# maxgillett/tinysplat

Measured on AMD Instinct MI355X. Metric: Gaussians*pixels/s fwd+bwd, higher is better.
Workload: dtype f32; 1 GPU; 1000000 random Gaussians, SH degree 3, 1920x1080, fwd+bwd (RGB), BASELINE configs[2]; max_per_tile=614, parallelism=single GPU, tile_lists=16x16 (gsplat's) (auto), gaussian_order=as generated (i.i.d.)

## Files before the change

### include/tinysplat_hip.h

```cpp
#ifndef TINYSPLAT_HIP_H
#define TINYSPLAT_HIP_H

#include <stdint.h>

#ifdef __cplusplus
extern "C" {
#endif

#define TS_ABI_VERSION 8

#define TS_E_BADARG (-1)
#define TS_E_DEGREE (-2)

#define TS_TILE 16
#define TS_SPLAT_RECORD_FLOATS 12
#define TS_PARTIAL_ROW_FLOATS 12

int ts_abi_version(void);

typedef struct ts_camera {
    float fx, fy, cx, cy;
    int32_t img_width, img_height;
    int32_t tile_bounds_x, tile_bounds_y;
    int32_t tile_row0, tile_rows;
    float glob_scale;
    float clip_thresh;
    int32_t wide_tiles;
    int32_t hints;
} ts_camera;
#define TS_HINT_BALANCED_WALK 1
#define TS_HINT_COOP_SPLIT (1 << 20)
#define TS_CAM_LIST_SEGMENTS(s) (((s) & 15) << 8)
#define TS_CAM_WHOLE_TILES(w16) (((w16) & 15) << 12)
#define TS_CAM_COOP_TILES(c16) (((c16) & 15) << 16)
int64_t ts_final_floats(const ts_camera* cam_host, int32_t channels);
int32_t ts_cut_tiles(const ts_camera* cam_host, int32_t* band, int32_t* whole);
int32_t ts_num_tiles(const ts_camera* cam_host);


#define TS_PROJECT_LOG_SCALES 1
#define TS_PROJECT_RAW_QUATS 2

int ts_project_fwd(int32_t n, const float* means3d, const float* scales, const float* quats,
                   const float* viewmat, const float* projmat, const ts_camera* cam_host,
                   int32_t flags, float* xys, float* depths, int32_t* radii, float* conics,
                   int32_t* num_tiles_hit, float* cov3d, void* stream);

int ts_project_bwd(int32_t n, const float* means3d, const float* scales, const float* quats,
                   const float* viewmat, const float* projmat, const ts_camera* cam_host,
                   int32_t flags, const int32_t* radii, const float* v_xy, const float* v_depth,
                   const float* v_conic, const float* v_cov3d,
                   float* v_means3d, float* v_scales, float* v_quats, void* stream);


int ts_sh_fwd(int32_t n, int32_t degrees_to_use, int32_t num_bases, const float* viewdirs,
              const float* coeffs, float* colors, void* stream);

int ts_sh_bwd(int32_t n, int32_t degrees_to_use, int32_t num_bases, const float* viewdirs,
              const float* v_colors, float* v_coeffs, void* stream);

int ts_sh_colors_fwd(int32_t n, int32_t degrees_to_use, int32_t num_bases, const float* means3d,
                     const float* origin, const float* colors_dc, const float* colors_rest,
                     float* colors, uint8_t* clamp_mask, const int32_t* live, void* stream);
int ts_sh_colors_bwd(int32_t n, int32_t degrees_to_use, int32_t num_bases, const float* means3d,
                     const float* origin, const uint8_t* clamp_mask, const float* v_colors,
                     float* v_colors_dc, float* v_colors_rest, void* stream);
int ts_colors_pack_fwd(int32_t n, int32_t degrees_to_use, int32_t num_bases, const float* means3d,
                       const float* origin, const float* colors_dc, const float* colors_rest,
                       uint8_t* clamp_mask, const int32_t* live, int32_t channels, int32_t flags,
                       const float* xys, const int32_t* radii, const float* conics, const float* opacity,
                       const int32_t* cum_tiles_hit, const ts_camera* cam_host, const float* depths,
                       float* splats, void* stream);


int64_t ts_scan_ws_ints(int32_t n);
int ts_scan_tiles(int32_t n, const int32_t* num_tiles_hit, int32_t* cum_tiles_hit,
                  int32_t* scan_ws, int32_t* total_out, void* stream);

int64_t ts_bin_ws_ints(int32_t n, int32_t num_tiles);

int ts_bin_count(int32_t n, const float* xys, const int32_t* radii, const float* splats,
                 const ts_camera* cam_host, int32_t* bin_ws, void* stream);

int ts_tile_offsets(int32_t n, int32_t num_tiles, int32_t* bin_ws, int32_t* tile_bins,
                    const int32_t* cum_tiles_hit, int64_t capacity, void* stream);
int ts_tile_offsets_stats(int32_t n, int32_t num_tiles, int32_t* bin_ws, int32_t* tile_bins,
                          const int32_t* cum_tiles_hit, int64_t capacity, int32_t* longest_list, void* stream);

int ts_bin_scatter(int32_t n, const float* xys, const int32_t* radii, const float* splats,
                   const ts_camera* cam_host, const int32_t* bin_ws, int32_t* bucket_ids, int32_t* scratch,
                   void* stream);

int ts_sort_tiles(int32_t num_tiles, const int32_t* tile_bins, const float* depths,
                  const int32_t* bucket_ids, int32_t* gaussian_ids_sorted, int32_t* sort_ws,
                  int32_t* zeroed_counter, void* stream);
int ts_sort_tiles_above(int32_t num_tiles, const int32_t* tile_bins, const float* depths,
                        const int32_t* bucket_ids, int32_t* gaussian_ids_sorted, int32_t* sort_ws,
                        int32_t* zeroed_counter, void* stream);

int32_t ts_bin_group_form(int32_t n);
int ts_bin_count_groups(int32_t n, const float* xys, const int32_t* radii, const float* splats,
                        const ts_camera* cam_host, int32_t* bin_ws, void* stream);
int ts_group_offsets(int32_t n, int32_t num_tiles, int32_t* bin_ws, int32_t* tile_bins,
                     const int32_t* cum_tiles_hit, int64_t capacity, int32_t* longest_list, void* stream);
int ts_bin_scatter_groups(int32_t n, const float* xys, const int32_t* radii, const float* splats,
                          const ts_camera* cam_host, int32_t* bin_ws, int32_t* tile_bins, int32_t* bucket_ids,
                          int32_t* scratch, void* stream);
int32_t ts_bin_one_walk_form(int32_t n, int32_t num_tiles);
int32_t ts_bin_stage_capacity(void);
int ts_bin_emit_groups(int32_t n, const float* xys, const int32_t* radii, const float* splats,
                       const ts_camera* cam_host, const int32_t* cum_tiles_hit, int64_t capacity, int32_t* bin_ws,
                       int32_t* scratch, void* stream);
int ts_emit_offsets(int32_t n, int32_t num_tiles, int32_t* bin_ws, int32_t* tile_bins,
                    const int32_t* cum_tiles_hit, int64_t capacity, int32_t* longest_list, void* stream);
int ts_bin_gather_groups(int32_t n, int32_t num_tiles, int32_t* bin_ws, int32_t* tile_bins, int32_t* bucket_ids,
                         const int32_t* scratch, void* stream);
int ts_sort_tiles_stats(int32_t num_tiles, const int32_t* tile_bins, const float* depths,
                        const int32_t* bucket_ids, int32_t* gaussian_ids_sorted, int32_t* sort_ws,
                        int32_t* zeroed_counter, int32_t n, const int32_t* bin_ws, int32_t* longest_list,
                        void* stream);
int ts_sort_tiles_above_stats(int32_t num_tiles, const int32_t* tile_bins, const float* depths,
                              const int32_t* bucket_ids, int32_t* gaussian_ids_sorted, int32_t n,
                              const int32_t* bin_ws, int32_t* longest_list, void* stream);

#define TS_RASTER_LOGIT_OPACITY 1

int ts_pack_splats(int32_t n, int32_t channels, int32_t flags, const float* xys, const int32_t* radii,
                   const float* conics, const float* colors, const float* opacity,
                   const int32_t* cum_tiles_hit, const ts_camera* cam_host, const float* depths,
                   float* splats, void* stream);

#define TS_RASTER_CLAMP_RGB 2
#define TS_RASTER_SPLIT_BLOCKS 4
#define TS_RASTER_NARROW_WAVES 8
#define TS_RASTER_FLAG_GEN(g) (((g) & 0xff) << 8)
int ts_raster_fwd(int32_t channels, int32_t flags, const ts_camera* cam_host, const int32_t* tile_bins,
                  const int32_t* gaussian_ids_sorted, const float* splats, const float* background,
                  float* out_img, float* final_Ts, int32_t* final_index, uint8_t* clamp_mask,
                  void* stream);
int ts_raster_fwd_planes(int32_t channels, int32_t flags, const ts_camera* cam_host, const int32_t* tile_bins,
                         const int32_t* gaussian_ids_sorted, const float* splats, const float* background,
                         float* out_img, float* out_depth, float* final_Ts, int32_t* final_index,
                         uint8_t* clamp_mask, void* stream);

int ts_raster_fwd_sort(int32_t channels, int32_t flags, const ts_camera* cam_host, const int32_t* tile_bins,
                       const int32_t* bucket_ids, const float* depths, int32_t* gaussian_ids_sorted,
                       const float* splats, const float* background, float* out_img, float* out_depth,
                       float* final_Ts, int32_t* final_index, uint8_t* clamp_mask, void* stream);

int ts_raster_bwd(int32_t channels, int32_t flags, int64_t num_intersects, const ts_camera* cam_host,
                  const int32_t* tile_bins, const int32_t* gaussian_ids_sorted, const float* splats,
                  const float* background, const float* final_Ts, const int32_t* final_index,
                  const float* v_out_img, const float* v_out_alpha, const uint8_t* clamp_mask,
                  float* partials, uint8_t* row_flags, void* stream);
int ts_raster_bwd_planes(int32_t channels, int32_t flags, int64_t num_intersects, const ts_camera* cam_host,
                         const int32_t* tile_bins, const int32_t* gaussian_ids_sorted, const float* splats,
                         const float* background, const float* final_Ts, const int32_t* final_index,
                         const float* v_out_img, const float* v_out_depth, int32_t planes,
                         const float* v_out_alpha, const uint8_t* clamp_mask,
                         float* partials, uint8_t* row_flags, void* stream);

int ts_reduce_partials(int32_t n, int32_t channels, int32_t flags, const int32_t* num_tiles_hit,
                       const int32_t* cum_tiles_hit, const float* partials,
                       const uint8_t* row_flags, const float* splats, float* v_xy, float* v_conic,
                       float* v_colors, float* v_opacity, float* v_depth, const uint8_t* color_mask,
                       void* stream);

#define TS_FRAME_TIGHT 1
#define TS_FRAME_SPLIT 2
#define TS_FRAME_NARROW_WAVES 8
#define TS_FRAME_DIRECT_SCATTER 32
#define TS_FRAME_PLANES 64
#define TS_FRAME_LIST_STATS 256
#define TS_FRAME_SEPARATE_SORT 128
#define TS_FRAME_STRIPE 16
#define TS_FRAME_GROUP_COUNTS 1024
#define TS_FRAME_ONE_WALK 2048
#define TS_FRAME_SURVIVORS 512
typedef struct ts_frame {
    int32_t n, num_bases, sh_degree, channels, flags;
    int32_t flag_gen;
    ts_camera cam;
    const float *means, *scales, *quats, *opacities, *colors_dc, *colors_rest;
    const float *view34, *projview, *origin, *background;
    float *xys, *depths, *conics, *colors, *splats;
    int32_t *radii, *num_tiles_hit, *cum_tiles_hit;
    uint8_t* sh_mask;
    int32_t *scan_ws, *bin_ws, *tile_bins;
    int32_t* total_host;
    int64_t num_intersects;
    int64_t capacity;
    int32_t *bucket_ids, *gaussian_ids_sorted;
    float *out_img, *final_Ts;
    int32_t* final_index;
    uint8_t* clamp_mask;
    const float* v_out_img;
    float* partials;
    uint8_t* row_flags;
    float *v_xy, *v_conic, *v_colors, *v_depth, *v_opacity;
    float *v_means, *v_scales, *v_quats, *v_colors_dc, *v_colors_rest;
    float* out_depth;
    const float* v_out_depth;
    int32_t* survivors;
} ts_frame;
int32_t ts_frame_struct_bytes(void);
int ts_frame_fwd_project(const ts_frame* f, void* stream);
int ts_frame_fwd_prepare(const ts_frame* f, void* stream);
int ts_frame_fwd_composite(const ts_frame* f, void* stream);
int ts_frame_bwd_composite(const ts_frame* f, void* stream);
int ts_frame_bwd_params(const ts_frame* f, void* stream);

typedef void (*ts_entry_probe)(const char* entry, int32_t end, void* user);
int ts_set_entry_probe(ts_entry_probe fn, void* user);

#define TS_MAX_RANKS 16
#define TS_EXPORT_RECORD_FLOATS 16
typedef struct ts_stripes {
    int32_t num;
    int32_t row[TS_MAX_RANKS + 1];
} ts_stripes;
int64_t ts_route_ws_ints(int32_t n, int32_t num_ranks);
int ts_route_count(int32_t n, const float* xys, const int32_t* radii, const ts_camera* cam_host,
                   const ts_stripes* stripes_host, int32_t* route_ws, int32_t* counts, void* stream);
int ts_route_count_padded(int32_t n, const float* xys, const int32_t* radii, const ts_camera* cam_host,
                          const ts_stripes* stripes_host, const int32_t* group_base_host, int32_t* route_ws,
                          int32_t* counts, void* stream);
int ts_route_pack(int32_t n, int32_t gid_base, const float* xys, const int32_t* radii, const float* depths,
                  const float* splats, const ts_camera* cam_host, const ts_stripes* stripes_host,
                  const int32_t* route_ws, float* records, void* stream);
int ts_import_records(int32_t m, const float* records, const ts_camera* cam_host, float* xys, float* depths,
                      int32_t* radii, int32_t* num_tiles_hit, void* stream);
int ts_import_pack(int32_t m, const float* records, const int32_t* cum_tiles_hit, const ts_camera* cam_host,
                   float* splats, void* stream);
int ts_reduce_partials_rows(int32_t n, int32_t channels, int32_t flags, const int32_t* num_tiles_hit,
                            const int32_t* cum_tiles_hit, const float* partials, const uint8_t* row_flags,
                            const float* splats, float* grad_rows, void* stream);
int ts_route_accumulate(int32_t n, int32_t channels, const float* xys, const int32_t* radii, const float* splats,
                        const uint8_t* color_mask, const ts_camera* cam_host, const ts_stripes* stripes_host,
                        const int32_t* route_ws, const float* grad_rows, float* v_xy, float* v_conic,
                        float* v_colors, float* v_depth, float* v_opacity, void* stream);

int ts_shard_owner_fwd(const ts_frame* fo, const ts_stripes* stripes_host, int32_t* route_ws, int32_t* counts,
                       void* stream);
int ts_shard_owner_fwd_padded(const ts_frame* fo, const ts_stripes* stripes_host, const int32_t* group_base_host,
                              int32_t* route_ws, int32_t* counts, void* stream);
int ts_shard_owner_fwd_fused(int32_t n, int32_t degrees_to_use, int32_t num_bases, const float* means3d,
                             const float* scales, const float* quats, const float* view34, const float* projview,
                             const ts_camera* cam_host, int32_t project_flags, const float* origin,
                             const float* colors_dc, const float* colors_rest, const float* opacity, int32_t channels,
                             int32_t raster_flags, float* xys, float* depths, int32_t* radii, float* conics,
                             int32_t* num_tiles_hit, uint8_t* clamp_mask, float* splats, const ts_stripes* stripes_host,
                             const int32_t* group_base_host, int32_t* route_ws, int32_t* counts, void* stream);
int ts_shard_owner_bwd_fused(int32_t n, int32_t channels, int32_t degrees_to_use, int32_t num_bases, const float* means3d,
                             const float* scales, const float* quats, const float* view34, const float* projview,
                             const float* origin, const float* xys, const int32_t* radii, const float* splats,
                             const uint8_t* color_mask, const ts_camera* cam_host, const ts_stripes* stripes_host,
                             const int32_t* route_ws, const float* grad_rows, float* v_xy, float* v_conic,
                             float* v_colors, float* v_depth, float* v_opacity, float* v_colors_dc, float* v_colors_rest,
                             float* v_means3d, float* v_scales, float* v_quats, void* stream);
int ts_shard_stripe_fwd_import(const ts_frame* fs, const float* records, void* stream);
int ts_shard_stripe_bwd(const ts_frame* fs, float* grad_rows, void* stream);
int ts_shard_owner_bwd(const ts_frame* fo, const ts_stripes* stripes_host, const int32_t* route_ws,
                       const float* grad_rows, void* stream);

typedef struct ts_rank_step {
    ts_stripes stripes;
    int32_t group_base[TS_MAX_RANKS + 1];
    int32_t gid_base;
    int32_t send_rows, recv_rows;
    int32_t* route_ws;
    int32_t* counts;
    float *send, *recv;
    float *grad_rows, *back;
} ts_rank_step;
int32_t ts_rank_step_struct_bytes(void);
int ts_shard_rank_fwd_a(const ts_frame* fo, const ts_rank_step* r, void* stream);
int ts_shard_rank_fwd_b(const ts_frame* fs, const ts_rank_step* r, void* stream);
int ts_shard_rank_bwd_a(const ts_frame* fs, const ts_rank_step* r, void* stream);
int ts_shard_rank_bwd_b(const ts_frame* fo, const ts_rank_step* r, void* stream);


int64_t ts_photometric_ws_floats(int32_t height, int32_t width);
int ts_photometric_loss_rgbd(int32_t height, int32_t width, int32_t pixel_floats, const float* image,
                             const float* target, const float* depth_target, float w_l1,
                             float w_ssim, float w_depth, float* ws, float* v_image, void* stream);
int ts_photometric_loss(int32_t height, int32_t width, const float* image, const float* target,
                        float w_l1, float w_ssim, float* ws, float* v_image, void* stream);
int ts_photometric_loss_planes(int32_t height, int32_t width, const float* image, const float* depth,
                               const float* target, const float* depth_target, float w_l1, float w_ssim,
                               float w_depth, float* ws, float* v_image, float* v_depth, void* stream);
int ts_photometric_loss_reduce(int32_t height, int32_t width, float w_l1, float w_ssim, float w_depth,
                               const float* ws, float* out4, void* stream);

#define TS_ADAM_MAX_TENSORS 8
int ts_adam_step(int32_t num_tensors, float* const* params_host, const float* const* grads_host,
                 float* const* exp_avg_host, float* const* exp_avg_sq_host, const int64_t* numel_host,
                 const float* lr_host, const int32_t* steps_host, float beta1, float beta2, float eps,
                 void* stream);

#define TS_ADAM_MEANS 0
#define TS_ADAM_COLORS_DC 1
#define TS_ADAM_COLORS_REST 2
#define TS_ADAM_SCALES 3
#define TS_ADAM_QUATS 4
#define TS_ADAM_OPACITIES 5
typedef struct ts_adam {
    float* exp_avg[6];
    float* exp_avg_sq[6];
    float lr[6];
    int32_t step[6];
    float beta1, beta2, eps;
} ts_adam;
int ts_sh_colors_bwd_adam(int32_t n, int32_t degrees_to_use, int32_t num_bases, const float* means3d,
                          const float* origin, const uint8_t* clamp_mask, const float* v_colors,
                          float* colors_dc, float* colors_rest, const ts_adam* adam_host, void* stream);
int ts_project_bwd_adam(int32_t n, float* means3d, float* scales, float* quats, const float* viewmat,
                        const float* projmat, const ts_camera* cam_host, int32_t flags, const int32_t* radii,
                        const float* v_xy, const float* v_depth, const float* v_conic, float* opacities,
                        const float* v_opacity, const ts_adam* adam_host, void* stream);
int ts_frame_bwd_params_adam(const ts_frame* f, const ts_adam* adam_host, void* stream);

#define TS_DENSIFY_CLONE 1
#define TS_DENSIFY_SPLIT 2
#define TS_DENSIFY_PRUNE 4

typedef struct ts_densify_policy {
    float interval_densify;
    float max_dim;
    float tau_means;
    float scale_thresh;
} ts_densify_policy;
// ... 161 lines not shown
```

### tinysplat_amd/_lib.py

```python
from __future__ import annotations

import ctypes
import os
from ctypes import POINTER, c_double, c_float, c_int32, c_int64, c_void_p
from pathlib import Path

LIB_PATH = Path(os.environ["TS_LIB_PATH"]) if os.environ.get("TS_LIB_PATH") else \
    Path(__file__).resolve().parent / "csrc" / "libtinysplat_hip.so"
ABI_VERSION = 8
HINT_BALANCED_WALK = 1
HINT_COOP_SPLIT = 1 << 20
PARTIAL_ROW_FLOATS = 12


class TsCamera(ctypes.Structure):
    _fields_ = [
        ("fx", c_float), ("fy", c_float), ("cx", c_float), ("cy", c_float),
        ("img_width", c_int32), ("img_height", c_int32),
        ("tile_bounds_x", c_int32), ("tile_bounds_y", c_int32),
        ("tile_row0", c_int32), ("tile_rows", c_int32),
        ("glob_scale", c_float), ("clip_thresh", c_float),
        ("wide_tiles", c_int32), ("hints", c_int32),
    ]


_P = c_void_p
_CAM = POINTER(TsCamera)


class TsDensifyPolicy(ctypes.Structure):
    _fields_ = [("interval_densify", c_float), ("max_dim", c_float), ("tau_means", c_float),
                ("scale_thresh", c_float)]


class TsFrame(ctypes.Structure):
    _fields_ = ([("n", c_int32), ("num_bases", c_int32), ("sh_degree", c_int32), ("channels", c_int32),
                 ("flags", c_int32), ("flag_gen", c_int32), ("cam", TsCamera)]
                + [(name, c_void_p) for name in (
                    "means", "scales", "quats", "opacities", "colors_dc", "colors_rest",
                    "view34", "projview", "origin", "background",
                    "xys", "depths", "conics", "colors", "splats",
                    "radii", "num_tiles_hit", "cum_tiles_hit", "sh_mask",
                    "scan_ws", "bin_ws", "tile_bins", "total_host")]
                + [("num_intersects", c_int64), ("capacity", c_int64)]
                + [(name, c_void_p) for name in (
                    "bucket_ids", "gaussian_ids_sorted", "out_img", "final_Ts", "final_index", "clamp_mask",
                    "v_out_img", "partials", "row_flags",
                    "v_xy", "v_conic", "v_colors", "v_depth", "v_opacity",
                    "v_means", "v_scales", "v_quats", "v_colors_dc", "v_colors_rest",
                    "out_depth", "v_out_depth", "survivors")])


_FRAME = POINTER(TsFrame)


class TsAdam(ctypes.Structure):
    _fields_ = [("exp_avg", c_void_p * 6), ("exp_avg_sq", c_void_p * 6), ("lr", c_float * 6), ("step", c_int32 * 6),
                ("beta1", c_float), ("beta2", c_float), ("eps", c_float)]


_ADAM = POINTER(TsAdam)

MAX_RANKS = 16


class TsStripes(ctypes.Structure):
    _fields_ = [("num", c_int32), ("row", c_int32 * (MAX_RANKS + 1))]


_STRIPES = POINTER(TsStripes)


class TsRankStep(ctypes.Structure):
    _fields_ = [("stripes", TsStripes), ("group_base", c_int32 * (MAX_RANKS + 1)), ("gid_base", c_int32),
                ("send_rows", c_int32), ("recv_rows", c_int32), ("route_ws", c_void_p), ("counts", c_void_p),
                ("send", c_void_p), ("recv", c_void_p), ("grad_rows", c_void_p), ("back", c_void_p)]


_RANK = POINTER(TsRankStep)

ENTRY_PROBE = ctypes.CFUNCTYPE(None, ctypes.c_char_p, c_int32, c_void_p)

SIGNATURES = {
    "ts_abi_version": (c_int32, []),
    "ts_project_fwd": (c_int32, [c_int32, _P, _P, _P, _P, _P, _CAM, c_int32, _P, _P, _P, _P, _P, _P, _P]),
    "ts_project_bwd": (c_int32, [c_int32, _P, _P, _P, _P, _P, _CAM, c_int32, _P, _P, _P, _P, _P, _P, _P, _P, _P]),
    "ts_sh_fwd": (c_int32, [c_int32, c_int32, c_int32, _P, _P, _P, _P]),
    "ts_sh_bwd": (c_int32, [c_int32, c_int32, c_int32, _P, _P, _P, _P]),
    "ts_sh_colors_fwd": (c_int32, [c_int32, c_int32, c_int32, _P, _P, _P, _P, _P, _P, _P, _P]),
    "ts_sh_colors_bwd": (c_int32, [c_int32, c_int32, c_int32, _P, _P, _P, _P, _P, _P, _P]),
    "ts_scan_ws_ints": (c_int64, [c_int32]),
    "ts_scan_tiles": (c_int32, [c_int32, _P, _P, _P, _P, _P]),
    "ts_bin_ws_ints": (c_int64, [c_int32, c_int32]),
    "ts_bin_count": (c_int32, [c_int32, _P, _P, _P, _CAM, _P, _P]),
    "ts_tile_offsets": (c_int32, [c_int32, c_int32, _P, _P, _P, c_int64, _P]),
    "ts_tile_offsets_stats": (c_int32, [c_int32, c_int32, _P, _P, _P, c_int64, _P, _P]),
    "ts_bin_scatter": (c_int32, [c_int32, _P, _P, _P, _CAM, _P, _P, _P, _P]),
    "ts_sort_tiles": (c_int32, [c_int32, _P, _P, _P, _P, _P, _P, _P]),
    "ts_sort_tiles_above": (c_int32, [c_int32, _P, _P, _P, _P, _P, _P, _P]),
    "ts_bin_group_form": (c_int32, [c_int32]),
    "ts_bin_count_groups": (c_int32, [c_int32, _P, _P, _P, _CAM, _P, _P]),
    "ts_group_offsets": (c_int32, [c_int32, c_int32, _P, _P, _P, c_int64, _P, _P]),
    "ts_bin_scatter_groups": (c_int32, [c_int32, _P, _P, _P, _CAM, _P, _P, _P, _P, _P]),
    "ts_bin_one_walk_form": (c_int32, [c_int32, c_int32]),
    "ts_bin_stage_capacity": (c_int32, []),
    "ts_bin_emit_groups": (c_int32, [c_int32, _P, _P, _P, _CAM, _P, c_int64, _P, _P, _P]),
    "ts_emit_offsets": (c_int32, [c_int32, c_int32, _P, _P, _P, c_int64, _P, _P]),
    "ts_bin_gather_groups": (c_int32, [c_int32, c_int32, _P, _P, _P, _P, _P]),
    "ts_sort_tiles_stats": (c_int32, [c_int32, _P, _P, _P, _P, _P, _P, c_int32, _P, _P, _P]),
    "ts_sort_tiles_above_stats": (c_int32, [c_int32, _P, _P, _P, _P, c_int32, _P, _P, _P]),
    "ts_num_tiles": (c_int32, [_CAM]),
    "ts_final_floats": (c_int64, [_CAM, c_int32]),
    "ts_cut_tiles": (c_int32, [_CAM, _P, _P]),
    "ts_colors_pack_fwd": (c_int32, [c_int32, c_int32, c_int32, _P, _P, _P, _P, _P, _P, c_int32, c_int32,
                                     _P, _P, _P, _P, _P, _CAM, _P, _P, _P]),
    "ts_pack_splats": (c_int32, [c_int32, c_int32, c_int32, _P, _P, _P, _P, _P, _P, _CAM, _P, _P, _P]),
    "ts_raster_fwd": (c_int32, [c_int32, c_int32, _CAM, _P, _P, _P, _P, _P, _P, _P, _P, _P]),
    "ts_raster_bwd": (c_int32, [c_int32, c_int32, c_int64, _CAM, _P, _P, _P, _P, _P, _P, _P, _P, _P, _P, _P, _P]),
    "ts_raster_fwd_planes": (c_int32, [c_int32, c_int32, _CAM, _P, _P, _P, _P, _P, _P, _P, _P, _P, _P]),
    "ts_raster_fwd_sort": (c_int32, [c_int32, c_int32, _CAM, _P, _P, _P, _P, _P, _P, _P, _P, _P, _P, _P, _P]),
    "ts_raster_bwd_planes": (c_int32, [c_int32, c_int32, c_int64, _CAM, _P, _P, _P, _P, _P, _P, _P, _P, c_int32,
                                       _P, _P, _P, _P, _P]),
    "ts_bench_stream_read": (c_int32, [_P, c_int64, _P, _P]),
    "ts_bench_gather48": (c_int32, [_P, _P, c_int64, _P, _P]),
    "ts_photometric_ws_floats": (c_int64, [c_int32, c_int32]),
    "ts_photometric_loss": (c_int32, [c_int32, c_int32, _P, _P, c_float, c_float, _P, _P, _P]),
    "ts_photometric_loss_rgbd": (c_int32, [c_int32, c_int32, c_int32, _P, _P, _P, c_float, c_float, c_float, _P, _P, _P]),
    "ts_photometric_loss_planes": (c_int32, [c_int32, c_int32, _P, _P, _P, _P, c_float, c_float, c_float, _P, _P, _P,
                                             _P]),
    "ts_photometric_loss_reduce": (c_int32, [c_int32, c_int32, c_float, c_float, c_float, _P, _P, _P]),
    "ts_adam_step": (c_int32, [c_int32, _P, _P, _P, _P, _P, _P, _P, c_float, c_float, c_float, _P]),
    "ts_sh_colors_bwd_adam": (c_int32, [c_int32, c_int32, c_int32, _P, _P, _P, _P, _P, _P, _ADAM, _P]),
    "ts_project_bwd_adam": (c_int32, [c_int32, _P, _P, _P, _P, _P, _CAM, c_int32, _P, _P, _P, _P, _P, _P, _ADAM, _P]),
    "ts_frame_bwd_params_adam": (c_int32, [_FRAME, _ADAM, _P]),
    "ts_grad_accum": (c_int32, [c_int32, _P, _P, _P]),
    "ts_densify_classify": (c_int32, [c_int32, _P, _P, _P, POINTER(TsDensifyPolicy), _P, _P]),
    "ts_densify_ws_ints": (c_int64, [c_int32]),
    "ts_densify_plan": (c_int32, [c_int32, _P, _P, _P, _P, _P]),
    "ts_gather_rows": (c_int32, [c_int32, _P, _P, _P, c_int32, c_int32, _P, _P]),
    "ts_split_fixup": (c_int32, [c_int32, _P, _P, _P, _P, _P, _P, _P, _P]),
    "ts_ply_row_floats": (c_int32, [c_int32]),
    "ts_ply_pack_rows": (c_int32, [c_int32, c_int32, _P, _P, _P, _P, _P, _P, _P, _P]),
    "ts_ply_unpack_rows": (c_int32, [c_int32, c_int32, _P, _P, _P, _P, _P, _P, _P, _P]),
    "ts_reduce_partials": (c_int32, [c_int32, c_int32, c_int32, _P, _P, _P, _P, _P, _P, _P, _P, _P, _P, _P, _P]),
    "ts_route_ws_ints": (c_int64, [c_int32, c_int32]),
    "ts_route_count": (c_int32, [c_int32, _P, _P, _CAM, _STRIPES, _P, _P, _P]),
    "ts_route_count_padded": (c_int32, [c_int32, _P, _P, _CAM, _STRIPES, _P, _P, _P, _P]),
    "ts_route_pack": (c_int32, [c_int32, c_int32, _P, _P, _P, _P, _CAM, _STRIPES, _P, _P, _P]),
    "ts_import_records": (c_int32, [c_int32, _P, _CAM, _P, _P, _P, _P, _P]),
    "ts_import_pack": (c_int32, [c_int32, _P, _P, _CAM, _P, _P]),
    "ts_reduce_partials_rows": (c_int32, [c_int32, c_int32, c_int32, _P, _P, _P, _P, _P, _P, _P]),
    "ts_route_accumulate": (c_int32, [c_int32, c_int32, _P, _P, _P, _P, _CAM, _STRIPES, _P, _P, _P, _P, _P, _P, _P, _P]),
    "ts_shard_owner_fwd": (c_int32, [_FRAME, _STRIPES, _P, _P, _P]),
    "ts_shard_owner_fwd_padded": (c_int32, [_FRAME, _STRIPES, _P, _P, _P, _P]),
    "ts_shard_owner_fwd_fused": (c_int32, [c_int32, c_int32, c_int32, _P, _P, _P, _P, _P, _CAM, c_int32, _P, _P, _P, _P,
                                           c_int32, c_int32, _P, _P, _P, _P, _P, _P, _P, _STRIPES, _P, _P, _P, _P]),
    "ts_shard_owner_bwd_fused": (c_int32, [c_int32, c_int32, c_int32, c_int32, _P, _P, _P, _P, _P, _P, _P, _P, _P, _P,
                                           _CAM, _STRIPES, _P, _P, _P, _P, _P, _P, _P, _P, _P, _P, _P, _P, _P]),
    "ts_shard_stripe_fwd_import": (c_int32, [_FRAME, _P, _P]),
    "ts_shard_stripe_bwd": (c_int32, [_FRAME, _P, _P]),
    "ts_shard_owner_bwd": (c_int32, [_FRAME, _STRIPES, _P, _P, _P]),
    "ts_rank_step_struct_bytes": (c_int32, []),
    "ts_shard_rank_fwd_a": (c_int32, [_FRAME, _RANK, _P]),
    "ts_shard_rank_fwd_b": (c_int32, [_FRAME, _RANK, _P]),
    "ts_shard_rank_bwd_a": (c_int32, [_FRAME, _RANK, _P]),
    "ts_shard_rank_bwd_b": (c_int32, [_FRAME, _RANK, _P]),
    "ts_frame_struct_bytes": (c_int32, []),
    "ts_frame_fwd_project": (c_int32, [_FRAME, _P]),
    "ts_frame_fwd_prepare": (c_int32, [_FRAME, _P]),
    "ts_frame_fwd_composite": (c_int32, [_FRAME, _P]),
    "ts_frame_bwd_composite": (c_int32, [_FRAME, _P]),
    "ts_frame_bwd_params": (c_int32, [_FRAME, _P]),
    "ts_set_entry_probe": (c_int32, [_P, _P]),
    "ts_knn_ws_bytes": (c_int64, [c_int32, c_int32, c_int32]),
    "ts_knn": (c_int32, [c_int32, _P, c_int32, _P, c_int32, _P, _P, _P, _P, _P]),
    "ts_init_from_points": (c_int32, [c_int32, c_int32, _P, _P, _P, _P, _P, _P, _P, _P, _P, _P, _P, _P, _P, _P]),
    "ts_opacity_entropy_ws_bytes": (c_int64, [c_int32]),
    "ts_opacity_entropy": (c_int32, [c_int32, _P, _P, _P, _P, _P]),
    "ts_density_sample_ws_bytes": (c_int64, [c_int32]),
    "ts_density_sample": (c_int32, [c_int32, c_int32, c_int32, _P, _P, _P, _P, _P, _P, _P, _P, _P, _P, _P]),
    "ts_density_loss_ws_bytes": (c_int64, [c_int32]),
    "ts_density_loss": (c_int32, [c_int32, c_int32, _P, _P, _P, _P, _P, _P, _P, _P, c_int32, c_int32, _P, _P, c_int32,
                                  c_float, _P, _P, _P, _P, _P, _P, _P, _P, _P, _P]),
    "ts_segment_sum_ws_bytes": (c_int64, [c_int64, c_int32]),
    "ts_segment_sum": (c_int32, [c_int64, c_int32, c_int32, _P, _P, _P, _P, _P, _P, _P]),
    "ts_extract_pack": (c_int32, [c_int32, _P, _P, _P, _P, _P, _P, _P]),
    "ts_extract_rays": (c_int32, [c_int32, _P, c_int32, c_int32, _P, c_int32, _P, _P, _P, _P, _P, _P]),
    "ts_extract_samples": (c_int32, [c_int32, c_int32, c_int32, c_float, _P, _P, _P, _P, _P, _P, _P]),
    "ts_extract_march": (c_int32, [c_int32, c_int32, c_int32, c_float, c_float, _P, _P, _P, _P, _P, _P, _P, _P, _P, _P,
                                   _P, _P, _P]),
    "ts_extract_normals": (c_int32, [c_int32, c_int32, _P, _P, _P, _P, _P]),
    "ts_extract_chunk_bytes": (c_int64, [c_int32, c_int32, c_int32]),
    "ts_mesh_boxes": (c_int32, [c_int32, _P, _P, _P, c_float, _P, _P]),
    "ts_mesh_mark": (c_int32, [c_int32, _P, _P, _P, _P, _P]),
    "ts_mesh_chunk_bytes": (c_int64, [c_int32, c_int32]),
    "ts_mesh_corners": (c_int32, [c_int32, _P, _P, _P, _P, _P]),
    "ts_mesh_density": (c_int32, [c_int32, c_int32, _P, _P, _P, _P, _P, _P, _P, _P]),
    "ts_mesh_count": (c_int32, [c_int32, _P, _P, _P, c_float, _P, _P, _P]),
    "ts_mesh_emit": (c_int32, [c_int32, _P, _P, _P, c_float, _P, _P, _P, _P, _P, _P]),
    "ts_field_colors": (c_int32, [c_int32, c_int32, _P, _P, _P, _P, _P, _P, c_int32, c_int32, _P, _P]),
    "ts_simplify_count": (c_int32, [c_int32, c_int32, _P, _P, _P, _P, _P, _P]),
    "ts_simplify_keys": (c_int32, [c_int32, _P, _P, _P, _P, _P]),
    "ts_simplify_ws_bytes": (c_int64, [c_int64]),
    "ts_simplify_accumulate": (c_int32, [c_int32, c_int32, c_int32, _P, _P, _P, _P, c_int32, c_int64, _P, _P, c_int64,
                                         c_int64, _P, _P, _P]),
    "ts_simplify_solve": (c_int32, [c_int32, _P, _P, _P, _P, _P, c_double, _P, _P]),
    "ts_simplify_faces": (c_int32, [c_int32, c_int32, _P, _P, _P, _P, _P]),
    "ts_clean_degenerate": (c_int32, [c_int32, _P, _P, _P]),
    "ts_clean_edge_keys": (c_int32, [c_int32, c_int32, _P, _P, _P]),
    "ts_clean_face_weights": (c_int32, [c_int32, c_int32, _P, _P, _P, _P]),
    "ts_clean_mark": (c_int32, [c_int32, c_int64, _P, _P, _P, _P]),
    "ts_clean_components": (c_int32, [c_int32, c_int32, _P, _P, _P, _P]),
    "ts_splat_keys": (c_int32, [c_int32, _P, _P, _P, _P]),
    "ts_splat_pack": (c_int32, [c_int32, c_int32, _P, _P, _P, _P, _P, _P, _P, _P]),
    "ts_splat_unpack": (c_int32, [c_int32, _P, _P, _P, _P, _P, _P, _P]),
    "ts_undistort_image": (c_int32, [_P, c_int32, c_int32, POINTER(c_float), POINTER(c_float), POINTER(c_float),
                                     c_int32, c_int32, c_int32, _P, _P]),
    "ts_jpeg_ws_bytes": (c_int64, [c_int32, c_int32, c_int32, c_int32]),
    "ts_jpeg_max_bytes": (c_int64, [c_int32, c_int32, c_int32, c_int32]),
    "ts_jpeg_header": (c_int64, [c_int32, c_int32, c_int32, c_int32, c_int32, _P, c_int64]),
    "ts_jpeg_encode": (c_int32, [_P, c_int32, c_int32, c_int32, c_int32, c_int32, c_int32, c_int32, _P, _P, c_int64, _P,
                                 _P, _P]),
    "ts_image_metrics_ws_bytes": (c_int64, [c_int32, c_int32]),
    "ts_image_metrics": (c_int32, [c_int32, c_int32, c_int32, _P, _P, c_int32, _P, _P, _P]),
}

_lib = None


class HipLibraryError(RuntimeError):
    pass


def load() -> ctypes.CDLL:
    global _lib
    if _lib is not None:
        return _lib
    if not LIB_PATH.exists():
        raise HipLibraryError(
            f"{LIB_PATH} is missing: tinysplat_amd has no CPU or PyTorch fallback. "
            "Build it with `python -m tinysplat_amd._build` (needs hipcc, targets gfx950).")
    stamp = LIB_PATH.with_suffix(LIB_PATH.suffix + ".flags")
    if stamp.exists() and "-DTS_" in stamp.read_text() and os.environ.get("TS_ALLOW_VARIANT_LIB") != "1":
        raise HipLibraryError(
            f"{LIB_PATH} was built with developer -DTS_* overrides (ablation variant; its results may be "
            "wrong). Rebuild with `python -m tinysplat_amd._build`, or set TS_ALLOW_VARIANT_LIB=1.")
    lib = ctypes.CDLL(str(LIB_PATH))
    for name, (res, args) in SIGNATURES.items():
        try:
            fn = getattr(lib, name)
        except AttributeError as e:
            raise HipLibraryError(f"{LIB_PATH} does not export {name}") from e
        fn.restype = res
        fn.argtypes = args
    v = lib.ts_abi_version()
    if v != ABI_VERSION:
        raise HipLibraryError(f"ABI version mismatch: library {v}, binding {ABI_VERSION}")
    if lib.ts_frame_struct_bytes() != ctypes.sizeof(TsFrame):
        raise HipLibraryError("struct ts_frame: the ctypes mirror does not match the library's layout")
    if lib.ts_rank_step_struct_bytes() != ctypes.sizeof(TsRankStep):
        raise HipLibraryError("struct ts_rank_step: the ctypes mirror does not match the library's layout")
    _lib = lib
    return lib


def check(code: int, what: str) -> None:
    if code == 0:
        return
# ... 6 lines not shown
```

### tinysplat_amd/csrc/binning.hip

```cpp
#include <hip/hip_runtime.h>

#include "../../include/tinysplat_hip.h"
#include "host_util.h"
#include "pack.h"
#include "splat_math.h"

namespace {

constexpr int kThreads = 256;
constexpr int kScanItems = 4;
constexpr int kScanBlock = kThreads * kScanItems;

__device__ __forceinline__ int wave_inclusive_scan(int v) {
    const int lane = threadIdx.x & 63;
#pragma unroll
    for (int d = 1; d < 64; d <<= 1) {
        const int u = __shfl_up(v, d, 64);
        if (lane >= d) v += u;
    }
    return v;
}

template <int WAVES = 4>
__device__ __forceinline__ int block_inclusive_scan(int v, int* total) {
    __shared__ int wave_sums[WAVES];
    const int lane = threadIdx.x & 63, wave = threadIdx.x >> 6;
    int inc = wave_inclusive_scan(v);
    if (lane == 63) wave_sums[wave] = inc;
    __syncthreads();
    int add = 0, tot = 0;
#pragma unroll
    for (int w = 0; w < WAVES; ++w) {
        const int s = wave_sums[w];
        if (w < wave) add += s;
        tot += s;
    }
    *total = tot;
    __syncthreads();
    return inc + add;
}

__global__ __launch_bounds__(kThreads) void scan_local_kernel(int n, const int* __restrict__ in,
                                                              int* __restrict__ out,
                                                              int* __restrict__ block_sums,
                                                              int* __restrict__ total_out) {
    const int base = blockIdx.x * kScanBlock + threadIdx.x * kScanItems;
    int v[kScanItems];
    int sum = 0;
#pragma unroll
    for (int k = 0; k < kScanItems; ++k) {
        v[k] = (base + k < n) ? in[base + k] : 0;
        sum += v[k];
        v[k] = sum;
    }
    int total;
    const int inc = block_inclusive_scan(sum, &total);
    const int excl = inc - sum;
#pragma unroll
    for (int k = 0; k < kScanItems; ++k)
        if (base + k < n) {
            out[base + k] = v[k] + excl;
            if (total_out && gridDim.x == 1 && base + k == n - 1)
                __hip_atomic_store(total_out, v[k] + excl, __ATOMIC_RELEASE, __HIP_MEMORY_SCOPE_SYSTEM);
        }
    if (threadIdx.x == 0) block_sums[blockIdx.x] = total;
}

__global__ __launch_bounds__(kThreads) void scan_add_kernel(int n, int* __restrict__ out,
                                                            const int* __restrict__ block_sums,
                                                            int* __restrict__ total_out) {
    __shared__ int red[kThreads / 64];
    int part = 0;
    for (int j = threadIdx.x; j < (int)blockIdx.x; j += kThreads) part += block_sums[j];
#pragma unroll
    for (int d = 32; d >= 1; d >>= 1) part += __shfl_xor(part, d, 64);
    if ((threadIdx.x & 63) == 0) red[threadIdx.x >> 6] = part;
    __syncthreads();
    int add = 0;
#pragma unroll
    for (int w = 0; w < kThreads / 64; ++w) add += red[w];
    const int base = blockIdx.x * kScanBlock + threadIdx.x * kScanItems;
#pragma unroll
    for (int k = 0; k < kScanItems; ++k)
        if (base + k < n) {
            const int v = out[base + k] + add;
            if (blockIdx.x != 0) out[base + k] = v;
            if (total_out && base + k == n - 1)
                __hip_atomic_store(total_out, v, __ATOMIC_RELEASE, __HIP_MEMORY_SCOPE_SYSTEM);
        }
}

#ifndef TS_BIN_THREADS
#define TS_BIN_THREADS 1024
#endif
constexpr int kBinThreads = TS_BIN_THREADS;
#ifndef TS_BIN_CHUNK
#define TS_BIN_CHUNK 4096
#endif
constexpr int kBinChunkMin = TS_BIN_CHUNK;
constexpr int kBinMaxChunks = 512;
constexpr int kBinWindowMax = 36864;
constexpr int kBinTargetBlocks = 1;

__host__ __device__ inline int bin_num_chunks(int n) {
    int per = n / 192;
    per = per < 1024 ? 1024 : (per > kBinChunkMin ? kBinChunkMin : per);
    int b = (n + per - 1) / per;
    if (b < 1) b = 1;
    if (b > kBinMaxChunks) b = kBinMaxChunks;
    return b;
}

inline int bin_window_tiles(int n, int num_tiles) {
    const int chunks = bin_num_chunks(n);
    int nwin = (kBinTargetBlocks + chunks - 1) / chunks;
    const int max_win = (num_tiles + 255) / 256;
    if (nwin > max_win) nwin = max_win;
    if (nwin < 1) nwin = 1;
    int window = (num_tiles + nwin - 1) / nwin;
    window = (window + 63) & ~63;
    if (window > kBinWindowMax) window = kBinWindowMax;
    return window;
}

using ts::TightTest;

#ifndef TS_BIN_PRE
#define TS_BIN_PRE 2
#endif
constexpr int kBinPre = TS_BIN_PRE;
template <typename Emit>
__device__ __forceinline__ void walk_chunk(int g0, int g1, const float* __restrict__ xys,
                                           const int* __restrict__ radii,
                                           const float4* __restrict__ splats, const ts_camera& cam,
                                           Emit emit) {
    const int ws = cam.wide_tiles ? 1 : 0;
    const int tbx = (cam.tile_bounds_x + ws) >> ws;
    const bool tight_lists = splats != nullptr;
    for (int base = g0 + threadIdx.x; base < g1; base += kBinPre * kBinThreads) {
        int r[kBinPre];
        float2 xy[kBinPre];
        float4 q0[kBinPre], q1[kBinPre];
#pragma unroll
        for (int u = 0; u < kBinPre; ++u) {
            const int i = base + u * kBinThreads;
            r[u] = i < g1 ? radii[i] : 0;
        }
#pragma unroll
        for (int u = 0; u < kBinPre; ++u) {
            const int i = base + u * kBinThreads;
            xy[u] = make_float2(0.f, 0.f);
            q0[u] = q1[u] = make_float4(0.f, 0.f, 0.f, 0.f);
            if (r[u] > 0) {
                xy[u] = reinterpret_cast<const float2*>(xys)[i];
                if (tight_lists) { q0[u] = splats[3 * (size_t)i]; q1[u] = splats[3 * (size_t)i + 1]; }
            }
        }
#pragma unroll
        for (int u = 0; u < kBinPre; ++u) {
            if (r[u] <= 0) continue;
            const ts::TileBox b = ts::tile_bbox(xy[u].x, xy[u].y, (float)r[u], cam.tile_bounds_x,
                                                cam.tile_bounds_y, cam.tile_row0, cam.tile_rows);
            if (b.maxy <= b.miny || b.maxx <= b.minx) continue;
            const TightTest tight(tight_lists, q0[u].x, q0[u].y, q0[u].z, q0[u].w, q1[u].x, q1[u].y, (float)r[u]);
            if (tight.cull_all) continue;
            const int i = base + u * kBinThreads;
            for (int ty = b.miny; ty < b.maxy; ++ty) {
                int lo, hi;
                tight.row_range(ty, b.minx, b.maxx, lo, hi);
                if (hi <= lo) continue;
                for (int tx = lo >> ws; tx <= (hi - 1) >> ws; ++tx) emit((ty - cam.tile_row0) * tbx + tx, i);
            }
        }
    }
}

constexpr int kItemCap = 4096;
constexpr int kStashWords = 11;
constexpr size_t kBalancedLds = (size_t)(kStashWords * kBinThreads + kItemCap + 32) * 4;
template <typename Emit>
__device__ __forceinline__ void walk_chunk_balanced(int g0, int g1, const float* __restrict__ xys,
                                                    const int* __restrict__ radii,
                                                    const float4* __restrict__ splats, const ts_camera& cam,
                                                    Emit emit) {
    static_assert(kBinThreads == 1024, "one Gaussian per thread and batch, items packed as lt | row << 10");
    __shared__ float stash[kStashWords][kBinThreads];
    __shared__ int items[kItemCap];
    __shared__ int wave_sum[kBinThreads / 64 + 1];
    const int ws = cam.wide_tiles ? 1 : 0;
    const int tbx = (cam.tile_bounds_x + ws) >> ws;
    const bool tight_lists = splats != nullptr;
    const int tid = threadIdx.x, lane = tid & 63, wave = tid >> 6;
    for (int base = g0; base < g1; base += kBinThreads) {
// ... 841 lines not shown

constexpr int kMaxSub = 512;
constexpr int kSubTarget = 96;
constexpr int kLargeLdsU64 = kSortCap + 2048;

__device__ __forceinline__ void sort_tile_sample(const int* __restrict__ g,
                                                 const float* __restrict__ depths,
                                                 int* __restrict__ out, int n,
                                                 unsigned long long* lds) {
    unsigned long long* scratch = lds;
    unsigned long long* smp = lds + kSortCap;
    int* start = reinterpret_cast<int*>(lds + kSortCap + 1024);
    int* cursor = start + (kMaxSub + 1);
    int* big = cursor + kMaxSub;
    __shared__ int nbig;
    const int t = threadIdx.x, lane = t & 63, wave = t >> 6;
    const int ns = n > 8192 ? 1024 : 256;
    int nb = n / kSubTarget;
    nb = nb < 2 ? 2 : (nb > kMaxSub ? kMaxSub : nb);

    if (ns == 1024) {
        unsigned long long k[4];
#pragma unroll
        for (int e = 0; e < 4; ++e)
            k[e] = make_key(depths, g[(int)(((long long)(t * 4 + e) * n) >> 10)]);
        bitonic_regs<4, kThreads>(k, t, 1024, scratch);
#pragma unroll
        for (int e = 0; e < 4; ++e) smp[t * 4 + e] = k[e];
    } else {
        unsigned long long k[1];
        k[0] = make_key(depths, g[(int)(((long long)t * n) >> 8)]);
        bitonic_regs<1, kThreads>(k, t, 256, scratch);
        smp[t] = k[0];
    }
    for (int b = t; b < nb; b += kThreads) cursor[b] = 0;
    if (t == 0) nbig = 0;
    __syncthreads();

    auto sub_of = [&](unsigned long long key) {
        int lo = 0, hi = nb - 1;
        while (lo < hi) {
            const int mid = (lo + hi) >> 1;
            if (smp[((mid + 1) * ns) / nb] <= key) lo = mid + 1; else hi = mid;
        }
        return lo;
    };
    for (int i = t; i < n; i += kThreads) atomicAdd(&cursor[sub_of(make_key(depths, g[i]))], 1);
    __syncthreads();
    {
        const int c0 = (2 * t < nb) ? cursor[2 * t] : 0, c1 = (2 * t + 1 < nb) ? cursor[2 * t + 1] : 0;
        int total;
        const int inc = block_inclusive_scan(c0 + c1, &total);
        const int ex = inc - (c0 + c1);
        if (2 * t < nb) start[2 * t] = ex;
        if (2 * t + 1 < nb) start[2 * t + 1] = ex + c0;
        if (t == 0) start[nb] = n;
    }
    __syncthreads();
    for (int b = t; b < nb; b += kThreads) cursor[b] = start[b];
    __syncthreads();
    for (int i = t; i < n; i += kThreads) {
        const int id = g[i];
        out[atomicAdd(&cursor[sub_of(make_key(depths, id))], 1)] = id;
    }
    __threadfence_block();
    __syncthreads();
    for (int b = wave; b < nb; b += kThreads / 64) {
        const int s0 = start[b], m = start[b + 1] - s0;
        if (m <= 1) continue;
        if (m <= 256) {
            unsigned long long k[4];
#pragma unroll
            for (int e = 0; e < 4; ++e) {
                const int i = lane * 4 + e;
                k[e] = i < m ? make_key(depths, out[s0 + i]) : ~0ull;
            }
            bitonic_regs<4, 64>(k, lane, min(pow2_at_least(m), 256), nullptr);
#pragma unroll
            for (int e = 0; e < 4; ++e) {
                const int i = lane * 4 + e;
                if (i < m) out[s0 + i] = (int)(unsigned int)k[e];
            }
        } else if (lane == 0) {
            big[atomicAdd(&nbig, 1)] = b;
        }
    }
    __syncthreads();
    const int nbg = nbig;
    for (int q = 0; q < nbg; ++q) {
        const int b = big[q];
        const int s0 = start[b], m = start[b + 1] - s0;
        __syncthreads();
        if (m <= kSortCap) {
            sort_bucket_block(out + s0, depths, out + s0, m, scratch);
        } else {
            IdKeyArray a{out + s0, depths};
            bitonic_network(a, m);
        }
        __syncthreads();
    }
}

__global__ __launch_bounds__(kThreads) void sort_tiles_small_kernel(
    int num_tiles, const int* __restrict__ tile_bins, const float* __restrict__ depths,
    const int* __restrict__ bucket_ids, int* __restrict__ ids_sorted, int* __restrict__ large_count,
    int* __restrict__ large_list, const ListStats stats) {
    if (stats.group_max && blockIdx.x == 0) store_longest(stats);
    const int lane = threadIdx.x & 63;
    const int tile = blockIdx.x * (kThreads / 64) + (threadIdx.x >> 6);
    if (tile >= num_tiles) return;
    const int2 range = reinterpret_cast<const int2*>(tile_bins)[tile];
    const int n = range.y - range.x;
    if (n <= 0) return;
    if (n > kWaveSortMax) {
        if (n > kSortCap && lane == 0) large_list[atomicAdd(large_count, 1)] = tile;
        return;
    }
    const int* g = bucket_ids + range.x;
    int* out = ids_sorted + range.x;
    if (n <= 64) sort_tile_wave<1>(g, depths, out, n, lane);
    else if (n <= 128) sort_tile_wave<2>(g, depths, out, n, lane);
    else if (n <= 256) sort_tile_wave<4>(g, depths, out, n, lane);
    else if (n <= 512) sort_tile_wave<8>(g, depths, out, n, lane);
    else sort_tile_wave<16>(g, depths, out, n, lane);
}

__global__ __launch_bounds__(kThreads) void sort_tiles_mid_kernel(
    const int* __restrict__ tile_bins, const float* __restrict__ depths,
    const int* __restrict__ bucket_ids, int* __restrict__ ids_sorted, int* __restrict__ large_count,
    int* __restrict__ large_list) {
    __shared__ unsigned long long lk[kSortCap / 2];
    const int2 range = reinterpret_cast<const int2*>(tile_bins)[blockIdx.x];
    const int n = range.y - range.x;
    if (n > kSortCap && large_count && threadIdx.x == 0) large_list[atomicAdd(large_count, 1)] = blockIdx.x;
    if (n <= kWaveSortMax || n > kSortCap) return;
    sort_bucket_block(bucket_ids + range.x, depths, ids_sorted + range.x, n, lk);
}

__global__ __launch_bounds__(kThreads) void sort_tiles_large_kernel(
    const int* __restrict__ tile_bins, const float* __restrict__ depths,
    const int* __restrict__ bucket_ids, int* __restrict__ ids_sorted,
    const int* __restrict__ large_count, const int* __restrict__ large_list) {
    __shared__ unsigned long long lds_large[kLargeLdsU64];
    const int count = *large_count;
    for (int q = blockIdx.x; q < count; q += gridDim.x) {
        const int2 range = reinterpret_cast<const int2*>(tile_bins)[large_list[q]];
        const int n = range.y - range.x;
        if (n <= kSortCap) continue;
        __syncthreads();
        sort_tile_sample(bucket_ids + range.x, depths, ids_sorted + range.x, n, lds_large);
    }
}

__global__ __launch_bounds__(kThreads) void sort_tiles_above_kernel(
    const int* __restrict__ tile_bins, const float* __restrict__ depths,
    const int* __restrict__ bucket_ids, int* __restrict__ ids_sorted, const ListStats stats) {
    __shared__ unsigned long long lds_u64[kLargeLdsU64 > kSortCap / 2 ? kLargeLdsU64 : kSortCap / 2];
    if (stats.group_max && blockIdx.x == 0) store_longest(stats);
    const int2 range = reinterpret_cast<const int2*>(tile_bins)[blockIdx.x];
    const int n = range.y - range.x;
    if (n <= kWaveSortMax) return;
    if (n <= kSortCap) sort_bucket_block(bucket_ids + range.x, depths, ids_sorted + range.x, n, lds_u64);
    else sort_tile_sample(bucket_ids + range.x, depths, ids_sorted + range.x, n, lds_u64);
}

__global__ __launch_bounds__(kThreads) void pack_splats_kernel(int n, const ts::PackArgs a,
                                                              const float* __restrict__ colors) {
    const int i = blockIdx.x * kThreads + threadIdx.x;
    if (i >= n) return;
    if (a.radii[i] <= 0) return;
    float c0, c1, c2, c3 = 0.0f;
    if (a.channels == 4 && a.depths == nullptr) {
        const float4 c = reinterpret_cast<const float4*>(colors)[i];
        c0 = c.x; c1 = c.y; c2 = c.z; c3 = c.w;
    } else {
        c0 = colors[3 * i]; c1 = colors[3 * i + 1]; c2 = colors[3 * i + 2];
        if (a.channels == 4) c3 = a.depths[i];
    }
    ts::pack_one(a, i, c0, c1, c2, c3);
}

}

extern "C" {

int32_t ts_num_tiles(const ts_camera* cam) {
    if (!cam) return 0;
    const int tbx = cam->wide_tiles ? (cam->tile_bounds_x + 1) / 2 : cam->tile_bounds_x;
    return cam->tile_rows * tbx;
}

int64_t ts_scan_ws_ints(int32_t n) {
    return n <= 0 ? 1 : (int64_t)((n + kScanBlock - 1) / kScanBlock);
}

int ts_scan_tiles(int32_t n, const int32_t* num_tiles_hit, int32_t* cum_tiles_hit,
                  int32_t* scan_ws, int32_t* total_out, void* stream) {
    if (n < 0) return TS_E_BADARG;
    if (n == 0) return 0;
    if (!num_tiles_hit || !cum_tiles_hit || !scan_ws) return TS_E_BADARG;
    hipStream_t s = (hipStream_t)stream;
    const int nb = (n + kScanBlock - 1) / kScanBlock;
    hipLaunchKernelGGL(scan_local_kernel, dim3(nb), dim3(kThreads), 0, s, n, num_tiles_hit,
                       cum_tiles_hit, scan_ws, total_out);
    if (nb > 1)
        hipLaunchKernelGGL(scan_add_kernel, dim3(nb), dim3(kThreads), 0, s, n, cum_tiles_hit, scan_ws,
                           total_out);
    return launch_status();
}

int64_t ts_bin_ws_ints(int32_t n, int32_t num_tiles) { return bin_geometry(n, num_tiles).spare + 1; }

int ts_bin_count(int32_t n, const float* xys, const int32_t* radii, const float* splats,
                 const ts_camera* cam, int32_t* bin_ws, void* stream) {
    if (n < 0 || !cam || !bin_ws) return TS_E_BADARG;
    const int nt = ts_num_tiles(cam);
    if (nt <= 0) return 0;
    if (n > 0 && (!xys || !radii)) return TS_E_BADARG;
    const BinGeometry g = bin_geometry(n, nt);
    const int window = bin_window_tiles(n, nt);
    const int windows = (nt + window - 1) / window;
    const size_t lds = (size_t)window * sizeof(int);
    if (lds > 64 * 1024)
        (void)hipFuncSetAttribute(reinterpret_cast<const void*>(&bin_count_kernel),
                                  hipFuncAttributeMaxDynamicSharedMemorySize, (int)lds);
    hipLaunchKernelGGL(bin_count_kernel, dim3(g.chunks, windows), dim3(kBinThreads), lds,
                       (hipStream_t)stream, n, g.chunk, xys, radii,
                       reinterpret_cast<const float4*>(splats), *cam, nt, window, bin_ws);
    return launch_status();
}

int ts_tile_offsets(int32_t n, int32_t num_tiles, int32_t* bin_ws, int32_t* tile_bins,
                    const int32_t* cum_tiles_hit, int64_t capacity, void* stream) {
    return ts_tile_offsets_stats(n, num_tiles, bin_ws, tile_bins, cum_tiles_hit, capacity, nullptr, stream);
}

int ts_tile_offsets_stats(int32_t n, int32_t num_tiles, int32_t* bin_ws, int32_t* tile_bins,
                          const int32_t* cum_tiles_hit, int64_t capacity, int32_t* longest_list, void* stream) {
    if (n < 0 || num_tiles < 0) return TS_E_BADARG;
    if (num_tiles == 0) return 0;
    if (!bin_ws || !tile_bins) return TS_E_BADARG;
    const BinGeometry g = bin_geometry(n, num_tiles);
    int* tile_total = bin_ws + g.tile_start;
    const int per_group = (g.chunks + kScanGroups - 1) / kScanGroups;
    hipStream_t s = (hipStream_t)stream;
    hipLaunchKernelGGL(column_scan_kernel, dim3((num_tiles + kColTiles - 1) / kColTiles),
                       dim3(kColTiles * kScanGroups), 0, s, num_tiles, g.chunks, per_group, bin_ws, tile_total, true);
    hipLaunchKernelGGL(tile_offsets_kernel, dim3(1), dim3(kOffsetsThreads), 0, s, num_tiles, tile_total,
                       tile_bins, bin_ws + g.spare,
                       (cum_tiles_hit && n > 0) ? cum_tiles_hit + (n - 1) : nullptr, (long long)capacity, longest_list);
    return launch_status();
}

int32_t ts_bin_group_form(int32_t n) { return two_hop(n) ? 1 : 0; }

int ts_bin_count_groups(int32_t n, const float* xys, const int32_t* radii, const float* splats,
                        const ts_camera* cam, int32_t* bin_ws, void* stream) {
    if (!cam || !bin_ws || !xys || !radii || !two_hop(n)) return TS_E_BADARG;
    const int nt = ts_num_tiles(cam);
    if (nt <= 0) return 0;
    const BinGeometry g = bin_geometry(n, nt);
    hipLaunchKernelGGL(group_bin_count_kernel, dim3(g.chunks), dim3(kBinThreads), (size_t)g.groups * sizeof(int),
                       (hipStream_t)stream, n, g.chunk, xys, radii, reinterpret_cast<const float4*>(splats), *cam,
                       g.groups, bin_ws);
    return launch_status();
}

}

namespace {
template <bool BASES>
int group_offsets(const BinGeometry& g, int num_tiles, int* bin_ws, int* tile_bins, const int* total_ptr,
                  long long capacity, int* longest_list, hipStream_t s) {
    int* counts = bin_ws + (BASES ? 0 : g.counts);
    int* col_total = nullptr;
    if ((long long)g.chunks * g.groups > kGoSingleMax || g.groups > kGoLdsGroups) {
        col_total = bin_ws + (BASES ? g.group_totals : g.col_total);
        const int per_group = (g.chunks + kScanGroups - 1) / kScanGroups;
        hipLaunchKernelGGL(column_scan_kernel, dim3((g.groups + kColTiles - 1) / kColTiles),
                           dim3(kColTiles * kScanGroups), 0, s, g.groups, g.chunks, per_group, counts, col_total, BASES);
        counts = nullptr;
    }
    hipLaunchKernelGGL(group_tile_offsets_kernel<BASES>, dim3(1), dim3(kGoThreads), 0, s, num_tiles, g.groups, g.chunks,
                       counts, (const int*)col_total, bin_ws + g.tile_start, tile_bins, bin_ws + g.spare, total_ptr,
                       capacity, longest_list);
    return launch_status();
}
}

extern "C" {

int ts_group_offsets(int32_t n, int32_t num_tiles, int32_t* bin_ws, int32_t* tile_bins,
                     const int32_t* cum_tiles_hit, int64_t capacity, int32_t* longest_list, void* stream) {
    if (num_tiles < 0 || !two_hop(n)) return TS_E_BADARG;
    if (num_tiles == 0) return 0;
    if (!bin_ws || !tile_bins) return TS_E_BADARG;
    return group_offsets<true>(bin_geometry(n, num_tiles), num_tiles, bin_ws, tile_bins,
                               cum_tiles_hit ? cum_tiles_hit + (n - 1) : nullptr, (long long)capacity, longest_list,
                               (hipStream_t)stream);
}

int ts_bin_scatter_groups(int32_t n, const float* xys, const int32_t* radii, const float* splats,
                          const ts_camera* cam, int32_t* bin_ws, int32_t* tile_bins, int32_t* bucket_ids,
                          int32_t* scratch, void* stream) {
    if (!cam || !xys || !radii || !bin_ws || !tile_bins || !bucket_ids || !scratch || !two_hop(n))
        return TS_E_BADARG;
    const int nt = ts_num_tiles(cam);
    if (nt <= 0) return 0;
    const BinGeometry g = bin_geometry(n, nt);
    int* tile_start = bin_ws + g.tile_start;
    hipStream_t s = (hipStream_t)stream;
    const auto coarse = (cam->hints & TS_HINT_BALANCED_WALK) ? bin_scatter_coarse_kernel<true, true>
                                                             : bin_scatter_coarse_kernel<false, true>;
    hipLaunchKernelGGL(coarse, dim3(g.chunks), dim3(kBinThreads), (size_t)g.groups * sizeof(int), s, n, g.chunk, xys,
                       radii, reinterpret_cast<const float4*>(splats), *cam, nt, (const int*)bin_ws,
                       (const int*)tile_start, scratch);
    hipLaunchKernelGGL(bin_scatter_fine_groups_kernel, dim3(g.groups), dim3(kFineThreads), 0, s, nt, tile_start,
                       tile_bins, bin_ws + g.group_max, (const int*)scratch, bucket_ids);
    return launch_status();
}

int32_t ts_bin_one_walk_form(int32_t n, int32_t num_tiles) { return one_walk_form(n, num_tiles) ? 1 : 0; }

int32_t ts_bin_stage_capacity(void) { return kStageCap; }

int ts_bin_emit_groups(int32_t n, const float* xys, const int32_t* radii, const float* splats,
                       const ts_camera* cam, const int32_t* cum_tiles_hit, int64_t capacity, int32_t* bin_ws,
                       int32_t* scratch, void* stream) {
    if (!cam || !xys || !radii || !cum_tiles_hit || !bin_ws || !scratch) return TS_E_BADARG;
    const int nt = ts_num_tiles(cam);
    if (!one_walk_form(n, nt) || (cam->hints & TS_HINT_BALANCED_WALK)) return TS_E_BADARG;
    const BinGeometry g = bin_geometry(n, nt);
    const size_t lds = (size_t)g.groups * 8 + (size_t)kStageCap * 6;
    (void)hipFuncSetAttribute(reinterpret_cast<const void*>(&bin_scatter_emit_kernel),
                              hipFuncAttributeMaxDynamicSharedMemorySize, (int)lds);
    hipLaunchKernelGGL(bin_scatter_emit_kernel, dim3(g.chunks), dim3(kBinThreads), lds, (hipStream_t)stream, n, g.chunk,
                       xys, radii, reinterpret_cast<const float4*>(splats), *cam, g.groups, cum_tiles_hit,
                       (long long)capacity, bin_ws + g.counts, bin_ws + g.starts, scratch);
    return launch_status();
}

int ts_emit_offsets(int32_t n, int32_t num_tiles, int32_t* bin_ws, int32_t* tile_bins,
                    const int32_t* cum_tiles_hit, int64_t capacity, int32_t* longest_list, void* stream) {
    if (!one_walk_form(n, num_tiles) || !bin_ws || !tile_bins || !cum_tiles_hit) return TS_E_BADARG;
    return group_offsets<false>(bin_geometry(n, num_tiles), num_tiles, bin_ws, tile_bins, cum_tiles_hit + (n - 1),
                                (long long)capacity, longest_list, (hipStream_t)stream);
}

int ts_bin_gather_groups(int32_t n, int32_t num_tiles, int32_t* bin_ws, int32_t* tile_bins, int32_t* bucket_ids,
                         const int32_t* scratch, void* stream) {
    if (!one_walk_form(n, num_tiles) || !bin_ws || !tile_bins || !bucket_ids || !scratch) return TS_E_BADARG;
    const BinGeometry g = bin_geometry(n, num_tiles);
    const size_t lds = (size_t)kRunPass * sizeof(int);
    (void)hipFuncSetAttribute(reinterpret_cast<const void*>(&bin_scatter_fine_runs_kernel),
                              hipFuncAttributeMaxDynamicSharedMemorySize, (int)lds);
    hipLaunchKernelGGL(bin_scatter_fine_runs_kernel, dim3(g.groups), dim3(kFineThreads), lds, (hipStream_t)stream,
                       num_tiles, g.groups, g.chunks, (const int*)(bin_ws + g.counts), (const int*)(bin_ws + g.starts),
                       bin_ws + g.tile_start, tile_bins, bin_ws + g.group_max, scratch, bucket_ids);
    return launch_status();
}

int ts_bin_scatter(int32_t n, const float* xys, const int32_t* radii, const float* splats,
                   const ts_camera* cam, const int32_t* bin_ws, int32_t* bucket_ids, int32_t* scratch,
                   void* stream) {
    if (n < 0 || !cam) return TS_E_BADARG;
    if (n == 0) return 0;
    if (!xys || !radii || !bin_ws || !bucket_ids) return TS_E_BADARG;
    const int nt = ts_num_tiles(cam);
    if (nt <= 0) return 0;
    const BinGeometry g = bin_geometry(n, nt);
    const int* tile_start = bin_ws + g.tile_start;
    hipStream_t s = (hipStream_t)stream;
    if (scratch && two_hop(n)) {
        const auto coarse = (cam->hints & TS_HINT_BALANCED_WALK) ? bin_scatter_coarse_kernel<true, false>
                                                                 : bin_scatter_coarse_kernel<false, false>;
        hipLaunchKernelGGL(coarse, dim3(g.chunks), dim3(kBinThreads), (size_t)g.groups * sizeof(int), s, n, g.chunk, xys,
                           radii, reinterpret_cast<const float4*>(splats), *cam, nt, bin_ws, tile_start, scratch);
        hipLaunchKernelGGL(bin_scatter_fine_kernel, dim3(g.groups), dim3(kFineThreads), 0, s, nt, tile_start,
                           (const int*)scratch, bucket_ids);
        return launch_status();
    }
    const int window = bin_window_tiles(n, nt);
    const int windows = (nt + window - 1) / window;
    const size_t lds = (size_t)window * sizeof(int);
    if (lds > 64 * 1024)
        (void)hipFuncSetAttribute(reinterpret_cast<const void*>(&bin_scatter_kernel),
                                  hipFuncAttributeMaxDynamicSharedMemorySize, (int)lds);
    hipLaunchKernelGGL(bin_scatter_kernel, dim3(g.chunks, windows), dim3(kBinThreads), lds, s, n, g.chunk, xys, radii,
                       reinterpret_cast<const float4*>(splats), *cam, nt, window, bin_ws, tile_start, bucket_ids);
    return launch_status();
}

}

namespace {
inline bool list_stats(int n, int num_tiles, const int32_t* bin_ws, int32_t* longest_list, ListStats* st) {
    *st = ListStats{nullptr, nullptr, nullptr, 0};
    if (!longest_list) return true;
    if (!bin_ws || !two_hop(n) || num_tiles <= 0) return false;
    const BinGeometry g = bin_geometry(n, num_tiles);
    *st = ListStats{bin_ws + g.group_max, bin_ws + g.guard, longest_list, g.groups};
    return true;
}
}

extern "C" {

int ts_sort_tiles(int32_t num_tiles, const int32_t* tile_bins, const float* depths,
                  const int32_t* bucket_ids, int32_t* gaussian_ids_sorted, int32_t* sort_ws,
                  int32_t* zeroed_counter, void* stream) {
    return ts_sort_tiles_stats(num_tiles, tile_bins, depths, bucket_ids, gaussian_ids_sorted, sort_ws, zeroed_counter,
                               0, nullptr, nullptr, stream);
}

int ts_sort_tiles_stats(int32_t num_tiles, const int32_t* tile_bins, const float* depths,
                        const int32_t* bucket_ids, int32_t* gaussian_ids_sorted, int32_t* sort_ws,
                        int32_t* zeroed_counter, int32_t n, const int32_t* bin_ws, int32_t* longest_list,
                        void* stream) {
    if (num_tiles < 0) return TS_E_BADARG;
    if (num_tiles == 0) return 0;
    if (!tile_bins || !depths || !bucket_ids || !gaussian_ids_sorted || !sort_ws) return TS_E_BADARG;
    ListStats stats;
    if (!list_stats(n, num_tiles, bin_ws, longest_list, &stats)) return TS_E_BADARG;
    hipStream_t s = (hipStream_t)stream;
    int32_t* counter = zeroed_counter ? zeroed_counter : sort_ws;
    int32_t* list = zeroed_counter ? sort_ws : sort_ws + 1;
    if (!zeroed_counter) {
        hipError_t e = hipMemsetAsync(sort_ws, 0, sizeof(int32_t), s);
        if (e != hipSuccess) return (int)e;
    }
    hipLaunchKernelGGL(sort_tiles_small_kernel, dim3((num_tiles + kThreads / 64 - 1) / (kThreads / 64)),
                       dim3(kThreads), 0, s, (int)num_tiles, tile_bins, depths, bucket_ids,
                       gaussian_ids_sorted, counter, list, stats);
    hipLaunchKernelGGL(sort_tiles_mid_kernel, dim3(num_tiles), dim3(kThreads), 0, s, tile_bins, depths,
                       bucket_ids, gaussian_ids_sorted, (int*)nullptr, (int*)nullptr);
    const int grid = num_tiles < 768 ? num_tiles : 768;
    hipLaunchKernelGGL(sort_tiles_large_kernel, dim3(grid), dim3(kThreads), 0, s, tile_bins, depths,
                       bucket_ids, gaussian_ids_sorted, counter, list);
    return launch_status();
}

int ts_sort_tiles_above(int32_t num_tiles, const int32_t* tile_bins, const float* depths,
                        const int32_t* bucket_ids, int32_t* gaussian_ids_sorted, int32_t* sort_ws,
                        int32_t* zeroed_counter, void* stream) {
    (void)sort_ws; (void)zeroed_counter;
    return ts_sort_tiles_above_stats(num_tiles, tile_bins, depths, bucket_ids, gaussian_ids_sorted, 0, nullptr, nullptr,
                                     stream);
}

int ts_sort_tiles_above_stats(int32_t num_tiles, const int32_t* tile_bins, const float* depths,
                              const int32_t* bucket_ids, int32_t* gaussian_ids_sorted, int32_t n,
                              const int32_t* bin_ws, int32_t* longest_list, void* stream) {
    if (num_tiles < 0) return TS_E_BADARG;
    if (num_tiles == 0) return 0;
    if (!tile_bins || !depths || !bucket_ids || !gaussian_ids_sorted) return TS_E_BADARG;
    ListStats stats;
    if (!list_stats(n, num_tiles, bin_ws, longest_list, &stats)) return TS_E_BADARG;
    hipLaunchKernelGGL(sort_tiles_above_kernel, dim3(num_tiles), dim3(kThreads), 0, (hipStream_t)stream, tile_bins,
                       depths, bucket_ids, gaussian_ids_sorted, stats);
    return launch_status();
}

int ts_pack_splats(int32_t n, int32_t channels, int32_t flags, const float* xys, const int32_t* radii,
                   const float* conics, const float* colors, const float* opacity,
                   const int32_t* cum_tiles_hit, const ts_camera* cam, const float* depths, float* splats,
                   void* stream) {
    if (n < 0 || !cam || (channels != 3 && channels != 4)) return TS_E_BADARG;
    if (n == 0) return 0;
    if (!xys || !radii || !conics || !colors || !opacity || !cum_tiles_hit || !splats)
        return TS_E_BADARG;
    ts::PackArgs a;
    a.channels = channels; a.flags = (int)flags; a.xys = xys; a.radii = radii; a.conics = conics;
    a.opacity = opacity; a.cum_tiles_hit = cum_tiles_hit; a.depths = depths;
    a.splats = reinterpret_cast<float4*>(splats); a.cam = *cam;
    hipLaunchKernelGGL(pack_splats_kernel, dim3((n + kThreads - 1) / kThreads), dim3(kThreads), 0,
                       (hipStream_t)stream, n, a, colors);
    return launch_status();
}

}
```

### tinysplat_amd/csrc/frame.hip

```cpp
#include <hip/hip_runtime.h>

#include <atomic>
#include <cstdlib>
#if !defined(TS_NO_ROCTX) && __has_include(<rocprofiler-sdk-roctx/roctx.h>)
#include <rocprofiler-sdk-roctx/roctx.h>
#define TS_HAVE_ROCTX 1
#else
#define TS_HAVE_ROCTX 0
#endif

#include "../../include/tinysplat_hip.h"
#include "raster_survivors.h"

struct TsRange {
#if TS_HAVE_ROCTX
    explicit TsRange(const char* name) { roctxRangePush(name); }
    ~TsRange() { roctxRangePop(); }
#else
    explicit TsRange(const char*) {}
#endif
};

static std::atomic<ts_entry_probe> g_probe{nullptr};
static std::atomic<void*> g_probe_user{nullptr};

struct TsEntry {
    explicit TsEntry(const char* label) : fn_(g_probe.load(std::memory_order_relaxed)), label_(label) {
        if (fn_) {
            std::atomic_thread_fence(std::memory_order_acquire);
            user_ = g_probe_user.load(std::memory_order_relaxed);
            fn_(label_, 0, user_);
        }
    }
    ~TsEntry() {
        if (fn_) fn_(label_, 1, user_);
    }
    ts_entry_probe fn_;
    const char* label_;
    void* user_ = nullptr;
};
#define TS_ENTRY(label, call) ((void)TsEntry(label), (call))

#define TS_TRY(call)                 \
    do {                             \
        const int e_ = (call);       \
        if (e_ != 0) return e_;      \
    } while (0)

namespace {
inline bool bad(const ts_frame* f) {
    return !f || f->n < 0 || (f->channels != 3 && f->channels != 4) || f->num_bases < 1;
}
inline int num_tiles(const ts_frame* f) { return ts_num_tiles(&f->cam); }
inline int32_t* mapped_pointer(int32_t* host) {
    static thread_local int32_t* last_host = nullptr;
    static thread_local int32_t* last_dev = nullptr;
    static thread_local int last_device = -1;
    int device = -1;
    if (hipGetDevice(&device) != hipSuccess) return nullptr;
    if (host == last_host && device == last_device) return last_dev;
    void* dev = nullptr;
    if (hipHostGetDevicePointer(&dev, host, 0) != hipSuccess || !dev) {
        (void)hipGetLastError();
        return nullptr;
    }
    last_host = host;
    last_device = device;
    last_dev = static_cast<int32_t*>(dev);
    return last_dev;
}
inline bool segmented(const ts_frame* f) {
    return ((f->cam.hints >> 8) & 15) > 1 && !f->cam.wide_tiles && !(f->flags & TS_FRAME_NARROW_WAVES);
}
inline int bwd_split(const ts_frame* f) {
    return ((f->flags & TS_FRAME_SPLIT) && !segmented(f)) ? TS_RASTER_SPLIT_BLOCKS : 0;
}
inline int small_n_fused() {
    static const int v = [] {
        const char* e = getenv("TS_SMALL_N_FUSED");
        return e ? atoi(e) : 262144;
    }();
    return v;
}
inline bool survivors(const ts_frame* f) {
    return (f->flags & TS_FRAME_SURVIVORS) && f->survivors && f->final_Ts && f->num_intersects > 0 &&
           f->cam.wide_tiles == 0 &&
           !(f->flags & (TS_FRAME_SPLIT | TS_FRAME_NARROW_WAVES | TS_FRAME_SEPARATE_SORT));
}
enum class ListForm { direct, matrix, group, one_walk };
inline ListForm list_form(const ts_frame* f) {
    if ((f->flags & TS_FRAME_DIRECT_SCATTER) || !ts_bin_group_form(f->n)) return ListForm::direct;
    if (!(f->flags & TS_FRAME_GROUP_COUNTS)) return ListForm::matrix;
    if ((f->flags & TS_FRAME_ONE_WALK) && !(f->cam.hints & TS_HINT_BALANCED_WALK) &&
        ts_bin_one_walk_form(f->n, num_tiles(f)))
        return ListForm::one_walk;
    return ListForm::group;
}
inline const float* tight_records(const ts_frame* f) { return (f->flags & TS_FRAME_TIGHT) ? f->splats : nullptr; }
inline int32_t* longest_word(const ts_frame* f) {
    if ((f->flags & TS_FRAME_LIST_STATS) && f->total_host) {
        int32_t* dev = mapped_pointer(f->total_host);
        if (dev) return dev + 1;
    }
    return nullptr;
}
inline int raster_flags(const ts_frame* f) {
    return TS_RASTER_CLAMP_RGB | ((f->flags & TS_FRAME_SPLIT) ? TS_RASTER_SPLIT_BLOCKS : 0) |
           ((f->flags & TS_FRAME_NARROW_WAVES) ? TS_RASTER_NARROW_WAVES : 0);
}
}

extern "C" {

int32_t ts_frame_struct_bytes(void) { return (int32_t)sizeof(ts_frame); }

int ts_set_entry_probe(ts_entry_probe fn, void* user) {
    g_probe_user.store(user, std::memory_order_relaxed);
    g_probe.store(fn, std::memory_order_release);
    return 0;
}

int ts_frame_fwd_project(const ts_frame* f, void* stream) {
    TsRange range_("ts_frame_fwd_project");
    if (bad(f)) return TS_E_BADARG;
    TS_TRY(TS_ENTRY("ts_project_fwd",
                    ts_project_fwd(f->n, f->means, f->scales, f->quats, f->view34, f->projview, &f->cam, 3, f->xys,
                                   f->depths, f->radii, f->conics, f->num_tiles_hit, nullptr, stream)));
    int32_t* total_dev = f->total_host ? mapped_pointer(f->total_host) : nullptr;
    TS_TRY(TS_ENTRY("ts_scan_tiles",
                    ts_scan_tiles(f->n, f->num_tiles_hit, f->cum_tiles_hit, f->scan_ws, total_dev, stream)));
    if (f->n > 0 && f->total_host && !total_dev) {
        const hipError_t e = hipMemcpyAsync(f->total_host, f->cum_tiles_hit + (f->n - 1), sizeof(int32_t),
                                            hipMemcpyDeviceToHost, (hipStream_t)stream);
        if (e != hipSuccess) return (int)e;
    }
    return 0;
}

int ts_frame_fwd_prepare(const ts_frame* f, void* stream) {
    TsRange range_("ts_frame_fwd_prepare");
    if (bad(f)) return TS_E_BADARG;
    TS_TRY(TS_ENTRY("ts_colors_pack_fwd",
                    ts_colors_pack_fwd(f->n, f->sh_degree, f->num_bases, f->means, f->origin, f->colors_dc,
                                       f->num_bases > 1 ? f->colors_rest : nullptr, f->sh_mask,
                                       (f->flags & TS_FRAME_STRIPE) ? f->num_tiles_hit : nullptr, f->channels,
                                       TS_RASTER_LOGIT_OPACITY, f->xys, f->radii, f->conics, f->opacities,
                                       f->cum_tiles_hit, &f->cam, f->channels == 4 ? f->depths : nullptr, f->splats,
                                       stream)));
    const float* tight = tight_records(f);
    switch (list_form(f)) {
    case ListForm::one_walk:
        return 0;
    case ListForm::group:
        TS_TRY(TS_ENTRY("ts_bin_count",
                        ts_bin_count_groups(f->n, f->xys, f->radii, tight, &f->cam, f->bin_ws, stream)));
        return TS_ENTRY("ts_tile_offsets",
                        ts_group_offsets(f->n, num_tiles(f), f->bin_ws, f->tile_bins, f->cum_tiles_hit, f->capacity,
                                         longest_word(f), stream));
    case ListForm::matrix:
    case ListForm::direct:
        TS_TRY(TS_ENTRY("ts_bin_count", ts_bin_count(f->n, f->xys, f->radii, tight, &f->cam, f->bin_ws, stream)));
        return TS_ENTRY("ts_tile_offsets",
                        ts_tile_offsets_stats(f->n, num_tiles(f), f->bin_ws, f->tile_bins, f->cum_tiles_hit,
                                              f->capacity, longest_word(f), stream));
    }
    return TS_E_BADARG;
}

int ts_frame_fwd_composite(const ts_frame* f, void* stream) {
    TsRange range_("ts_frame_fwd_composite");
    if (bad(f) || f->num_intersects < 0) return TS_E_BADARG;
    const bool planes = (f->flags & TS_FRAME_PLANES) != 0;
    if (planes && (f->channels != 4 || !f->out_depth)) return TS_E_BADARG;
    const bool fused_sort = f->num_intersects > 0 && f->cam.wide_tiles == 0 &&
                            !(f->flags & (TS_FRAME_NARROW_WAVES | TS_FRAME_SEPARATE_SORT));
    const ListForm form = list_form(f);
    const float* tight = tight_records(f);
    const bool listed = f->num_intersects > 0;
    int32_t* scratch = f->gaussian_ids_sorted;
    switch (form) {
    case ListForm::one_walk:
        TS_TRY(TS_ENTRY("ts_bin_scatter",
                        ts_bin_emit_groups(f->n, f->xys, f->radii, tight, &f->cam, f->cum_tiles_hit, f->capacity,
                                           f->bin_ws, scratch, stream)));
        TS_TRY(TS_ENTRY("ts_tile_offsets",
                        ts_emit_offsets(f->n, num_tiles(f), f->bin_ws, f->tile_bins, f->cum_tiles_hit, f->capacity,
                                        longest_word(f), stream)));
        if (listed)
            TS_TRY(TS_ENTRY("ts_bin_scatter",
                            ts_bin_gather_groups(f->n, num_tiles(f), f->bin_ws, f->tile_bins, f->bucket_ids, scratch,
                                                 stream)));
        break;
    case ListForm::group:
        if (listed)
            TS_TRY(TS_ENTRY("ts_bin_scatter",
                            ts_bin_scatter_groups(f->n, f->xys, f->radii, tight, &f->cam, f->bin_ws, f->tile_bins,
                                                  f->bucket_ids, scratch, stream)));
        break;
    case ListForm::matrix:
    case ListForm::direct:
        if (listed)
            TS_TRY(TS_ENTRY("ts_bin_scatter",
                            ts_bin_scatter(f->n, f->xys, f->radii, tight, &f->cam, f->bin_ws, f->bucket_ids,
                                           form == ListForm::matrix ? scratch : nullptr, stream)));
        break;
    }
    if (listed) {
        int32_t* counter = f->bin_ws + (ts_bin_ws_ints(f->n, num_tiles(f)) - 1);
        int32_t* longest = (form == ListForm::group || form == ListForm::one_walk) ? longest_word(f) : nullptr;
        if (fused_sort)
            TS_TRY(TS_ENTRY("ts_sort_tiles",
                            ts_sort_tiles_above_stats(num_tiles(f), f->tile_bins, f->depths, f->bucket_ids,
                                                      f->gaussian_ids_sorted, f->n, f->bin_ws, longest, stream)));
        else
            TS_TRY(TS_ENTRY("ts_sort_tiles",
                            ts_sort_tiles_stats(num_tiles(f), f->tile_bins, f->depths, f->bucket_ids,
                                                f->gaussian_ids_sorted, f->bin_ws, counter, f->n, f->bin_ws, longest,
                                                stream)));
    }
    if (fused_sort)
        return TS_ENTRY("ts_raster_fwd",
                        ts_surv::raster_fwd_sort(f->channels, raster_flags(f), &f->cam, f->tile_bins, f->bucket_ids,
                                                 f->depths, f->gaussian_ids_sorted, f->splats, f->background,
                                                 f->out_img, planes ? f->out_depth : nullptr, f->final_Ts,
                                                 f->final_index, f->clamp_mask, survivors(f) ? f->survivors : nullptr,
                                                 stream));
    return TS_ENTRY("ts_raster_fwd",
                    ts_raster_fwd_planes(f->channels, raster_flags(f), &f->cam, f->tile_bins, f->gaussian_ids_sorted,
                                         f->splats, f->background, f->out_img, planes ? f->out_depth : nullptr,
                                         f->final_Ts, f->final_index, f->clamp_mask, stream));
}

int ts_frame_bwd_composite(const ts_frame* f, void* stream) {
    TsRange range_("ts_frame_bwd_composite");
    if (bad(f) || f->num_intersects < 0) return TS_E_BADARG;
    const bool planes = (f->flags & TS_FRAME_PLANES) != 0;
    const bool surv = survivors(f);
    TS_TRY(TS_ENTRY("ts_raster_bwd",
                    ts_surv::raster_bwd(f->channels,
                                        ((raster_flags(f) & ~(TS_RASTER_CLAMP_RGB | TS_RASTER_SPLIT_BLOCKS)) | bwd_split(f)) |
                                            TS_RASTER_FLAG_GEN(f->flag_gen),
                                        f->num_intersects, &f->cam, f->tile_bins, f->gaussian_ids_sorted, f->splats,
                                        f->background, f->final_Ts, f->final_index, f->v_out_img,
                                        planes ? f->v_out_depth : nullptr, planes ? 1 : 0, nullptr, f->clamp_mask,
                                        f->partials, f->row_flags, surv ? f->bucket_ids : nullptr,
                                        surv ? f->survivors : nullptr, stream)));
    const bool stripe = (f->flags & TS_FRAME_STRIPE) != 0;
    return TS_ENTRY("ts_reduce_partials",
                    ts_reduce_partials(f->n, f->channels,
                                       TS_RASTER_LOGIT_OPACITY | bwd_split(f) | TS_RASTER_FLAG_GEN(f->flag_gen),
                                       f->num_tiles_hit, f->cum_tiles_hit, f->partials, f->row_flags, f->splats,
                                       f->v_xy, f->v_conic, f->v_colors, f->v_opacity,
                                       f->channels == 4 ? f->v_depth : nullptr, stripe ? f->sh_mask : nullptr, stream));
}

int ts_frame_bwd_params(const ts_frame* f, void* stream) {
    TsRange range_("ts_frame_bwd_params");
    if (bad(f)) return TS_E_BADARG;
    TS_TRY(TS_ENTRY("ts_sh_colors_bwd",
                    ts_sh_colors_bwd(f->n, f->sh_degree, f->num_bases, f->means, f->origin,
                                     (f->flags & TS_FRAME_STRIPE) ? nullptr : f->sh_mask, f->v_colors, f->v_colors_dc,
                                     f->num_bases > 1 ? f->v_colors_rest : nullptr, stream)));
    return TS_ENTRY("ts_project_bwd",
                    ts_project_bwd(f->n, f->means, f->scales, f->quats, f->view34, f->projview, &f->cam, 3, f->radii,
                                   f->v_xy, f->v_depth, f->v_conic, nullptr, f->v_means, f->v_scales, f->v_quats,
                                   stream));
}

int ts_frame_bwd_params_adam(const ts_frame* f, const ts_adam* adam, void* stream) {
    TsRange range_("ts_frame_bwd_params_adam");
    if (bad(f) || !adam) return TS_E_BADARG;
    TS_TRY(TS_ENTRY("ts_sh_colors_bwd_adam",
                    ts_sh_colors_bwd_adam(f->n, f->sh_degree, f->num_bases, f->means, f->origin,
                                          (f->flags & TS_FRAME_STRIPE) ? nullptr : f->sh_mask, f->v_colors,
                                          const_cast<float*>(f->colors_dc),
                                          f->num_bases > 1 ? const_cast<float*>(f->colors_rest) : nullptr, adam,
                                          stream)));
    return TS_ENTRY("ts_project_bwd_adam",
                    ts_project_bwd_adam(f->n, const_cast<float*>(f->means), const_cast<float*>(f->scales),
                                        const_cast<float*>(f->quats), f->view34, f->projview, &f->cam, 3, f->radii,
                                        f->v_xy, f->v_depth, f->v_conic, const_cast<float*>(f->opacities), f->v_opacity,
                                        adam, stream));
}


int ts_shard_owner_fwd(const ts_frame* fo, const ts_stripes* stripes, int32_t* route_ws, int32_t* counts,
                       void* stream) {
    return ts_shard_owner_fwd_padded(fo, stripes, nullptr, route_ws, counts, stream);
}

int ts_shard_owner_fwd_padded(const ts_frame* fo, const ts_stripes* stripes, const int32_t* group_base,
                              int32_t* route_ws, int32_t* counts, void* stream) {
    TsRange range_("ts_shard_owner_fwd");
    if (bad(fo) || !stripes) return TS_E_BADARG;
    if (fo->n > 0 && fo->n <= small_n_fused())
        return TS_ENTRY("ts_owner_fwd_fused",
                        ts_shard_owner_fwd_fused(fo->n, fo->sh_degree, fo->num_bases, fo->means, fo->scales, fo->quats,
                                                 fo->view34, fo->projview, &fo->cam, 3, fo->origin, fo->colors_dc,
                                                 fo->num_bases > 1 ? fo->colors_rest : nullptr, fo->opacities,
                                                 fo->channels, TS_RASTER_LOGIT_OPACITY, fo->xys, fo->depths, fo->radii,
                                                 fo->conics, fo->num_tiles_hit, fo->sh_mask, fo->splats, stripes,
                                                 group_base, route_ws, counts, stream));
    TS_TRY(TS_ENTRY("ts_project_fwd",
                    ts_project_fwd(fo->n, fo->means, fo->scales, fo->quats, fo->view34, fo->projview, &fo->cam, 3,
                                   fo->xys, fo->depths, fo->radii, fo->conics, fo->num_tiles_hit, nullptr, stream)));
    TS_TRY(TS_ENTRY("ts_colors_pack_fwd",
                    ts_colors_pack_fwd(fo->n, fo->sh_degree, fo->num_bases, fo->means, fo->origin, fo->colors_dc,
                                       fo->num_bases > 1 ? fo->colors_rest : nullptr, fo->sh_mask, nullptr,
                                       fo->channels, TS_RASTER_LOGIT_OPACITY, fo->xys, fo->radii, fo->conics,
                                       fo->opacities, fo->num_tiles_hit, &fo->cam,
                                       fo->channels == 4 ? fo->depths : nullptr, fo->splats, stream)));
    return TS_ENTRY("ts_route_count",
                    ts_route_count_padded(fo->n, fo->xys, fo->radii, &fo->cam, stripes, group_base, route_ws, counts,
                                          stream));
}

int ts_shard_stripe_fwd_import(const ts_frame* fs, const float* records, void* stream) {
    TsRange range_("ts_shard_stripe_fwd_import");
    if (bad(fs)) return TS_E_BADARG;
    if (fs->n > 0) {
        TS_TRY(TS_ENTRY("ts_import_records",
                        ts_import_records(fs->n, records, &fs->cam, fs->xys, fs->depths, fs->radii, fs->num_tiles_hit,
                                          stream)));
        int32_t* total_dev = fs->total_host ? mapped_pointer(fs->total_host) : nullptr;
        TS_TRY(TS_ENTRY("ts_scan_tiles",
                        ts_scan_tiles(fs->n, fs->num_tiles_hit, fs->cum_tiles_hit, fs->scan_ws, total_dev, stream)));
        if (fs->total_host && !total_dev) {
            const hipError_t e = hipMemcpyAsync(fs->total_host, fs->cum_tiles_hit + (fs->n - 1), sizeof(int32_t),
                                                hipMemcpyDeviceToHost, (hipStream_t)stream);
            if (e != hipSuccess) return (int)e;
        }
        TS_TRY(TS_ENTRY("ts_import_pack",
                        ts_import_pack(fs->n, records, fs->cum_tiles_hit, &fs->cam, fs->splats, stream)));
    }
    TS_TRY(TS_ENTRY("ts_bin_count",
                    ts_bin_count(fs->n, fs->xys, fs->radii, tight_records(fs), &fs->cam, fs->bin_ws, stream)));
    return TS_ENTRY("ts_tile_offsets",
                    ts_tile_offsets(fs->n, num_tiles(fs), fs->bin_ws, fs->tile_bins, fs->cum_tiles_hit, fs->capacity,
                                    stream));
}

int ts_shard_stripe_bwd(const ts_frame* fs, float* grad_rows, void* stream) {
    TsRange range_("ts_shard_stripe_bwd");
    if (bad(fs) || fs->num_intersects < 0) return TS_E_BADARG;
    TS_TRY(TS_ENTRY("ts_raster_bwd",
                    ts_raster_bwd(fs->channels,
                                  ((raster_flags(fs) & ~(TS_RASTER_CLAMP_RGB | TS_RASTER_SPLIT_BLOCKS)) | bwd_split(fs)) |
                                      TS_RASTER_FLAG_GEN(fs->flag_gen),
                                  fs->num_intersects, &fs->cam, fs->tile_bins, fs->gaussian_ids_sorted, fs->splats,
                                  fs->background, fs->final_Ts, fs->final_index, fs->v_out_img, nullptr, fs->clamp_mask,
                                  fs->partials, fs->row_flags, stream)));
    return TS_ENTRY("ts_reduce_partials_rows",
                    ts_reduce_partials_rows(fs->n, fs->channels, bwd_split(fs) | TS_RASTER_FLAG_GEN(fs->flag_gen),
                                            fs->num_tiles_hit, fs->cum_tiles_hit, fs->partials, fs->row_flags,
                                            fs->splats, grad_rows, stream));
}

int ts_shard_owner_bwd(const ts_frame* fo, const ts_stripes* stripes, const int32_t* route_ws,
                       const float* grad_rows, void* stream) {
    TsRange range_("ts_shard_owner_bwd");
    if (bad(fo) || !stripes) return TS_E_BADARG;
    if (fo->n > 0 && fo->n <= small_n_fused())
        return TS_ENTRY("ts_owner_bwd_fused",
// ... 55 lines not shown
```

### tinysplat_amd/csrc/pack.h

```cpp
#pragma once

#include <hip/hip_runtime.h>

#include "../../include/tinysplat_hip.h"
#include "splat_math.h"

namespace ts {

struct PackArgs {
    int channels, flags;
    const float* xys;
    const int* radii;
    const float* conics;
    const float* opacity;
    const int* cum_tiles_hit;
    const float* depths;
    float4* splats;
    ts_camera cam;
};

__device__ __forceinline__ void pack_one(const PackArgs& a, int i, float c0, float c1, float c2, float c3) {
    const int r = a.radii[i];
    if (r <= 0) return;
    const float2 xy = reinterpret_cast<const float2*>(a.xys)[i];
    const TileBox b = tile_bbox(xy.x, xy.y, (float)r, a.cam.tile_bounds_x, a.cam.tile_bounds_y,
                                a.cam.tile_row0, a.cam.tile_rows);
    const int w = b.maxx - b.minx, h = b.maxy - b.miny;
    const int cnt = h > 0 ? w * h : 0;
    if (cnt <= 0) return;
    const int excl = a.cum_tiles_hit[i] - cnt;
    const int slot_base = excl - b.miny * w - b.minx;
    float op = a.opacity[i];
    if (a.flags & TS_RASTER_LOGIT_OPACITY) op = 1.0f / (1.0f + expf(-op));
    a.splats[3 * (size_t)i] = make_float4(xy.x, xy.y, op, a.conics[3 * i]);
    a.splats[3 * (size_t)i + 1] = make_float4(a.conics[3 * i + 1], a.conics[3 * i + 2], c0, c1);
    a.splats[3 * (size_t)i + 2] =
        make_float4(c2, c3, __int_as_float(slot_base), __int_as_float(w | (b.minx << 16)));
}

}
```

### tinysplat_amd/csrc/project.hip

```cpp
#include <hip/hip_runtime.h>

#include "../../include/tinysplat_hip.h"
#include "host_util.h"
#include "pack.h"
#include "splat_math.h"
#include "adam_math.h"

namespace {

constexpr int kThreads = 256;
#ifndef TS_SH_THREADS_FWD
#define TS_SH_THREADS_FWD 128
#endif
#ifndef TS_SH_THREADS_BWD
#define TS_SH_THREADS_BWD 256
#endif
typedef float f4v __attribute__((ext_vector_type(4)));
__device__ __forceinline__ void store4(float4* p, float a, float b, float c, float d) {
    f4v v = {a, b, c, d};
    __builtin_nontemporal_store(v, reinterpret_cast<f4v*>(p));
}
constexpr int kShThreadsFwd = TS_SH_THREADS_FWD, kShThreadsBwd = TS_SH_THREADS_BWD;
__device__ __forceinline__ float4 load4_stream(const float4* p) {
    const f4v v = __builtin_nontemporal_load(reinterpret_cast<const f4v*>(p));
    return make_float4(v.x, v.y, v.z, v.w);
}

#include "project_inputs.h"

__global__ __launch_bounds__(kThreads) void project_fwd_kernel(
    int n, const float* __restrict__ means3d, const float* __restrict__ scales,
    const float* __restrict__ quats, const float* __restrict__ viewmat,
    const float* __restrict__ projmat, const ts_camera cam, const int flags,
    float* __restrict__ xys, float* __restrict__ depths, int* __restrict__ radii,
    float* __restrict__ conics, int* __restrict__ num_tiles_hit, float* __restrict__ cov3d) {
    const int i = blockIdx.x * kThreads + threadIdx.x;
    if (i >= n) return;
    const ts::Cam C = load_cam(viewmat, projmat, cam);
    const float m[3] = {means3d[3 * i], means3d[3 * i + 1], means3d[3 * i + 2]};
    float s[3] = {scales[3 * i], scales[3 * i + 1], scales[3 * i + 2]};
    const float4 qv = reinterpret_cast<const float4*>(quats)[i];
    float q[4] = {qv.x, qv.y, qv.z, qv.w};
    prep_inputs(flags, s, q, nullptr);
    ts::ProjOut o;
    ts::project_one(C, m, s, q, o);
    reinterpret_cast<float2*>(xys)[i] = make_float2(o.x, o.y);
    depths[i] = o.depth;
    radii[i] = o.radius;
    conics[3 * i] = o.conic[0]; conics[3 * i + 1] = o.conic[1]; conics[3 * i + 2] = o.conic[2];
    num_tiles_hit[i] = o.tiles;
    if (cov3d) {
        float2* c3 = reinterpret_cast<float2*>(cov3d) + 3 * (size_t)i;
        c3[0] = make_float2(o.cov3d[0], o.cov3d[1]);
        c3[1] = make_float2(o.cov3d[2], o.cov3d[3]);
        c3[2] = make_float2(o.cov3d[4], o.cov3d[5]);
    }
}

struct ProjAdam {
    float *means, *scales, *quats, *opacities;
    const float* v_opacity;
    float *m_means, *v_means, *m_scales, *v_scales, *m_quats, *v_quats, *m_opac, *v_opac;
    ts::AdamCoef c_means, c_scales, c_quats, c_opac;
};
template <bool ADAM>
__global__ __launch_bounds__(kThreads) void project_bwd_kernel(
    int n, const float* __restrict__ means3d, const float* __restrict__ scales,
    const float* __restrict__ quats, const float* __restrict__ viewmat,
    const float* __restrict__ projmat, const ts_camera cam, const int flags,
    const int* __restrict__ radii, const float* __restrict__ v_xy, const float* __restrict__ v_depth,
    const float* __restrict__ v_conic, const float* __restrict__ v_cov3d,
    float* __restrict__ v_means3d, float* __restrict__ v_scales, float* __restrict__ v_quats, const ProjAdam ad) {
    const int i = blockIdx.x * kThreads + threadIdx.x;
    if (i >= n) return;
    ts::ProjGrad g;
    for (int k = 0; k < 3; ++k) { g.v_mean[k] = 0.0f; g.v_scale[k] = 0.0f; }
    for (int k = 0; k < 4; ++k) g.v_quat[k] = 0.0f;
    float pm[3] = {0.f, 0.f, 0.f}, ps[3] = {0.f, 0.f, 0.f}, pq[4] = {0.f, 0.f, 0.f, 0.f};
    if (ADAM) {
        pm[0] = means3d[3 * i]; pm[1] = means3d[3 * i + 1]; pm[2] = means3d[3 * i + 2];
        ps[0] = scales[3 * i]; ps[1] = scales[3 * i + 1]; ps[2] = scales[3 * i + 2];
        const float4 qv = reinterpret_cast<const float4*>(quats)[i];
        pq[0] = qv.x; pq[1] = qv.y; pq[2] = qv.z; pq[3] = qv.w;
    }
    if (radii[i] > 0) {
        const ts::Cam C = load_cam(viewmat, projmat, cam);
        const float m[3] = {ADAM ? pm[0] : means3d[3 * i], ADAM ? pm[1] : means3d[3 * i + 1], ADAM ? pm[2] : means3d[3 * i + 2]};
        float s[3] = {ADAM ? ps[0] : scales[3 * i], ADAM ? ps[1] : scales[3 * i + 1], ADAM ? ps[2] : scales[3 * i + 2]};
        float4 qv;
        if (ADAM) qv = make_float4(pq[0], pq[1], pq[2], pq[3]);
        else qv = reinterpret_cast<const float4*>(quats)[i];
        float q[4] = {qv.x, qv.y, qv.z, qv.w};
        float inv_n = 1.0f;
        prep_inputs(flags, s, q, &inv_n);
        const float2 vxy = reinterpret_cast<const float2*>(v_xy)[i];
        const float vx[2] = {vxy.x, vxy.y};
        const float vc[3] = {v_conic[3 * i], v_conic[3 * i + 1], v_conic[3 * i + 2]};
        float vcov[6];
        if (v_cov3d) {
            for (int k = 0; k < 6; ++k) vcov[k] = v_cov3d[6 * (size_t)i + k];
        }
        ts::project_one_vjp(C, m, s, q, vx, v_depth ? v_depth[i] : 0.0f, vc, v_cov3d ? vcov : nullptr, g);
        if (flags & TS_PROJECT_LOG_SCALES) {
            g.v_scale[0] *= s[0]; g.v_scale[1] *= s[1]; g.v_scale[2] *= s[2];
        }
        if (flags & TS_PROJECT_RAW_QUATS) {
            const float dotp = q[0] * g.v_quat[0] + q[1] * g.v_quat[1] + q[2] * g.v_quat[2] +
                               q[3] * g.v_quat[3];
            for (int k = 0; k < 4; ++k) g.v_quat[k] = (g.v_quat[k] - q[k] * dotp) * inv_n;
        }
    }
    if (ADAM) {
        float mo[3], vo[3];
#pragma unroll
        for (int k = 0; k < 3; ++k) { mo[k] = ad.m_means[3 * i + k]; vo[k] = ad.v_means[3 * i + k]; }
#pragma unroll
        for (int k = 0; k < 3; ++k) {
            ts::adam_update(pm[k], g.v_mean[k], mo[k], vo[k], ad.c_means);
            ad.means[3 * i + k] = pm[k]; ad.m_means[3 * i + k] = mo[k]; ad.v_means[3 * i + k] = vo[k];
        }
#pragma unroll
        for (int k = 0; k < 3; ++k) { mo[k] = ad.m_scales[3 * i + k]; vo[k] = ad.v_scales[3 * i + k]; }
#pragma unroll
        for (int k = 0; k < 3; ++k) {
            ts::adam_update(ps[k], g.v_scale[k], mo[k], vo[k], ad.c_scales);
            ad.scales[3 * i + k] = ps[k]; ad.m_scales[3 * i + k] = mo[k]; ad.v_scales[3 * i + k] = vo[k];
        }
        float4 mq = reinterpret_cast<float4*>(ad.m_quats)[i], vq = reinterpret_cast<float4*>(ad.v_quats)[i];
        ts::adam_update(pq[0], g.v_quat[0], mq.x, vq.x, ad.c_quats); ts::adam_update(pq[1], g.v_quat[1], mq.y, vq.y, ad.c_quats);
        ts::adam_update(pq[2], g.v_quat[2], mq.z, vq.z, ad.c_quats); ts::adam_update(pq[3], g.v_quat[3], mq.w, vq.w, ad.c_quats);
        reinterpret_cast<float4*>(ad.quats)[i] = make_float4(pq[0], pq[1], pq[2], pq[3]);
        reinterpret_cast<float4*>(ad.m_quats)[i] = mq;
        reinterpret_cast<float4*>(ad.v_quats)[i] = vq;
        if (ad.opacities) {
            float po = ad.opacities[i], mo1 = ad.m_opac[i], vo1 = ad.v_opac[i];
            ts::adam_update(po, ad.v_opacity[i], mo1, vo1, ad.c_opac);
            ad.opacities[i] = po; ad.m_opac[i] = mo1; ad.v_opac[i] = vo1;
        }
        return;
    }
    v_means3d[3 * i] = g.v_mean[0]; v_means3d[3 * i + 1] = g.v_mean[1];
    v_means3d[3 * i + 2] = g.v_mean[2];
    v_scales[3 * i] = g.v_scale[0]; v_scales[3 * i + 1] = g.v_scale[1];
    v_scales[3 * i + 2] = g.v_scale[2];
    reinterpret_cast<float4*>(v_quats)[i] =
        make_float4(g.v_quat[0], g.v_quat[1], g.v_quat[2], g.v_quat[3]);
}

template <int DEG>
__global__ __launch_bounds__(kThreads) void sh_fwd_kernel(
    int n, int num_bases, const float* __restrict__ viewdirs, const float* __restrict__ coeffs,
    float* __restrict__ colors) {
    constexpr int KA = (DEG + 1) * (DEG + 1);
    constexpr int RS = 3 * KA;
    constexpr int RSP = RS | 1;
    extern __shared__ __align__(16) float lds[];
    const int g0 = blockIdx.x * kThreads;
    const int cnt = min(kThreads, n - g0);
    const int tid = threadIdx.x;
    const size_t row = 3 * (size_t)num_bases;
    const float* src = coeffs + (size_t)g0 * row;
    if (num_bases == KA && cnt == kThreads) {
        const float4* src4 = reinterpret_cast<const float4*>(src);
        constexpr int total4 = kThreads * RS / 4;
        for (int f4 = tid; f4 < total4; f4 += kThreads) {
            const float4 v = src4[f4];
            const int f = 4 * f4;
            const float e[4] = {v.x, v.y, v.z, v.w};
#pragma unroll
            for (int u = 0; u < 4; ++u) {
                const int ff = f + u;
                lds[(ff / RS) * RSP + (ff % RS)] = e[u];
            }
        }
    } else {
        const int total = cnt * RS;
        for (int f = tid; f < total; f += kThreads) {
            const int g = f / RS, j = f % RS;
            lds[g * RSP + j] = src[(size_t)g * row + j];
        }
    }
    __syncthreads();
    if (tid >= cnt) return;
    const int i = g0 + tid;
    float Y[KA];
    ts::sh_basis(DEG, viewdirs[3 * i], viewdirs[3 * i + 1], viewdirs[3 * i + 2], Y);
    const float* r = lds + tid * RSP;
    float c0 = Y[0] * r[0], c1 = Y[0] * r[1], c2 = Y[0] * r[2];
#pragma unroll
    for (int k = 1; k < KA; ++k) {
        c0 = c0 + Y[k] * r[3 * k];
        c1 = c1 + Y[k] * r[3 * k + 1];
        c2 = c2 + Y[k] * r[3 * k + 2];
    }
    colors[3 * i] = c0; colors[3 * i + 1] = c1; colors[3 * i + 2] = c2;
}

template <int DEG>
__global__ __launch_bounds__(kThreads) void sh_bwd_kernel(
    int n, int num_bases, const float* __restrict__ viewdirs, const float* __restrict__ v_colors,
    float* __restrict__ v_coeffs) {
    constexpr int KA = (DEG + 1) * (DEG + 1);
    extern __shared__ __align__(16) float lds[];
    const int RS = 3 * num_bases;
    const int RSP = RS | 1;
    const int g0 = blockIdx.x * kThreads;
    const int cnt = min(kThreads, n - g0);
    const int tid = threadIdx.x;
    if (tid < cnt) {
        const int i = g0 + tid;
        float Y[KA];
        ts::sh_basis(DEG, viewdirs[3 * i], viewdirs[3 * i + 1], viewdirs[3 * i + 2], Y);
        const float v0 = v_colors[3 * i], v1 = v_colors[3 * i + 1], v2 = v_colors[3 * i + 2];
        float* r = lds + tid * RSP;
#pragma unroll
        for (int k = 0; k < KA; ++k) {
            r[3 * k] = Y[k] * v0; r[3 * k + 1] = Y[k] * v1; r[3 * k + 2] = Y[k] * v2;
        }
        for (int j = 3 * KA; j < RS; ++j) r[j] = 0.0f;
    }
    __syncthreads();
    float* dst = v_coeffs + (size_t)g0 * RS;
    const int total = cnt * RS;
    if ((total & 3) == 0) {
        float4* dst4 = reinterpret_cast<float4*>(dst);
        for (int f4 = tid; f4 < total / 4; f4 += kThreads) {
            float e[4];
#pragma unroll
            for (int u = 0; u < 4; ++u) {
                const int ff = 4 * f4 + u;
                e[u] = lds[(ff / RS) * RSP + (ff % RS)];
            }
            dst4[f4] = make_float4(e[0], e[1], e[2], e[3]);
        }
    } else {
        for (int f = tid; f < total; f += kThreads) dst[f] = lds[(f / RS) * RSP + (f % RS)];
    }
}

template <int DEG>
__global__ __launch_bounds__(kShThreadsFwd) void sh_colors_fwd_kernel(
    int n, int num_bases, const float* __restrict__ means, const float* __restrict__ origin,
    const float* __restrict__ dc, const float* __restrict__ rest, float* __restrict__ colors,
    unsigned char* __restrict__ mask, const ts::PackArgs pk) {
    constexpr int KA = (DEG + 1) * (DEG + 1);
    constexpr int RS = 3 * (KA - 1);
    constexpr int RSP = RS | 1;
    extern __shared__ __align__(16) float lds[];
    const int g0 = blockIdx.x * kShThreadsFwd;
    const int cnt = min(kShThreadsFwd, n - g0);
    const int tid = threadIdx.x;
    if (RS > 0) {
        const size_t row = 3 * (size_t)(num_bases - 1);
        const float* src = rest + (size_t)g0 * row;
        if (num_bases == KA && cnt == kShThreadsFwd && ((kShThreadsFwd * RS) & 3) == 0) {
            const float4* src4 = reinterpret_cast<const float4*>(src);
            constexpr int total4 = kShThreadsFwd * RS / 4;
            constexpr int per = (total4 + kShThreadsFwd - 1) / kShThreadsFwd;
            float4 v[per > 0 ? per : 1];
#pragma unroll
            for (int u = 0; u < per; ++u) {
                const int f4 = tid + u * kShThreadsFwd;
                v[u] = f4 < total4 ? load4_stream(src4 + f4) : make_float4(0.f, 0.f, 0.f, 0.f);
            }
#pragma unroll
            for (int u = 0; u < per; ++u) {
                const int f4 = tid + u * kShThreadsFwd;
                if (f4 < total4) {
                    const float e[4] = {v[u].x, v[u].y, v[u].z, v[u].w};
#pragma unroll
                    for (int c = 0; c < 4; ++c) {
                        const int ff = 4 * f4 + c;
                        lds[(ff / RS) * RSP + (ff % RS)] = e[c];
                    }
                }
            }
        } else {
            const int total = cnt * RS;
            for (int f = tid; f < total; f += kShThreadsFwd) {
                const int g = f / RS, j = f % RS;
                lds[g * RSP + j] = src[(size_t)g * row + j];
            }
        }
        __syncthreads();
    }
    if (tid >= cnt) return;
    const int i = g0 + tid;
    float Y[KA];
    ts::sh_basis(DEG, means[3 * i] - origin[0], means[3 * i + 1] - origin[1],
                 means[3 * i + 2] - origin[2], Y);
    float c0 = Y[0] * dc[3 * i], c1 = Y[0] * dc[3 * i + 1], c2 = Y[0] * dc[3 * i + 2];
    const float* r = lds + tid * RSP;
#pragma unroll
    for (int k = 1; k < KA; ++k) {
        c0 = c0 + Y[k] * r[3 * (k - 1)];
        c1 = c1 + Y[k] * r[3 * (k - 1) + 1];
        c2 = c2 + Y[k] * r[3 * (k - 1) + 2];
    }
    c0 = c0 + 0.5f; c1 = c1 + 0.5f; c2 = c2 + 0.5f;
    if (mask) mask[i] = (unsigned char)((c0 >= 0.0f ? 1 : 0) | (c1 >= 0.0f ? 2 : 0) | (c2 >= 0.0f ? 4 : 0));
    c0 = fmaxf(c0, 0.0f); c1 = fmaxf(c1, 0.0f); c2 = fmaxf(c2, 0.0f);
    if (colors) { colors[3 * i] = c0; colors[3 * i + 1] = c1; colors[3 * i + 2] = c2; }
    if (pk.splats) ts::pack_one(pk, i, c0, c1, c2, pk.channels == 4 ? pk.depths[i] : 0.0f);
}

template <int DEG>
__global__ __launch_bounds__(kThreads) void sh_colors_fwd_sparse_kernel(
    int n, int num_bases, const int* __restrict__ live, const float* __restrict__ means,
    const float* __restrict__ origin, const float* __restrict__ dc, const float* __restrict__ rest,
    float* __restrict__ colors, unsigned char* __restrict__ mask, const ts::PackArgs pk) {
    constexpr int KA = (DEG + 1) * (DEG + 1);
    const int i = blockIdx.x * kThreads + threadIdx.x;
    if (i >= n || live[i] == 0) return;
    float Y[KA];
    ts::sh_basis(DEG, means[3 * i] - origin[0], means[3 * i + 1] - origin[1],
                 means[3 * i + 2] - origin[2], Y);
    float c0 = Y[0] * dc[3 * i], c1 = Y[0] * dc[3 * i + 1], c2 = Y[0] * dc[3 * i + 2];
    const float* r = rest + (size_t)i * 3 * (num_bases - 1);
#pragma unroll
    for (int k = 1; k < KA; ++k) {
        c0 = c0 + Y[k] * r[3 * (k - 1)];
        c1 = c1 + Y[k] * r[3 * (k - 1) + 1];
        c2 = c2 + Y[k] * r[3 * (k - 1) + 2];
    }
    c0 = c0 + 0.5f; c1 = c1 + 0.5f; c2 = c2 + 0.5f;
    if (mask) mask[i] = (unsigned char)((c0 >= 0.0f ? 1 : 0) | (c1 >= 0.0f ? 2 : 0) | (c2 >= 0.0f ? 4 : 0));
    c0 = fmaxf(c0, 0.0f); c1 = fmaxf(c1, 0.0f); c2 = fmaxf(c2, 0.0f);
    if (colors) { colors[3 * i] = c0; colors[3 * i + 1] = c1; colors[3 * i + 2] = c2; }
    if (pk.splats) ts::pack_one(pk, i, c0, c1, c2, pk.channels == 4 ? pk.depths[i] : 0.0f);
}

struct ShAdam {
    float *dc, *rest, *m_dc, *v_dc, *m_rest, *v_rest;
    ts::AdamCoef c_dc, c_rest;
};
template <int DEG, bool ADAM>
__global__ __launch_bounds__(kShThreadsBwd) void sh_colors_bwd_kernel(
    int n, int num_bases, const float* __restrict__ means, const float* __restrict__ origin,
    const unsigned char* __restrict__ mask, const float* __restrict__ v_colors,
    float* __restrict__ v_dc, float* __restrict__ v_rest, const ShAdam ad) {
    constexpr int KA = (DEG + 1) * (DEG + 1);
    extern __shared__ __align__(16) float lds[];
    const int RS = 3 * (num_bases - 1);
    const int RSP = RS | 1;
    const int g0 = blockIdx.x * kShThreadsBwd;
    const int cnt = min(kShThreadsBwd, n - g0);
    const int tid = threadIdx.x;
    if (tid < cnt) {
        const int i = g0 + tid;
        float Y[KA];
        ts::sh_basis(DEG, means[3 * i] - origin[0], means[3 * i + 1] - origin[1],
                     means[3 * i + 2] - origin[2], Y);
        const int m = mask ? mask[i] : 7;
        const float v0 = (m & 1) ? v_colors[3 * i] : 0.0f, v1 = (m & 2) ? v_colors[3 * i + 1] : 0.0f,
                    v2 = (m & 4) ? v_colors[3 * i + 2] : 0.0f;
        if (ADAM) {
            const float gd[3] = {Y[0] * v0, Y[0] * v1, Y[0] * v2};
#pragma unroll
            for (int c = 0; c < 3; ++c) {
                float p_ = ad.dc[3 * i + c], m_ = ad.m_dc[3 * i + c], s_ = ad.v_dc[3 * i + c];
                ts::adam_update(p_, gd[c], m_, s_, ad.c_dc);
                ad.dc[3 * i + c] = p_; ad.m_dc[3 * i + c] = m_; ad.v_dc[3 * i + c] = s_;
            }
        } else {
            v_dc[3 * i] = Y[0] * v0; v_dc[3 * i + 1] = Y[0] * v1; v_dc[3 * i + 2] = Y[0] * v2;
        }
        float* r = lds + tid * RSP;
#pragma unroll
        for (int k = 1; k < KA; ++k) {
            r[3 * (k - 1)] = Y[k] * v0; r[3 * (k - 1) + 1] = Y[k] * v1; r[3 * (k - 1) + 2] = Y[k] * v2;
        }
        for (int j = 3 * (KA - 1); j < RS; ++j) r[j] = 0.0f;
    }
    if (RS == 0) return;
    __syncthreads();
    const size_t off = (size_t)g0 * RS;
    float* dst = ADAM ? nullptr : v_rest + off;
    const int total = cnt * RS;
    if ((total & 3) == 0 && ((off) & 3) == 0) {
        float4* dst4 = reinterpret_cast<float4*>(dst);
        for (int f4 = tid; f4 < total / 4; f4 += kShThreadsBwd) {
            float e[4];
#pragma unroll
            for (int u = 0; u < 4; ++u) {
                const int ff = 4 * f4 + u;
                e[u] = lds[(ff / RS) * RSP + (ff % RS)];
            }
            if (ADAM) {
                float4* p4 = reinterpret_cast<float4*>(ad.rest + off) + f4;
                float4* m4 = reinterpret_cast<float4*>(ad.m_rest + off) + f4;
                float4* s4 = reinterpret_cast<float4*>(ad.v_rest + off) + f4;
                float4 pp = *p4, mm = *m4, ss = *s4;
                ts::adam_update(pp.x, e[0], mm.x, ss.x, ad.c_rest); ts::adam_update(pp.y, e[1], mm.y, ss.y, ad.c_rest);
                ts::adam_update(pp.z, e[2], mm.z, ss.z, ad.c_rest); ts::adam_update(pp.w, e[3], mm.w, ss.w, ad.c_rest);
                *p4 = pp; *m4 = mm; *s4 = ss;
            } else {
                store4(dst4 + f4, e[0], e[1], e[2], e[3]);
            }
        }
    } else {
        for (int f = tid; f < total; f += kShThreadsBwd) {
            const float e = lds[(f / RS) * RSP + (f % RS)];
            if (ADAM) {
                float p_ = ad.rest[off + f], m_ = ad.m_rest[off + f], s_ = ad.v_rest[off + f];
                ts::adam_update(p_, e, m_, s_, ad.c_rest);
                ad.rest[off + f] = p_; ad.m_rest[off + f] = m_; ad.v_rest[off + f] = s_;
            } else {
                dst[f] = e;
            }
        }
    }
}

__global__ __launch_bounds__(kThreads) void stream_read_kernel(const float4* __restrict__ src,
                                                               size_t n16, float* __restrict__ sink) {
    constexpr int U = 8;
    const size_t stride = (size_t)gridDim.x * kThreads;
    size_t i = (size_t)blockIdx.x * kThreads + threadIdx.x;
    float4 acc[U];
#pragma unroll
    for (int u = 0; u < U; ++u) acc[u] = make_float4(0.f, 0.f, 0.f, 0.f);
    for (; i + (U - 1) * stride < n16; i += U * stride) {
        float4 v[U];
#pragma unroll
        for (int u = 0; u < U; ++u) {
            const f4v t = __builtin_nontemporal_load(reinterpret_cast<const f4v*>(src + i + u * stride));
            v[u] = make_float4(t.x, t.y, t.z, t.w);
        }
#pragma unroll
        for (int u = 0; u < U; ++u) {
            acc[u].x += v[u].x; acc[u].y += v[u].y; acc[u].z += v[u].z; acc[u].w += v[u].w;
        }
    }
    for (; i < n16; i += stride) {
        const float4 v0 = src[i];
        acc[0].x += v0.x; acc[0].y += v0.y; acc[0].z += v0.z; acc[0].w += v0.w;
    }
    float t = 0.f;
#pragma unroll
    for (int u = 0; u < U; ++u) t += (acc[u].x + acc[u].y) + (acc[u].z + acc[u].w);
    if (t == 123456.789f) sink[0] = t;
}

__global__ __launch_bounds__(kThreads) void gather48_kernel(const float4* __restrict__ records,
                                                            const int* __restrict__ ids, size_t m,
                                                            float* __restrict__ sink) {
    const size_t stride = (size_t)gridDim.x * kThreads;
    float4 a = make_float4(0.f, 0.f, 0.f, 0.f);
    for (size_t j = (size_t)blockIdx.x * kThreads + threadIdx.x; j < m; j += stride) {
        const size_t g = (size_t)ids[j];
        const float4 q0 = records[3 * g], q1 = records[3 * g + 1], q2 = records[3 * g + 2];
        a.x += q0.x + q1.x + q2.x; a.y += q0.y + q1.y + q2.y; a.z += q0.z + q1.z + q2.z; a.w += q0.w + q1.w + q2.w;
    }
    if ((a.x + a.y) + (a.z + a.w) == 123456.789f) sink[0] = a.x;
}

}

extern "C" {

int ts_abi_version(void) { return TS_ABI_VERSION; }

int ts_project_fwd(int32_t n, const float* means3d, const float* scales, const float* quats,
                   const float* viewmat, const float* projmat, const ts_camera* cam,
                   int32_t flags, float* xys, float* depths, int32_t* radii, float* conics,
                   int32_t* num_tiles_hit, float* cov3d, void* stream) {
    if (n < 0 || !cam) return TS_E_BADARG;
    if (n == 0) return 0;
    if (!means3d || !scales || !quats || !viewmat || !projmat || !xys || !depths || !radii ||
        !conics || !num_tiles_hit)
        return TS_E_BADARG;
    const int grid = (n + kThreads - 1) / kThreads;
    hipLaunchKernelGGL(project_fwd_kernel, dim3(grid), dim3(kThreads), 0, (hipStream_t)stream, n,
                       means3d, scales, quats, viewmat, projmat, *cam, (int)flags, xys, depths, radii,
                       conics, num_tiles_hit, cov3d);
    return launch_status();
}

int ts_project_bwd(int32_t n, const float* means3d, const float* scales, const float* quats,
                   const float* viewmat, const float* projmat, const ts_camera* cam,
                   int32_t flags, const int32_t* radii, const float* v_xy, const float* v_depth,
                   const float* v_conic, const float* v_cov3d, float* v_means3d, float* v_scales,
                   float* v_quats, void* stream) {
    if (n < 0 || !cam) return TS_E_BADARG;
    if (n == 0) return 0;
    if (!means3d || !scales || !quats || !viewmat || !projmat || !radii || !v_xy ||
        !v_conic || !v_means3d || !v_scales || !v_quats)
        return TS_E_BADARG;
    const int grid = (n + kThreads - 1) / kThreads;
    hipLaunchKernelGGL(project_bwd_kernel<false>, dim3(grid), dim3(kThreads), 0, (hipStream_t)stream, n,
                       means3d, scales, quats, viewmat, projmat, *cam, (int)flags, radii, v_xy, v_depth,
                       v_conic, v_cov3d, v_means3d, v_scales, v_quats, ProjAdam{});
    return launch_status();
}

static bool adam_group_ok(const ts_adam* a, int k) {
    return a->exp_avg[k] && a->exp_avg_sq[k] && a->step[k] >= 1;
}

int ts_project_bwd_adam(int32_t n, float* means3d, float* scales, float* quats, const float* viewmat,
                        const float* projmat, const ts_camera* cam, int32_t flags, const int32_t* radii,
                        const float* v_xy, const float* v_depth, const float* v_conic, float* opacities,
                        const float* v_opacity, const ts_adam* adam, void* stream) {
    if (n < 0 || !cam || !adam) return TS_E_BADARG;
    if (n == 0) return 0;
    if (!means3d || !scales || !quats || !viewmat || !projmat || !radii || !v_xy || !v_conic) return TS_E_BADARG;
    if (!adam_group_ok(adam, TS_ADAM_MEANS) || !adam_group_ok(adam, TS_ADAM_SCALES) || !adam_group_ok(adam, TS_ADAM_QUATS))
        return TS_E_BADARG;
    if (opacities && (!v_opacity || !adam_group_ok(adam, TS_ADAM_OPACITIES))) return TS_E_BADARG;
    ProjAdam ad{};
    ad.means = means3d; ad.scales = scales; ad.quats = quats; ad.opacities = opacities; ad.v_opacity = v_opacity;
    ad.m_means = adam->exp_avg[TS_ADAM_MEANS]; ad.v_means = adam->exp_avg_sq[TS_ADAM_MEANS];
    ad.m_scales = adam->exp_avg[TS_ADAM_SCALES]; ad.v_scales = adam->exp_avg_sq[TS_ADAM_SCALES];
    ad.m_quats = adam->exp_avg[TS_ADAM_QUATS]; ad.v_quats = adam->exp_avg_sq[TS_ADAM_QUATS];
    ad.m_opac = adam->exp_avg[TS_ADAM_OPACITIES]; ad.v_opac = adam->exp_avg_sq[TS_ADAM_OPACITIES];
    auto coef = [&](int k) { return ts::adam_coef(adam->lr[k], adam->step[k], adam->beta1, adam->beta2, adam->eps); };
    ad.c_means = coef(TS_ADAM_MEANS); ad.c_scales = coef(TS_ADAM_SCALES); ad.c_quats = coef(TS_ADAM_QUATS);
    if (opacities) ad.c_opac = coef(TS_ADAM_OPACITIES);
    const int grid = (n + kThreads - 1) / kThreads;
    hipLaunchKernelGGL(project_bwd_kernel<true>, dim3(grid), dim3(kThreads), 0, (hipStream_t)stream, n,
                       means3d, scales, quats, viewmat, projmat, *cam, (int)flags, radii, v_xy, v_depth,
                       v_conic, (const float*)nullptr, (float*)nullptr, (float*)nullptr, (float*)nullptr, ad);
    return launch_status();
}

static int sh_check(int32_t n, int32_t degree, int32_t num_bases) {
    if (n < 0) return TS_E_BADARG;
    if (num_bases != 1 && num_bases != 4 && num_bases != 9 && num_bases != 16 && num_bases != 25)
        return TS_E_DEGREE;
    if (degree < 0 || degree > 4 || (degree + 1) * (degree + 1) > num_bases) return TS_E_DEGREE;
    return 0;
}

int ts_sh_fwd(int32_t n, int32_t degrees_to_use, int32_t num_bases, const float* viewdirs,
              const float* coeffs, float* colors, void* stream) {
    const int chk = sh_check(n, degrees_to_use, num_bases);
    if (chk) return chk;
    if (n == 0) return 0;
    if (!viewdirs || !coeffs || !colors) return TS_E_BADARG;
    const int grid = (n + kThreads - 1) / kThreads;
    const int ka = (degrees_to_use + 1) * (degrees_to_use + 1);
    const size_t lds = (size_t)kThreads * ((3 * ka) | 1) * sizeof(float);
    hipStream_t s = (hipStream_t)stream;
#define TS_SH_FWD(D)                                                                          \
    hipLaunchKernelGGL(sh_fwd_kernel<D>, dim3(grid), dim3(kThreads), lds, s, n, num_bases,     \
                       viewdirs, coeffs, colors)
    switch (degrees_to_use) {
        case 0: TS_SH_FWD(0); break;
        case 1: TS_SH_FWD(1); break;
        case 2: TS_SH_FWD(2); break;
        case 3: TS_SH_FWD(3); break;
        default: {
            (void)hipFuncSetAttribute(reinterpret_cast<const void*>(&sh_fwd_kernel<4>),
                                hipFuncAttributeMaxDynamicSharedMemorySize, (int)lds);
            TS_SH_FWD(4);
        } break;
    }
#undef TS_SH_FWD
    return launch_status();
}

int ts_sh_bwd(int32_t n, int32_t degrees_to_use, int32_t num_bases, const float* viewdirs,
              const float* v_colors, float* v_coeffs, void* stream) {
    const int chk = sh_check(n, degrees_to_use, num_bases);
    if (chk) return chk;
    if (n == 0) return 0;
    if (!viewdirs || !v_colors || !v_coeffs) return TS_E_BADARG;
    const int grid = (n + kThreads - 1) / kThreads;
    const size_t lds = (size_t)kThreads * ((3 * num_bases) | 1) * sizeof(float);
    hipStream_t s = (hipStream_t)stream;
#define TS_SH_BWD(D)                                                                          \
    do {                                                                                      \
        if (lds > 48 * 1024)                                                                  \
            (void)hipFuncSetAttribute(reinterpret_cast<const void*>(&sh_bwd_kernel<D>),           \
                                hipFuncAttributeMaxDynamicSharedMemorySize, (int)lds);        \
        hipLaunchKernelGGL(sh_bwd_kernel<D>, dim3(grid), dim3(kThreads), lds, s, n, num_bases, \
                           viewdirs, v_colors, v_coeffs);                                     \
    } while (0)
    switch (degrees_to_use) {
        case 0: TS_SH_BWD(0); break;
        case 1: TS_SH_BWD(1); break;
        case 2: TS_SH_BWD(2); break;
        case 3: TS_SH_BWD(3); break;
        default: TS_SH_BWD(4); break;
    }
#undef TS_SH_BWD
    return launch_status();
}

static int launch_colors_fwd(int32_t n, int32_t degrees_to_use, int32_t num_bases, const float* means3d,
                             const float* origin, const float* colors_dc, const float* colors_rest,
                             float* colors, uint8_t* clamp_mask, const int32_t* live, const ts::PackArgs& pk,
                             void* stream) {
    const int chk = sh_check(n, degrees_to_use, num_bases);
    if (chk) return chk;
    if (n == 0) return 0;
    if (!means3d || !origin || !colors_dc || (!colors && !pk.splats) || (num_bases > 1 && !colors_rest))
        return TS_E_BADARG;
    const int grid = (n + kThreads - 1) / kThreads;
    hipStream_t s = (hipStream_t)stream;
    if (live) {
#define TS_SHC_SPARSE(D)                                                                           \
        hipLaunchKernelGGL(sh_colors_fwd_sparse_kernel<D>, dim3(grid), dim3(kThreads), 0, s, n,    \
                           num_bases, live, means3d, origin, colors_dc, colors_rest, colors, clamp_mask, pk)
        switch (degrees_to_use) {
            case 0: TS_SHC_SPARSE(0); break;
            case 1: TS_SHC_SPARSE(1); break;
            case 2: TS_SHC_SPARSE(2); break;
            case 3: TS_SHC_SPARSE(3); break;
            default: TS_SHC_SPARSE(4); break;
        }
#undef TS_SHC_SPARSE
        return launch_status();
    }
    const int ka = (degrees_to_use + 1) * (degrees_to_use + 1);
    const size_t lds = (size_t)kShThreadsFwd * ((3 * (ka - 1)) | 1) * sizeof(float);
    const int grid_d = (n + kShThreadsFwd - 1) / kShThreadsFwd;
#define TS_SHC_FWD(D)                                                                             \
    do {                                                                                          \
        if (lds > 48 * 1024)                                                                      \
            (void)hipFuncSetAttribute(reinterpret_cast<const void*>(&sh_colors_fwd_kernel<D>),    \
                                      hipFuncAttributeMaxDynamicSharedMemorySize, (int)lds);      \
        hipLaunchKernelGGL(sh_colors_fwd_kernel<D>, dim3(grid_d), dim3(kShThreadsFwd), lds, s, n,  \
                           num_bases, means3d, origin, colors_dc, colors_rest, colors, clamp_mask, pk); \
    } while (0)
    switch (degrees_to_use) {
        case 0: TS_SHC_FWD(0); break;
        case 1: TS_SHC_FWD(1); break;
        case 2: TS_SHC_FWD(2); break;
        case 3: TS_SHC_FWD(3); break;
        default: TS_SHC_FWD(4); break;
    }
#undef TS_SHC_FWD
    return launch_status();
}

int ts_sh_colors_fwd(int32_t n, int32_t degrees_to_use, int32_t num_bases, const float* means3d,
                     const float* origin, const float* colors_dc, const float* colors_rest,
                     float* colors, uint8_t* clamp_mask, const int32_t* live, void* stream) {
    ts::PackArgs none;
    none.splats = nullptr;
    if (!colors) return TS_E_BADARG;
    return launch_colors_fwd(n, degrees_to_use, num_bases, means3d, origin, colors_dc, colors_rest, colors,
                             clamp_mask, live, none, stream);
}

int ts_colors_pack_fwd(int32_t n, int32_t degrees_to_use, int32_t num_bases, const float* means3d,
                       const float* origin, const float* colors_dc, const float* colors_rest,
                       uint8_t* clamp_mask, const int32_t* live, int32_t channels, int32_t flags,
                       const float* xys, const int32_t* radii, const float* conics, const float* opacity,
                       const int32_t* cum_tiles_hit, const ts_camera* cam, const float* depths,
                       float* splats, void* stream) {
    if (n < 0 || !cam || (channels != 3 && channels != 4)) return TS_E_BADARG;
    if (n > 0 && (!xys || !radii || !conics || !opacity || !cum_tiles_hit || !splats ||
                  (channels == 4 && !depths)))
        return TS_E_BADARG;
    ts::PackArgs pk;
    pk.channels = channels; pk.flags = (int)flags; pk.xys = xys; pk.radii = radii; pk.conics = conics;
    pk.opacity = opacity; pk.cum_tiles_hit = cum_tiles_hit; pk.depths = depths;
    pk.splats = reinterpret_cast<float4*>(splats); pk.cam = *cam;
    return launch_colors_fwd(n, degrees_to_use, num_bases, means3d, origin, colors_dc, colors_rest, nullptr,
                             clamp_mask, live, pk, stream);
}

static int sh_colors_bwd_launch(int32_t n, int32_t degrees_to_use, int32_t num_bases, const float* means3d,
                                const float* origin, const uint8_t* clamp_mask, const float* v_colors,
                                float* v_colors_dc, float* v_colors_rest, const ShAdam* ad, void* stream) {
    const int grid = (n + kShThreadsBwd - 1) / kShThreadsBwd;
    const size_t lds = (size_t)kShThreadsBwd * ((3 * (num_bases - 1)) | 1) * sizeof(float);
    hipStream_t s = (hipStream_t)stream;
#define TS_SHC_BWD2(D, A)                                                                            \
    do {                                                                                             \
        if (lds > 48 * 1024)                                                                         \
            (void)hipFuncSetAttribute(reinterpret_cast<const void*>(&sh_colors_bwd_kernel<D, A>),    \
                                      hipFuncAttributeMaxDynamicSharedMemorySize, (int)lds);         \
        hipLaunchKernelGGL((sh_colors_bwd_kernel<D, A>), dim3(grid), dim3(kShThreadsBwd), lds, s, n, \
                           num_bases, means3d, origin, clamp_mask, v_colors, v_colors_dc,            \
                           v_colors_rest, ad ? *ad : ShAdam{});                                      \
    } while (0)
#define TS_SHC_BWD(D)                                       \
    do {                                                    \
        if (ad) TS_SHC_BWD2(D, true);                       \
        else TS_SHC_BWD2(D, false);                         \
    } while (0)
    switch (degrees_to_use) {
        case 0: TS_SHC_BWD(0); break;
        case 1: TS_SHC_BWD(1); break;
        case 2: TS_SHC_BWD(2); break;
        case 3: TS_SHC_BWD(3); break;
        default: TS_SHC_BWD(4); break;
    }
#undef TS_SHC_BWD
#undef TS_SHC_BWD2
    return launch_status();
}

int ts_sh_colors_bwd(int32_t n, int32_t degrees_to_use, int32_t num_bases, const float* means3d,
                     const float* origin, const uint8_t* clamp_mask, const float* v_colors,
                     float* v_colors_dc, float* v_colors_rest, void* stream) {
    const int chk = sh_check(n, degrees_to_use, num_bases);
    if (chk) return chk;
    if (n == 0) return 0;
    if (!means3d || !origin || !v_colors || !v_colors_dc || (num_bases > 1 && !v_colors_rest))
        return TS_E_BADARG;
    return sh_colors_bwd_launch(n, degrees_to_use, num_bases, means3d, origin, clamp_mask, v_colors, v_colors_dc,
                                v_colors_rest, nullptr, stream);
}

int ts_sh_colors_bwd_adam(int32_t n, int32_t degrees_to_use, int32_t num_bases, const float* means3d,
                          const float* origin, const uint8_t* clamp_mask, const float* v_colors,
                          float* colors_dc, float* colors_rest, const ts_adam* adam, void* stream) {
    const int chk = sh_check(n, degrees_to_use, num_bases);
    if (chk) return chk;
    if (n == 0) return 0;
    if (!adam || !means3d || !origin || !v_colors || !colors_dc || (num_bases > 1 && !colors_rest)) return TS_E_BADARG;
    if (!adam_group_ok(adam, TS_ADAM_COLORS_DC) || (num_bases > 1 && !adam_group_ok(adam, TS_ADAM_COLORS_REST)))
        return TS_E_BADARG;
    ShAdam ad{};
    ad.dc = colors_dc; ad.rest = colors_rest;
    ad.m_dc = adam->exp_avg[TS_ADAM_COLORS_DC]; ad.v_dc = adam->exp_avg_sq[TS_ADAM_COLORS_DC];
    ad.m_rest = adam->exp_avg[TS_ADAM_COLORS_REST]; ad.v_rest = adam->exp_avg_sq[TS_ADAM_COLORS_REST];
    ad.c_dc = ts::adam_coef(adam->lr[TS_ADAM_COLORS_DC], adam->step[TS_ADAM_COLORS_DC], adam->beta1, adam->beta2, adam->eps);
    if (num_bases > 1)
        ad.c_rest = ts::adam_coef(adam->lr[TS_ADAM_COLORS_REST], adam->step[TS_ADAM_COLORS_REST], adam->beta1, adam->beta2,
                                  adam->eps);
    return sh_colors_bwd_launch(n, degrees_to_use, num_bases, means3d, origin, clamp_mask, v_colors, nullptr, nullptr, &ad,
                                stream);
}

int ts_bench_gather48(const float* records, const int32_t* ids, int64_t m, float* sink, void* stream) {
    if (!records || !ids || !sink || m < 1) return TS_E_BADARG;
    hipLaunchKernelGGL(gather48_kernel, dim3(256 * 8), dim3(kThreads), 0, (hipStream_t)stream,
                       reinterpret_cast<const float4*>(records), ids, (size_t)m, sink);
    return launch_status();
}

int ts_bench_stream_read(const float* src, int64_t n_floats, float* sink, void* stream) {
    if (!src || !sink || n_floats < 4) return TS_E_BADARG;
    const size_t n16 = (size_t)n_floats / 4;
    hipLaunchKernelGGL(stream_read_kernel, dim3(256 * 8), dim3(kThreads), 0, (hipStream_t)stream,
                       reinterpret_cast<const float4*>(src), n16, sink);
    return launch_status();
}

}
```

### tinysplat_amd/frame.py

```python
from __future__ import annotations

import ctypes
import os
import threading
from typing import Optional, Tuple

import torch
import torch.distributed as dist
from torch import Tensor

from ._comm import collective_timer
from . import _lib
from ._lib import TsFrame
from .ops import TileBinning, _camera, _f32c, _need_hip, _stream, _stripe_rows, _tile_bounds, deg_from_sh

TIGHT_BINNING = os.environ.get("TS_TIGHT_BINNING", "1") != "0"

SPLIT_BLOCKS_BELOW = int(os.environ.get("TS_SPLIT_BLOCKS_BELOW", "2400"))

_ls = os.environ.get("TS_LIST_SEGMENTS", "auto")
LIST_SEGMENTS = _ls if _ls == "auto" else max(1, min(8, int(_ls)))
LIST_SEGMENTS_FROM = int(os.environ.get("TS_LIST_SEGMENTS_FROM", "192"))
SEGMENT_ITEMS = int(os.environ.get("TS_SEGMENT_ITEMS", "16384"))


HYBRID_FROM = int(os.environ.get("TS_HYBRID_FROM", "4096"))
HYBRID_SEGS = max(1, min(8, int(os.environ.get("TS_HYBRID_SEGS", "8"))))
HYBRID_WHOLE16 = max(1, min(15, int(os.environ.get("TS_HYBRID_WHOLE16", "13"))))
HYBRID_MID_FROM = int(os.environ.get("TS_HYBRID_MID_FROM", "1537"))
HYBRID_MID_WHOLE16 = max(1, min(15, int(os.environ.get("TS_HYBRID_MID_WHOLE16", "6"))))
HYBRID_MID_COOP16 = max(0, min(15, int(os.environ.get("TS_HYBRID_MID_COOP16", "6"))))
HYBRID_COOP16 = max(0, min(15, int(os.environ.get("TS_HYBRID_COOP16", "3"))))
COOP_SPLIT = os.environ.get("TS_COOP_SPLIT", "1") != "0"


def set_launch_hints(cam, segs: int, w16: int, mode: int, split: bool, skewed: bool = False) -> None:
    cam.hints = (cam.hints & ~0x1FFF00) | (((segs << 8) | (w16 << 12)) if segs > 1 else 0)
    tiles16 = cam.tile_rows * cam.tile_bounds_x
    if mode == 0 and not split and tiles16 >= HYBRID_FROM:
        cam.hints |= (HYBRID_MID_COOP16 if skewed else HYBRID_COOP16) << 16
    elif mode == 0 and not split and tiles16 >= HYBRID_MID_FROM:
        cam.hints |= HYBRID_MID_COOP16 << 16
    if mode == 0 and split and COOP_SPLIT:
        cam.hints |= _lib.HINT_COOP_SPLIT


def _list_segments(tiles16: int, mode: int, split: bool, skewed: bool = False):
    if mode != 0 or tiles16 <= 0:
        return 1, 0
    if not split:
        if HYBRID_SEGS > 1 and tiles16 >= HYBRID_FROM:
            return HYBRID_SEGS, (HYBRID_MID_WHOLE16 if skewed else HYBRID_WHOLE16)
        if HYBRID_SEGS > 1 and tiles16 >= HYBRID_MID_FROM:
            return HYBRID_SEGS, HYBRID_MID_WHOLE16
        return 1, 0
    if LIST_SEGMENTS != "auto":
        return int(LIST_SEGMENTS), 0
    return max(2, min(8, SEGMENT_ITEMS // tiles16)), 0


last_segments = {}


def segments_for_count(cam, segs: int, total: int) -> int:
    if segs > 1 and total >= LIST_SEGMENTS_FROM * cam.tile_rows * cam.tile_bounds_x:
        return segs
    cam.hints &= ~0xFF00
    return 1


def backward_segments(cam, segs: int, total: int, dev_index: int = 0) -> int:
    segs = segments_for_count(cam, segs, total)
    last_segments[dev_index] = segs
    return segs

_wt = os.environ.get("TS_WIDE_TILES", "auto")
WIDE_TILES = _wt if _wt == "auto" else int(_wt)
WIDE_LISTS_FROM = int(os.environ.get("TS_WIDE_LISTS_FROM", "2300"))
BALANCED_WALK_FROM = float(os.environ.get("TS_BALANCED_WALK_FROM", "10"))
_pairs_per_tile = {}


MANY_TILES_FROM = int(os.environ.get("TS_MANY_TILES_FROM", "20000"))
LONG_LIST = int(os.environ.get("TS_LONG_LIST", "2048"))
SKEW_FROM = float(os.environ.get("TS_SKEW_FROM", "4"))
_stats_mode = {}
_longest_list = {}


def _list_mode(dev_index: int, tiles16: int) -> int:
    if WIDE_TILES != "auto":
        return int(WIDE_TILES)
    prev = _pairs_per_tile.get(dev_index)
    if prev is None:
        return 2 if tiles16 >= MANY_TILES_FROM else 0
    if prev >= WIDE_LISTS_FROM:
        return 2
    st = _longest_list.get(dev_index)
    if tiles16 >= MANY_TILES_FROM and st is not None:
        longest, mode = st
        return 2 if longest < (2 * LONG_LIST if mode == 2 else LONG_LIST) else 0
    return 0


def _skewed(dev_index: int, mode: int) -> bool:
    st, prev = _longest_list.get(dev_index), _pairs_per_tile.get(dev_index)
    if WIDE_TILES != "auto" or mode != 0 or st is None or prev is None or st[1] != 0:
        return False
    return st[0] >= SKEW_FROM * max(prev, 1.0)

last_binning = {}

TRACE = None


def _mark(label):
    if TRACE is not None:
        import time
        TRACE.append((label, time.perf_counter()))


_layouts = {}
_pinned_total = {}
_row_flags = {}
_row_flags_lock = threading.Lock()
_row_flags_tick = [0]

FLAG_GENERATIONS = os.environ.get("TS_FLAG_GENERATIONS", "1") != "0"


FLAGS_SHRINK_AFTER = 256


def row_flags_for(dev: torch.device, rows: int):
    if not FLAG_GENERATIONS:
        return torch.empty((rows,), dtype=torch.uint8, device=dev), 0
    key = (dev.index, _stream(dev))
    with _row_flags_lock:
        slot = _row_flags.get(key)
        if slot is not None and slot[0].numel() > 8 * max(rows, 1 << 20):
            slot[2] += 1
            if slot[2] >= FLAGS_SHRINK_AFTER:
                slot = None
        elif slot is not None:
            slot[2] = 0
        if slot is None or slot[0].numel() < rows:
            if key not in _row_flags and len(_row_flags) >= 32:
                _row_flags.pop(min(_row_flags, key=lambda k_: _row_flags[k_][3]))
            slot = _row_flags[key] = [torch.zeros((int(rows * 1.25) + 4096,), dtype=torch.uint8, device=dev), 0, 0, 0]
        _row_flags_tick[0] += 1
        slot[3] = _row_flags_tick[0]
        slot[1] += 1
        if slot[1] > 255:
            slot[0].zero_()
            slot[1] = 1
        return slot[0], slot[1]

_bg_cache = {}

STRIPE_SPARSE = os.environ.get("TS_STRIPE_SPARSE", "1") != "0"

TWO_HOP_SCATTER = os.environ.get("TS_TWO_HOP_SCATTER", "1") != "0"
INLINE_SORT = os.environ.get("TS_INLINE_SORT", "1") != "0"

DIRECT_GRADS = os.environ.get("TS_DIRECT_GRADS", "1") != "0"

SURVIVORS = os.environ.get("TS_SURVIVORS", "1") != "0"

GROUP_COUNTS = os.environ.get("TS_GROUP_COUNTS", "1") != "0"

ONE_WALK = os.environ.get("TS_ONE_WALK", "1") != "0"

CAPACITY_ALLOC = os.environ.get("TS_CAPACITY_ALLOC", "0") != "0"
CAPACITY_GROWTH = 1.25
_capacity = {}

COUNT_WAIT = os.environ.get("TS_COUNT_WAIT", "spin")
_SPIN_LIMIT = 50_000_000


def alloc_quantum(count: int) -> int:
    count = max(int(count), 1)
    if count <= 65536:
        return 65536
    g = 1 << (count.bit_length() - 4)
    return (count + g - 1) // g * g


def _total_slot(dev: torch.device):
    slot = _pinned_total.get(dev.index)
    if slot is None:
        slot = (torch.zeros((4,), dtype=torch.int32, pin_memory=True), torch.cuda.Event(), threading.Lock())
        _pinned_total[dev.index] = slot
    return slot


class _Frame:
    __slots__ = ("fr", "cam", "n", "nb", "ch", "w", "h", "num_tiles", "total", "split", "segs", "keep",
                 "wf", "tile_bins", "ids", "bucket_ids", "out_img", "out_depth", "planes", "xys", "radii", "nth", "cum",
                 "inputs", "bg")


def _forward(means, scales, quats, opacities, colors_dc, colors_rest, view34, projview, origin, background,
             fx, fy, width, height, sh_degree, with_depth, tile_rows, keep: bool, planes: bool = False) -> _Frame:
    _mark("fwd:enter")
    dev = _need_hip(means, scales, quats, opacities, colors_dc, colors_rest, view34, projview, origin, background)
    n = means.shape[0]
    nb = colors_rest.shape[1] + 1
    if sh_degree < 0 or sh_degree > deg_from_sh(nb):
        raise ValueError("sh_degree exceeds the stored coefficients")
    means, scales, quats = _f32c(means), _f32c(scales), _f32c(quats)
    opacities, colors_dc, colors_rest = _f32c(opacities), _f32c(colors_dc), _f32c(colors_rest)
    view34, projview, origin = _f32c(view34), _f32c(projview), _f32c(origin)
    w, h = int(width), int(height)
    cam = _camera(fx, fy, w / 2, h / 2, h, w, _tile_bounds(h, w), 1.0, tile_rows=tile_rows)
    slot_ = _pinned_total.get(dev.index)
    if slot_ is not None and dev.index in _stats_mode:
        _longest_list[dev.index] = (int(ctypes.c_int32.from_address(slot_[0].data_ptr() + 4).value), _stats_mode[dev.index])
    mode = _list_mode(dev.index, cam.tile_rows * cam.tile_bounds_x)
    cam.wide_tiles = 1 if mode else 0
    prev_i = _pairs_per_tile.get(dev.index)
    if prev_i is not None and n > 0 and prev_i * cam.tile_rows * cam.tile_bounds_x >= BALANCED_WALK_FROM * n:
        cam.hints = _lib.HINT_BALANCED_WALK
    ch = 4 if with_depth else 3
    if with_depth:
        key = (background.data_ptr(), background._version, dev.index)
        hit = _bg_cache.get(key)
        if hit is None:
            if len(_bg_cache) > 16:
                _bg_cache.clear()
            hit = _bg_cache[key] = (_f32c(torch.cat([background, background[:1]])), background)
        bg = hit[0]
    else:
        bg = _f32c(background)
    lib = _lib.load()
    s = _stream(dev)
    F = _Frame()
    F.cam, F.n, F.nb, F.ch, F.w, F.h, F.keep = cam, n, nb, ch, w, h, keep
    F.inputs = (means, scales, quats, opacities, colors_dc, colors_rest, view34, projview, origin)
    F.bg = bg
    num_tiles = int(lib.ts_num_tiles(ctypes.byref(cam)))
    F.num_tiles = num_tiles
    F.split = 0 < cam.tile_rows * cam.tile_bounds_x <= SPLIT_BLOCKS_BELOW
    rows = _stripe_rows(cam)
    m = max(n, 1)
    skewed = _skewed(dev.index, mode)
    segs, w16 = _list_segments(cam.tile_rows * cam.tile_bounds_x, mode, F.split, skewed) if keep else (1, 0)
    set_launch_hints(cam, segs, w16, mode, F.split, skewed)
    F.segs = segs
    _mark("fwd:inputs checked")
    cur = torch.cuda.current_device()
    if cur != dev.index:
        torch.cuda.set_device(dev)
    try:
        f32 = dict(dtype=torch.float32, device=dev)
        i32 = dict(dtype=torch.int32, device=dev)
        px = rows * w
        lkey = (n, num_tiles, w, rows, ch, keep, cam.hints & 0xFFFF00, cam.wide_tiles, cam.tile_rows, cam.tile_row0, cam.tile_bounds_x, cam.img_height)
        lay = _layouts.get(lkey)
        if lay is None:
            nscan = int(lib.ts_scan_ws_ints(n))
            nbin = int(lib.ts_bin_ws_ints(n, num_tiles))
            fin_floats = int(lib.ts_final_floats(ctypes.byref(cam), ch)) if keep else px
            sizes = [48 * m, 8 * m, 12 * m, 0, 4 * m, 4 * m, 4 * m, 4 * m, 4 * nscan, 4 * nbin,
                     8 * max(num_tiles, 1)] + ([m, 4 * fin_floats, 4 * px, px] if keep else [])
            offs, off = [], 0
            for sz in sizes:
                offs.append(off)
                off += (sz + 255) & ~255
            if len(_layouts) > 64:
                _layouts.clear()
            lay = _layouts[lkey] = (offs, off)
        offs, off = lay
        _mark("fwd:sizes")
        F.wf = torch.empty((off,), dtype=torch.uint8, device=dev)
        _mark("fwd:workspace allocated")
        base = F.wf.data_ptr()
        ptr = [base + o for o in offs]
        F.planes = bool(planes and with_depth)
        F.out_img = torch.empty((rows, w, 3 if F.planes else ch), **f32)
        F.out_depth = torch.empty((rows, w), **f32) if F.planes else None
        _mark("fwd:image allocated")

        def view(k, dtype, count, shape):
            return F.wf[offs[k]:offs[k] + count * dtype.itemsize].view(dtype).view(shape)
        F.xys = view(1, torch.float32, 2 * n, (n, 2))
        F.radii = view(5, torch.int32, n, (n,))
        F.nth = view(6, torch.int32, n, (n,))
        F.cum = view(7, torch.int32, n, (n,))
        F.tile_bins = view(10, torch.int32, 2 * max(num_tiles, 1), (max(num_tiles, 1), 2))
        host, event, count_lock = _total_slot(dev)
        fr = TsFrame()
        fr.n, fr.num_bases, fr.sh_degree, fr.channels = n, nb, int(sh_degree), ch
        stripe = STRIPE_SPARSE and cam.tile_rows < cam.tile_bounds_y
        full = cam.tile_rows == cam.tile_bounds_y
        fr.flags = ((1 if TIGHT_BINNING else 0) | (2 if F.split else 0) | (8 if mode == 2 else 0) | (16 if stripe else 0)
                    | (0 if TWO_HOP_SCATTER else 32) | (64 if F.planes else 0) | (0 if INLINE_SORT else 128)
                    | (256 if full else 0))
        surv = SURVIVORS and keep and full and mode == 0 and not F.split and INLINE_SORT
        if surv:
            fr.flags |= 512
        if GROUP_COUNTS:
            fr.flags |= 1024
        if ONE_WALK:
            fr.flags |= 2048
        if full:
            _stats_mode[dev.index] = mode
        fr.cam = cam
        fr.means, fr.scales, fr.quats, fr.opacities = means.data_ptr(), scales.data_ptr(), quats.data_ptr(), opacities.data_ptr()
        fr.colors_dc, fr.colors_rest = colors_dc.data_ptr(), colors_rest.data_ptr()
        fr.view34, fr.projview, fr.origin, fr.background = view34.data_ptr(), projview.data_ptr(), origin.data_ptr(), bg.data_ptr()
        fr.splats, fr.xys, fr.conics, fr.depths = ptr[0], ptr[1], ptr[2], ptr[4]
        fr.radii, fr.num_tiles_hit, fr.cum_tiles_hit, fr.scan_ws = ptr[5], ptr[6], ptr[7], ptr[8]
        fr.bin_ws, fr.tile_bins = ptr[9], ptr[10]
        fr.total_host = host.data_ptr()
        fr.out_img = F.out_img.data_ptr()
        if F.planes:
            fr.out_depth = F.out_depth.data_ptr()
        if keep:
            fr.sh_mask, fr.final_Ts, fr.final_index, fr.clamp_mask = ptr[11], ptr[12], ptr[13], ptr[14]
        F.fr = fr
        _mark("fwd:allocated + struct")
        spin = COUNT_WAIT == "spin" and n > 0
        cap_key = (dev.index, n, w, h, cam.tile_row0, cam.tile_rows)
        est = _capacity.get(cap_key) if (CAPACITY_ALLOC and n > 0) else None

        def lists(size):
            cap = alloc_quantum(size)
            counts = (8 * num_tiles + 63) // 64 * 64 if surv else 0
            F.bucket_ids = torch.empty(((3 * cap + counts) if surv else 2 * cap,), **i32)
            fr.bucket_ids, fr.gaussian_ids_sorted = F.bucket_ids.data_ptr(), F.bucket_ids.data_ptr() + 4 * cap
            if surv:
                fr.survivors = F.bucket_ids.data_ptr() + 8 * cap
            return cap

        def prepare():
            _lib.check(lib.ts_frame_fwd_prepare(ctypes.byref(fr), s), "ts_frame_fwd_prepare")

        def composite():
            _lib.check(lib.ts_frame_fwd_composite(ctypes.byref(fr), s), "ts_frame_fwd_composite")

        count_lock.acquire()
        issued = consumed = False
        try:
            if spin:
                word = ctypes.c_int32.from_address(host.data_ptr())
                word.value = -(1 << 31)
            _lib.check(lib.ts_frame_fwd_project(ctypes.byref(fr), s), "ts_frame_fwd_project")
            issued = n > 0
            _mark("fwd:call project")
            event.record()
            cap = None
            if est is not None:
                cap = lists(est)
                fr.capacity, fr.num_intersects = cap, cap
                prepare()
                composite()
            else:
                fr.capacity = -1
                prepare()
            _mark("fwd:call prepare")
            total = 0
            if n > 0:
                if spin:
                    k = 0
                    while word.value == -(1 << 31):
                        k += 1
                        if k > _SPIN_LIMIT:
                            event.synchronize()
                            break
                    total = int(word.value)
                else:
                    event.synchronize()
                    total = int(host[0])
            consumed = True
        finally:
            if issued and not consumed:
                try:
                    event.synchronize()
                except Exception:
                    pass
            count_lock.release()
        if total < 0:
            raise OverflowError("more than 2^31-1 tile intersections: num_tiles_hit overflows its "
                                "int32 prefix sum (gsplat's cum_tiles_hit is int32 as well)")
        _mark("fwd:waited for count")
        F.total = total
        _pairs_per_tile[dev.index] = total / max(1, cam.tile_rows * cam.tile_bounds_x)
        if n > 0 and CAPACITY_ALLOC:
            if len(_capacity) > 64:
                _capacity.clear()
            _capacity[cap_key] = int(total * CAPACITY_GROWTH) + 4096
        if cap is None or total > cap:
            redo = cap is not None
            cap = lists(total)
            _mark("fwd:lists allocated")
            fr.capacity, fr.num_intersects = -1, total
            F.segs = segments_for_count(fr.cam, F.segs, total)
            if redo:
                prepare()
            composite()
            _mark("fwd:composite enqueued")
        else:
            fr.num_intersects = total
        F.ids = F.bucket_ids[cap:cap + total]
        _mark("fwd:call composite")
    finally:
        if cur != dev.index:
            torch.cuda.set_device(cur)
    b = TileBinning()
    b.cam, b.n, b.num_tiles, b.num_intersects = cam, n, num_tiles, total
    b.tile_bins, b.gaussian_ids_sorted, b.cum_tiles_hit, b.num_tiles_hit = F.tile_bins[:num_tiles], F.ids, F.cum, F.nth
    last_binning[dev.index] = b
    _mark("fwd:exit")
    return F


class _AdamHook:
    opt = None


_adam_hook = _AdamHook()


class fused_adam:
    def __init__(self, optimizer):
        self.optimizer = optimizer

    def __enter__(self):
        self.prev = getattr(_adam_hook, "opt", None)
        _adam_hook.opt = self.optimizer
        return self

    def __exit__(self, *exc):
        _adam_hook.opt = self.prev
        return False


class _RenderFrame(torch.autograd.Function):
    @staticmethod
    def forward(ctx, means, scales, quats, opacities, colors_dc, colors_rest, view34, projview,
                origin, background, fx, fy, width, height, sh_degree, with_depth, tile_rows, group, planes=False):
        F = _forward(means, scales, quats, opacities, colors_dc, colors_rest, view34, projview, origin,
                     background, fx, fy, width, height, sh_degree, with_depth, tile_rows, keep=True, planes=planes)
        ctx.frame, ctx.group = F, group
        ctx.opacity_shape = opacities.shape
        ctx.rest_shape = colors_rest.shape
        xys, radii = F.xys, F.radii
        ctx.xys_out = xys
        ctx.mark_non_differentiable(xys, radii)
        ctx.set_materialize_grads(False)
        out, F.out_img = F.out_img, None
        depth, F.out_depth = F.out_depth, None
        return out, depth, xys, radii

    @staticmethod
    def backward(ctx, v_img, v_depth_img, _v_xys, _v_radii):
        _mark("bwd:enter")
        F = ctx.frame
        if F is None:
            raise RuntimeError("the frame's buffers were released by an earlier backward pass")
        fr, n, ch = F.fr, F.n, F.ch
        dev = F.wf.device
        f32 = dict(dtype=torch.float32, device=dev)
        lib = _lib.load()
        s = _stream(dev)
        if F.planes:
            v_img = None if v_img is None else _f32c(v_img)
            v_depth_img = None if v_depth_img is None else _f32c(v_depth_img)
        else:
            if v_img is None:
                v_img = torch.zeros((F.cam.tile_rows and _stripe_rows(F.cam), F.w, ch), dtype=torch.float32, device=dev)
            v_img = _f32c(v_img)
        _mark("bwd:v_img contiguous")
        with torch.cuda.device(dev):
            _mark("bwd:device ctx")
            single = ctx.group is None and DIRECT_GRADS
            flat = torch.empty((n * ((3 + ch) if single else (6 + ch)),), **f32)
            if single:
                v_xy = torch.empty((n, 2), **f32)
                v_opac = torch.empty(tuple(ctx.opacity_shape), **f32)
            F.segs = backward_segments(fr.cam, F.segs, F.total, dev.index)
            rows = max(F.total, 1) * (4 if (F.split and F.segs <= 1) else 1)
            partials = torch.empty((alloc_quantum(rows), _lib.PARTIAL_ROW_FLOATS), **f32)
            row_flags, fr.flag_gen = row_flags_for(dev, rows)
            _mark("bwd:flat+partials+flags")
            opt = getattr(_adam_hook, "opt", None)
            adam = opt.fused_begin(F.inputs[:6]) if (opt is not None and single) else None
            if adam is None:
                v_means = torch.empty((n, 3), **f32)
                v_scales = torch.empty((n, 3), **f32)
                v_quats = torch.empty((n, 4), **f32)
                v_dc = torch.empty((n, 3), **f32)
                v_rest = torch.empty(tuple(ctx.rest_shape), **f32)
            p = flat.data_ptr()
            fr.v_out_img = None if v_img is None else v_img.data_ptr()
            fr.v_out_depth = None if (not F.planes or v_depth_img is None) else v_depth_img.data_ptr()
            fr.partials, fr.row_flags = partials.data_ptr(), row_flags.data_ptr()
            if single:
                fr.v_xy, fr.v_conic, fr.v_colors = v_xy.data_ptr(), p, p + 12 * n
                fr.v_depth = p + 24 * n if ch == 4 else None
                fr.v_opacity = v_opac.data_ptr()
            else:
                fr.v_xy, fr.v_conic, fr.v_colors = p, p + 8 * n, p + 20 * n
                fr.v_depth = p + 32 * n if ch == 4 else None
                fr.v_opacity = p + (20 + 4 * ch) * n
            if adam is None:
                fr.v_means, fr.v_scales, fr.v_quats = v_means.data_ptr(), v_scales.data_ptr(), v_quats.data_ptr()
                fr.v_colors_dc, fr.v_colors_rest = v_dc.data_ptr(), v_rest.data_ptr()
            _mark("bwd:allocated")
            _lib.check(lib.ts_frame_bwd_composite(ctypes.byref(fr), s), "ts_frame_bwd_composite")
            if ctx.group is not None:
                with collective_timer.span(on_device=flat.is_cuda and dist.get_backend(ctx.group) != "gloo",
                                           label="all_reduce(2-D gradients)", nbytes=flat.numel() * flat.element_size()):
                    dist.all_reduce(flat, op=dist.ReduceOp.SUM, group=ctx.group)
            if adam is not None:
                _lib.check(lib.ts_frame_bwd_params_adam(ctypes.byref(fr), ctypes.byref(adam), s),
                           "ts_frame_bwd_params_adam")
            else:
                _lib.check(lib.ts_frame_bwd_params(ctypes.byref(fr), s), "ts_frame_bwd_params")
        _mark("bwd:calls")
        if not single:
            v_xy = flat[:2 * n].view(n, 2).clone()
            v_opac = flat[(5 + ch) * n:].view(ctx.opacity_shape).clone()
        xo = ctx.xys_out
        xo.grad = v_xy if xo.grad is None else xo.grad + v_xy
        _mark("bwd:exit")
        if adam is not None:
            return (None,) * 19
        return (v_means, v_scales, v_quats, v_opac, v_dc, v_rest) + (None,) * 13


@torch.no_grad()
def render_view(model, view34: Tensor, projview: Tensor, origin: Tensor, fx: float, fy: float,
                width: int, height: int, with_depth: bool = True,
                tile_rows: Optional[Tuple[int, int]] = None, planes: bool = False):
    F = _forward(model.means.detach(), model.scales.detach(), model.quats.detach(), model.opacities.detach(),
                 model.colors_dc.detach(), model.colors_rest.detach(), view34, projview, origin,
                 model.background, fx, fy, width, height, int(model.active_sh_degree), with_depth, tile_rows,
                 keep=False, planes=planes)
    if F.planes:
        return F.out_img, F.out_depth, F.xys, F.radii
    return F.out_img, F.xys, F.radii


def render_frame(model, view34: Tensor, projview: Tensor, origin: Tensor, fx: float, fy: float,
                 width: int, height: int, with_depth: bool = True,
                 tile_rows: Optional[Tuple[int, int]] = None, group=None):
    out, _, xys, radii = _RenderFrame.apply(model.means, model.scales, model.quats, model.opacities,
                                            model.colors_dc, model.colors_rest, view34, projview, origin,
                                            model.background, fx, fy, width, height, model.active_sh_degree,
                                            with_depth, tile_rows, group, False)
    return out, xys, radii
# ... 9 lines not shown
```

Baseline: 2062000 billion Gaussians*pixels/s.

## Fuse tile-count prefix scan into projection and color-pack kernels; group sort launches

Projection now computes per-span local inclusive scans of tiles-hit and span sums in a 1024-thread variant. The color/pack kernel finishes the scan, writes cum_tiles_hit and the total to mapped host memory, which removes the separate scan launches. The host count event is moved to after prepare, so the host waits on more work before it can size the lists. Separately, the above-threshold sort launches one block per tile group and skips groups whose longest list is short, instead of launching one block per tile.

```diff
diff --git a/include/tinysplat_hip.h b/include/tinysplat_hip.h
--- a/include/tinysplat_hip.h
+++ b/include/tinysplat_hip.h
@@ -71,6 +71,17 @@
                        const float* xys, const int32_t* radii, const float* conics, const float* opacity,
                        const int32_t* cum_tiles_hit, const ts_camera* cam_host, const float* depths,
                        float* splats, void* stream);
+
+int ts_project_fwd_scan(int32_t n, const float* means3d, const float* scales, const float* quats,
+                        const float* viewmat, const float* projmat, const ts_camera* cam_host,
+                        int32_t flags, float* xys, float* depths, int32_t* radii, float* conics,
+                        int32_t* num_tiles_hit, int32_t* cum_tiles_hit, int32_t* scan_ws, void* stream);
+int ts_colors_pack_fwd_scan(int32_t n, int32_t degrees_to_use, int32_t num_bases, const float* means3d,
+                            const float* origin, const float* colors_dc, const float* colors_rest,
+                            uint8_t* clamp_mask, int32_t channels, int32_t flags, const float* xys,
+                            const int32_t* radii, const float* conics, const float* opacity,
+                            int32_t* cum_tiles_hit, const int32_t* scan_ws, int32_t* total_out,
+                            const ts_camera* cam_host, const float* depths, float* splats, void* stream);
 
 
 int64_t ts_scan_ws_ints(int32_t n);
@@ -122,6 +133,9 @@
 int ts_sort_tiles_above_stats(int32_t num_tiles, const int32_t* tile_bins, const float* depths,
                               const int32_t* bucket_ids, int32_t* gaussian_ids_sorted, int32_t n,
                               const int32_t* bin_ws, int32_t* longest_list, void* stream);
+int ts_sort_tiles_above_groups(int32_t num_tiles, const int32_t* tile_bins, const float* depths,
+                               const int32_t* bucket_ids, int32_t* gaussian_ids_sorted, int32_t n,
+                               const int32_t* bin_ws, int32_t* longest_list, void* stream);
 
 #define TS_RASTER_LOGIT_OPACITY 1
 
@@ -177,6 +191,7 @@
 #define TS_FRAME_GROUP_COUNTS 1024
 #define TS_FRAME_ONE_WALK 2048
 #define TS_FRAME_SURVIVORS 512
+#define TS_FRAME_FUSED_SCAN 4096
 typedef struct ts_frame {
     int32_t n, num_bases, sh_degree, channels, flags;
     int32_t flag_gen;
diff --git a/tinysplat_amd/_lib.py b/tinysplat_amd/_lib.py
--- a/tinysplat_amd/_lib.py
+++ b/tinysplat_amd/_lib.py
@@ -114,6 +114,10 @@
     "ts_cut_tiles": (c_int32, [_CAM, _P, _P]),
     "ts_colors_pack_fwd": (c_int32, [c_int32, c_int32, c_int32, _P, _P, _P, _P, _P, _P, c_int32, c_int32,
                                      _P, _P, _P, _P, _P, _CAM, _P, _P, _P]),
+    "ts_project_fwd_scan": (c_int32, [c_int32, _P, _P, _P, _P, _P, _CAM, c_int32, _P, _P, _P, _P, _P, _P, _P, _P]),
+    "ts_colors_pack_fwd_scan": (c_int32, [c_int32, c_int32, c_int32, _P, _P, _P, _P, _P, c_int32, c_int32,
+                                          _P, _P, _P, _P, _P, _P, _P, _CAM, _P, _P, _P]),
+    "ts_sort_tiles_above_groups": (c_int32, [c_int32, _P, _P, _P, _P, c_int32, _P, _P, _P]),
     "ts_pack_splats": (c_int32, [c_int32, c_int32, c_int32, _P, _P, _P, _P, _P, _P, _CAM, _P, _P, _P]),
     "ts_raster_fwd": (c_int32, [c_int32, c_int32, _CAM, _P, _P, _P, _P, _P, _P, _P, _P, _P]),
     "ts_raster_bwd": (c_int32, [c_int32, c_int32, c_int64, _CAM, _P, _P, _P, _P, _P, _P, _P, _P, _P, _P, _P, _P]),
diff --git a/tinysplat_amd/csrc/binning.hip b/tinysplat_amd/csrc/binning.hip
--- a/tinysplat_amd/csrc/binning.hip
+++ b/tinysplat_amd/csrc/binning.hip
@@ -3,6 +3,7 @@
 #include "../../include/tinysplat_hip.h"
 #include "host_util.h"
 #include "pack.h"
+#include "scan_util.h"
 #include "splat_math.h"
 
 namespace {
@@ -11,34 +12,8 @@
 constexpr int kScanItems = 4;
 constexpr int kScanBlock = kThreads * kScanItems;
 
-__device__ __forceinline__ int wave_inclusive_scan(int v) {
-    const int lane = threadIdx.x & 63;
-#pragma unroll
-    for (int d = 1; d < 64; d <<= 1) {
-        const int u = __shfl_up(v, d, 64);
-        if (lane >= d) v += u;
-    }
-    return v;
-}
-
-template <int WAVES = 4>
-__device__ __forceinline__ int block_inclusive_scan(int v, int* total) {
-    __shared__ int wave_sums[WAVES];
-    const int lane = threadIdx.x & 63, wave = threadIdx.x >> 6;
-    int inc = wave_inclusive_scan(v);
-    if (lane == 63) wave_sums[wave] = inc;
-    __syncthreads();
-    int add = 0, tot = 0;
-#pragma unroll
-    for (int w = 0; w < WAVES; ++w) {
-        const int s = wave_sums[w];
-        if (w < wave) add += s;
-        tot += s;
-    }
-    *total = tot;
-    __syncthreads();
-    return inc + add;
-}
+using ts::block_inclusive_scan;
+static_assert(kScanBlock == ts::kScanSpan, "ts_scan_tiles and the fused scan cut the Gaussians into the same spans");
 
 __global__ __launch_bounds__(kThreads) void scan_local_kernel(int n, const int* __restrict__ in,
                                                               int* __restrict__ out,
@@ -1186,16 +1161,24 @@
     }
 }
 
+template <bool GROUPS>
 __global__ __launch_bounds__(kThreads) void sort_tiles_above_kernel(
     const int* __restrict__ tile_bins, const float* __restrict__ depths,
-    const int* __restrict__ bucket_ids, int* __restrict__ ids_sorted, const ListStats stats) {
+    const int* __restrict__ bucket_ids, int* __restrict__ ids_sorted, int num_tiles,
+    const int* __restrict__ group_max, const ListStats stats) {
     __shared__ unsigned long long lds_u64[kLargeLdsU64 > kSortCap / 2 ? kLargeLdsU64 : kSortCap / 2];
     if (stats.group_max && blockIdx.x == 0) store_longest(stats);
-    const int2 range = reinterpret_cast<const int2*>(tile_bins)[blockIdx.x];
-    const int n = range.y - range.x;
-    if (n <= kWaveSortMax) return;
-    if (n <= kSortCap) sort_bucket_block(bucket_ids + range.x, depths, ids_sorted + range.x, n, lds_u64);
-    else sort_tile_sample(bucket_ids + range.x, depths, ids_sorted + range.x, n, lds_u64);
+    if (GROUPS && group_max[blockIdx.x] <= kWaveSortMax) return;
+    const int first = GROUPS ? (int)(blockIdx.x << kCoarseShift) : (int)blockIdx.x;
+    const int last = GROUPS ? min(num_tiles, first + kCoarseTiles) : first + 1;
+    for (int tile = first; tile < last; ++tile) {
+        const int2 range = reinterpret_cast<const int2*>(tile_bins)[tile];
+        const int n = range.y - range.x;
+        if (n <= kWaveSortMax) continue;
+        if (GROUPS) __syncthreads();
+        if (n <= kSortCap) sort_bucket_block(bucket_ids + range.x, depths, ids_sorted + range.x, n, lds_u64);
+        else sort_tile_sample(bucket_ids + range.x, depths, ids_sorted + range.x, n, lds_u64);
+    }
 }
 
 __global__ __launch_bounds__(kThreads) void pack_splats_kernel(int n, const ts::PackArgs a,
@@ -1490,8 +1473,22 @@
     if (!tile_bins || !depths || !bucket_ids || !gaussian_ids_sorted) return TS_E_BADARG;
     ListStats stats;
     if (!list_stats(n, num_tiles, bin_ws, longest_list, &stats)) return TS_E_BADARG;
-    hipLaunchKernelGGL(sort_tiles_above_kernel, dim3(num_tiles), dim3(kThreads), 0, (hipStream_t)stream, tile_bins,
-                       depths, bucket_ids, gaussian_ids_sorted, stats);
+    hipLaunchKernelGGL(sort_tiles_above_kernel<false>, dim3(num_tiles), dim3(kThreads), 0, (hipStream_t)stream, tile_bins,
+                       depths, bucket_ids, gaussian_ids_sorted, (int)num_tiles, (const int*)nullptr, stats);
+    return launch_status();
+}
+
+int ts_sort_tiles_above_groups(int32_t num_tiles, const int32_t* tile_bins, const float* depths,
+                               const int32_t* bucket_ids, int32_t* gaussian_ids_sorted, int32_t n,
+                               const int32_t* bin_ws, int32_t* longest_list, void* stream) {
+    if (num_tiles < 0 || !two_hop(n)) return TS_E_BADARG;
+    if (num_tiles == 0) return 0;
+    if (!tile_bins || !depths || !bucket_ids || !gaussian_ids_sorted || !bin_ws) return TS_E_BADARG;
+    ListStats stats;
+    if (!list_stats(n, num_tiles, bin_ws, longest_list, &stats)) return TS_E_BADARG;
+    const BinGeometry g = bin_geometry(n, num_tiles);
+    hipLaunchKernelGGL(sort_tiles_above_kernel<true>, dim3(g.groups), dim3(kThreads), 0, (hipStream_t)stream, tile_bins,
+                       depths, bucket_ids, gaussian_ids_sorted, (int)num_tiles, bin_ws + g.group_max, stats);
     return launch_status();
 }
 
diff --git a/tinysplat_amd/csrc/frame.hip b/tinysplat_amd/csrc/frame.hip
--- a/tinysplat_amd/csrc/frame.hip
+++ b/tinysplat_amd/csrc/frame.hip
@@ -104,6 +104,10 @@
     }
     return nullptr;
 }
+inline bool fused_scan(const ts_frame* f) {
+    if (!(f->flags & TS_FRAME_FUSED_SCAN) || (f->flags & TS_FRAME_STRIPE) || f->n <= 0) return false;
+    return !f->total_host || mapped_pointer(f->total_host) != nullptr;
+}
 inline int raster_flags(const ts_frame* f) {
     return TS_RASTER_CLAMP_RGB | ((f->flags & TS_FRAME_SPLIT) ? TS_RASTER_SPLIT_BLOCKS : 0) |
            ((f->flags & TS_FRAME_NARROW_WAVES) ? TS_RASTER_NARROW_WAVES : 0);
@@ -123,6 +127,13 @@
 int ts_frame_fwd_project(const ts_frame* f, void* stream) {
     TsRange range_("ts_frame_fwd_project");
     if (bad(f)) return TS_E_BADARG;
+    if (fused_scan(f)) {
+        TS_TRY(TS_ENTRY("ts_project_fwd",
+                        ts_project_fwd_scan(f->n, f->means, f->scales, f->quats, f->view34, f->projview, &f->cam, 3,
+                                            f->xys, f->depths, f->radii, f->conics, f->num_tiles_hit, f->cum_tiles_hit,
+                                            f->scan_ws, stream)));
+        return TS_ENTRY("ts_scan_tiles", 0);
+    }
     TS_TRY(TS_ENTRY("ts_project_fwd",
                     ts_project_fwd(f->n, f->means, f->scales, f->quats, f->view34, f->projview, &f->cam, 3, f->xys,
                                    f->depths, f->radii, f->conics, f->num_tiles_hit, nullptr, stream)));
@@ -140,13 +151,23 @@
 int ts_frame_fwd_prepare(const ts_frame* f, void* stream) {
     TsRange range_("ts_frame_fwd_prepare");
     if (bad(f)) return TS_E_BADARG;
-    TS_TRY(TS_ENTRY("ts_colors_pack_fwd",
-                    ts_colors_pack_fwd(f->n, f->sh_degree, f->num_bases, f->means, f->origin, f->colors_dc,
-                                       f->num_bases > 1 ? f->colors_rest : nullptr, f->sh_mask,
-                                       (f->flags & TS_FRAME_STRIPE) ? f->num_tiles_hit : nullptr, f->channels,
-                                       TS_RASTER_LOGIT_OPACITY, f->xys, f->radii, f->conics, f->opacities,
-                                       f->cum_tiles_hit, &f->cam, f->channels == 4 ? f->depths : nullptr, f->splats,
-                                       stream)));
+    if (fused_scan(f)) {
+        TS_TRY(TS_ENTRY("ts_colors_pack_fwd",
+                        ts_colors_pack_fwd_scan(f->n, f->sh_degree, f->num_bases, f->means, f->origin, f->colors_dc,
+                                                f->num_bases > 1 ? f->colors_rest : nullptr, f->sh_mask, f->channels,
+                                                TS_RASTER_LOGIT_OPACITY, f->xys, f->radii, f->conics, f->opacities,
+                                                f->cum_tiles_hit, f->scan_ws,
+                                                f->total_host ? mapped_pointer(f->total_host) : nullptr, &f->cam,
+                                                f->channels == 4 ? f->depths : nullptr, f->splats, stream)));
+    } else {
+        TS_TRY(TS_ENTRY("ts_colors_pack_fwd",
+                        ts_colors_pack_fwd(f->n, f->sh_degree, f->num_bases, f->means, f->origin, f->colors_dc,
+                                           f->num_bases > 1 ? f->colors_rest : nullptr, f->sh_mask,
+                                           (f->flags & TS_FRAME_STRIPE) ? f->num_tiles_hit : nullptr, f->channels,
+                                           TS_RASTER_LOGIT_OPACITY, f->xys, f->radii, f->conics, f->opacities,
+                                           f->cum_tiles_hit, &f->cam, f->channels == 4 ? f->depths : nullptr, f->splats,
+                                           stream)));
+    }
     const float* tight = tight_records(f);
     switch (list_form(f)) {
     case ListForm::one_walk:
@@ -208,7 +229,11 @@
     if (listed) {
         int32_t* counter = f->bin_ws + (ts_bin_ws_ints(f->n, num_tiles(f)) - 1);
         int32_t* longest = (form == ListForm::group || form == ListForm::one_walk) ? longest_word(f) : nullptr;
-        if (fused_sort)
+        if (fused_sort && (form == ListForm::group || form == ListForm::one_walk))
+            TS_TRY(TS_ENTRY("ts_sort_tiles",
+                            ts_sort_tiles_above_groups(num_tiles(f), f->tile_bins, f->depths, f->bucket_ids,
+                                                       f->gaussian_ids_sorted, f->n, f->bin_ws, longest, stream)));
+        else if (fused_sort)
             TS_TRY(TS_ENTRY("ts_sort_tiles",
                             ts_sort_tiles_above_stats(num_tiles(f), f->tile_bins, f->depths, f->bucket_ids,
                                                       f->gaussian_ids_sorted, f->n, f->bin_ws, longest, stream)));
diff --git a/tinysplat_amd/csrc/pack.h b/tinysplat_amd/csrc/pack.h
--- a/tinysplat_amd/csrc/pack.h
+++ b/tinysplat_amd/csrc/pack.h
@@ -19,7 +19,8 @@
     ts_camera cam;
 };
 
-__device__ __forceinline__ void pack_one(const PackArgs& a, int i, float c0, float c1, float c2, float c3) {
+__device__ __forceinline__ void pack_one(const PackArgs& a, int i, float c0, float c1, float c2, float c3,
+                                         const int* cum = nullptr) {
     const int r = a.radii[i];
     if (r <= 0) return;
     const float2 xy = reinterpret_cast<const float2*>(a.xys)[i];
@@ -28,7 +29,7 @@
     const int w = b.maxx - b.minx, h = b.maxy - b.miny;
     const int cnt = h > 0 ? w * h : 0;
     if (cnt <= 0) return;
-    const int excl = a.cum_tiles_hit[i] - cnt;
+    const int excl = (cum ? *cum : a.cum_tiles_hit[i]) - cnt;
     const int slot_base = excl - b.miny * w - b.minx;
     float op = a.opacity[i];
     if (a.flags & TS_RASTER_LOGIT_OPACITY) op = 1.0f / (1.0f + expf(-op));
diff --git a/tinysplat_amd/csrc/project.hip b/tinysplat_amd/csrc/project.hip
--- a/tinysplat_amd/csrc/project.hip
+++ b/tinysplat_amd/csrc/project.hip
@@ -3,6 +3,7 @@
 #include "../../include/tinysplat_hip.h"
 #include "host_util.h"
 #include "pack.h"
+#include "scan_util.h"
 #include "splat_math.h"
 #include "adam_math.h"
 
@@ -28,14 +29,12 @@
 
 #include "project_inputs.h"
 
-__global__ __launch_bounds__(kThreads) void project_fwd_kernel(
-    int n, const float* __restrict__ means3d, const float* __restrict__ scales,
+__device__ __forceinline__ int project_store(
+    int i, const float* __restrict__ means3d, const float* __restrict__ scales,
     const float* __restrict__ quats, const float* __restrict__ viewmat,
-    const float* __restrict__ projmat, const ts_camera cam, const int flags,
+    const float* __restrict__ projmat, const ts_camera& cam, const int flags,
     float* __restrict__ xys, float* __restrict__ depths, int* __restrict__ radii,
     float* __restrict__ conics, int* __restrict__ num_tiles_hit, float* __restrict__ cov3d) {
-    const int i = blockIdx.x * kThreads + threadIdx.x;
-    if (i >= n) return;
     const ts::Cam C = load_cam(viewmat, projmat, cam);
     const float m[3] = {means3d[3 * i], means3d[3 * i + 1], means3d[3 * i + 2]};
     float s[3] = {scales[3 * i], scales[3 * i + 1], scales[3 * i + 2]};
@@ -55,6 +54,59 @@
         c3[1] = make_float2(o.cov3d[2], o.cov3d[3]);
         c3[2] = make_float2(o.cov3d[4], o.cov3d[5]);
     }
+    return o.tiles;
+}
+
+constexpr int kScanThreads = 1024, kScanWaves = kScanThreads / 64;
+constexpr int kSpanRounds = ts::kScanSpan / kScanThreads;
+static_assert(kSpanRounds >= 1 && kSpanRounds * kScanThreads == ts::kScanSpan, "a span is a whole number of rounds");
+template <bool SCAN>
+__global__ __launch_bounds__(SCAN ? kScanThreads : kThreads) void project_fwd_kernel(
+    int n, const float* __restrict__ means3d, const float* __restrict__ scales,
+    const float* __restrict__ quats, const float* __restrict__ viewmat,
+    const float* __restrict__ projmat, const ts_camera cam, const int flags,
+    float* __restrict__ xys, float* __restrict__ depths, int* __restrict__ radii,
+    float* __restrict__ conics, int* __restrict__ num_tiles_hit, float* __restrict__ cov3d,
+    int* __restrict__ cum_local, int* __restrict__ span_sums) {
+    if (!SCAN) {
+        const int i = blockIdx.x * kThreads + threadIdx.x;
+        if (i >= n) return;
+        project_store(i, means3d, scales, quats, viewmat, projmat, cam, flags, xys, depths, radii, conics,
+                      num_tiles_hit, cov3d);
+        return;
+    }
+    __shared__ int wave_sums[kSpanRounds * kScanWaves];
+    const int lane = threadIdx.x & 63, wave = threadIdx.x >> 6;
+    int inc[kSpanRounds];
+#pragma unroll
+    for (int r = 0; r < kSpanRounds; ++r) {
+        const int i = blockIdx.x * ts::kScanSpan + r * kScanThreads + threadIdx.x;
+        int tiles = 0;
+        if (i < n)
+            tiles = project_store(i, means3d, scales, quats, viewmat, projmat, cam, flags, xys, depths, radii, conics,
+                                  num_tiles_hit, cov3d);
+        inc[r] = ts::wave_inclusive_scan(tiles);
+        if (lane == 63) wave_sums[r * kScanWaves + wave] = inc[r];
+    }
+    __syncthreads();
+    unsigned int before = 0, total = 0;
+#pragma unroll
+    for (int k = 0; k < kSpanRounds * kScanWaves; ++k) {
+        const unsigned int s = (unsigned int)wave_sums[k];
+        if (k == wave) before = total;
+        total += s;
+    }
+    unsigned int run = before;
+#pragma unroll
+    for (int r = 0; r < kSpanRounds; ++r) {
+        const int i = blockIdx.x * ts::kScanSpan + r * kScanThreads + threadIdx.x;
+        if (i < n) cum_local[i] = (int)(run + (unsigned int)inc[r]);
+        if (r + 1 < kSpanRounds) {
+#pragma unroll
+            for (int k = 0; k < kScanWaves; ++k) run += (unsigned int)wave_sums[r * kScanWaves + wave + k];
+        }
+    }
+    if (threadIdx.x == 0) span_sums[blockIdx.x] = (int)total;
 }
 
 struct ProjAdam {
@@ -238,11 +290,63 @@
     }
 }
 
-template <int DEG>
+struct ScanArgs {
+    int* cum;
+    const int* span_sums;
+    int* total_out;
+    int spans;
+};
+constexpr int kSpanLoads = 4;
+static_assert(ts::kScanSpan % kShThreadsFwd == 0, "a colour-stage workgroup must not straddle two spans");
+struct SpanBatch {
+    int4 v[kSpanLoads];
+    int tail[3];
+    unsigned int rest;
+};
+__device__ __forceinline__ int4 span_load4(const int* __restrict__ span_sums, int b, int count) {
+    int4 v = make_int4(0, 0, 0, 0);
+    if (b + 4 <= count) v = *reinterpret_cast<const int4*>(span_sums + b);
+    return v;
+}
+__device__ __forceinline__ unsigned int sum4(const int4& v) {
+    return ((unsigned int)v.x + (unsigned int)v.y) + ((unsigned int)v.z + (unsigned int)v.w);
+}
+__device__ __forceinline__ SpanBatch span_request(const int* __restrict__ span_sums, int count, int lane) {
+    SpanBatch b;
+#pragma unroll
+    for (int u = 0; u < kSpanLoads; ++u) b.v[u] = span_load4(span_sums, 4 * (u * 64 + lane), count);
+#pragma unroll
+    for (int k = 0; k < 3; ++k) {
+        const int j = (count & ~3) + k;
+        b.tail[k] = (lane == 0 && j < count) ? span_sums[j] : 0;
+    }
+    b.rest = 0;
+    for (int j0 = 4 * kSpanLoads * 64; j0 + 4 <= count; j0 += 4 * kSpanLoads * 64) {
+        int4 v[kSpanLoads];
+#pragma unroll
+        for (int u = 0; u < kSpanLoads; ++u) v[u] = span_load4(span_sums, j0 + 4 * (u * 64 + lane), count);
+#pragma unroll
+        for (int u = 0; u < kSpanLoads; ++u) b.rest += sum4(v[u]);
+    }
+    return b;
+}
+__device__ __forceinline__ unsigned int wave_sum(unsigned int v) {
+#pragma unroll
+    for (int d = 32; d >= 1; d >>= 1) v += __shfl_xor(v, d, 64);
+    return v;
+}
+__device__ __forceinline__ unsigned int span_sum(const SpanBatch& b) {
+    unsigned int part = b.rest + (((unsigned int)b.tail[0] + (unsigned int)b.tail[1]) + (unsigned int)b.tail[2]);
+#pragma unroll
+    for (int u = 0; u < kSpanLoads; ++u) part += sum4(b.v[u]);
+    return wave_sum(part);
+}
+
+template <int DEG, bool SCAN>
 __global__ __launch_bounds__(kShThreadsFwd) void sh_colors_fwd_kernel(
     int n, int num_bases, const float* __restrict__ means, const float* __restrict__ origin,
     const float* __restrict__ dc, const float* __restrict__ rest, float* __restrict__ colors,
-    unsigned char* __restrict__ mask, const ts::PackArgs pk) {
+    unsigned char* __restrict__ mask, const ts::PackArgs pk, const ScanArgs sc) {
     constexpr int KA = (DEG + 1) * (DEG + 1);
     constexpr int RS = 3 * (KA - 1);
     constexpr int RSP = RS | 1;
@@ -250,6 +354,16 @@
     const int g0 = blockIdx.x * kShThreadsFwd;
     const int cnt = min(kShThreadsFwd, n - g0);
     const int tid = threadIdx.x;
+    int own = 0;
+    SpanBatch front = {};
+    if (SCAN) {
+        if (blockIdx.x == 0 && tid < 64 && sc.total_out) {
+            const unsigned int total = span_sum(span_request(sc.span_sums, sc.spans, tid));
+            if (tid == 0) __hip_atomic_store(sc.total_out, (int)total, __ATOMIC_RELEASE, __HIP_MEMORY_SCOPE_SYSTEM);
+        }
+        if (tid < cnt) own = sc.cum[g0 + tid];
+        front = span_request(sc.span_sums, g0 / ts::kScanSpan, tid & 63);
+    }
     if (RS > 0) {
         const size_t row = 3 * (size_t)(num_bases - 1);
         const float* src = rest + (size_t)g0 * row;
@@ -282,10 +396,17 @@
                 lds[g * RSP + j] = src[(size_t)g * row + j];
             }
         }
-        __syncthreads();
-    }
+    }
+    unsigned int before = 0;
+    if (SCAN) before = span_sum(front);
+    if (RS > 0) __syncthreads();
     if (tid >= cnt) return;
     const int i = g0 + tid;
+    int cum_i = 0;
+    if (SCAN) {
+        cum_i = (int)((unsigned int)own + before);
+        if (g0 >= ts::kScanSpan) sc.cum[i] = cum_i;
+    }
     float Y[KA];
     ts::sh_basis(DEG, means[3 * i] - origin[0], means[3 * i + 1] - origin[1],
                  means[3 * i + 2] - origin[2], Y);
@@ -301,7 +422,7 @@
     if (mask) mask[i] = (unsigned char)((c0 >= 0.0f ? 1 : 0) | (c1 >= 0.0f ? 2 : 0) | (c2 >= 0.0f ? 4 : 0));
     c0 = fmaxf(c0, 0.0f); c1 = fmaxf(c1, 0.0f); c2 = fmaxf(c2, 0.0f);
     if (colors) { colors[3 * i] = c0; colors[3 * i + 1] = c1; colors[3 * i + 2] = c2; }
-    if (pk.splats) ts::pack_one(pk, i, c0, c1, c2, pk.channels == 4 ? pk.depths[i] : 0.0f);
+    if (pk.splats) ts::pack_one(pk, i, c0, c1, c2, pk.channels == 4 ? pk.depths[i] : 0.0f, SCAN ? &cum_i : nullptr);
 }
 
 template <int DEG>
@@ -461,20 +582,44 @@
 
 int ts_abi_version(void) { return TS_ABI_VERSION; }
 
-int ts_project_fwd(int32_t n, const float* means3d, const float* scales, const float* quats,
-                   const float* viewmat, const float* projmat, const ts_camera* cam,
-                   int32_t flags, float* xys, float* depths, int32_t* radii, float* conics,
-                   int32_t* num_tiles_hit, float* cov3d, void* stream) {
+static int launch_project_fwd(int32_t n, const float* means3d, const float* scales, const float* quats,
+                              const float* viewmat, const float* projmat, const ts_camera* cam, int32_t flags,
+                              float* xys, float* depths, int32_t* radii, float* conics, int32_t* num_tiles_hit,
+                              float* cov3d, int32_t* cum_local, int32_t* span_sums, void* stream) {
     if (n < 0 || !cam) return TS_E_BADARG;
     if (n == 0) return 0;
     if (!means3d || !scales || !quats || !viewmat || !projmat || !xys || !depths || !radii ||
         !conics || !num_tiles_hit)
         return TS_E_BADARG;
+    if (span_sums) {
+        const int spans = (n + ts::kScanSpan - 1) / ts::kScanSpan;
+        hipLaunchKernelGGL(project_fwd_kernel<true>, dim3(spans), dim3(kScanThreads), 0, (hipStream_t)stream, n,
+                           means3d, scales, quats, viewmat, projmat, *cam, (int)flags, xys, depths, radii,
+                           conics, num_tiles_hit, cov3d, cum_local, span_sums);
+        return launch_status();
+    }
     const int grid = (n + kThreads - 1) / kThreads;
-    hipLaunchKernelGGL(project_fwd_kernel, dim3(grid), dim3(kThreads), 0, (hipStream_t)stream, n,
+    hipLaunchKernelGGL(project_fwd_kernel<false>, dim3(grid), dim3(kThreads), 0, (hipStream_t)stream, n,
                        means3d, scales, quats, viewmat, projmat, *cam, (int)flags, xys, depths, radii,
-                       conics, num_tiles_hit, cov3d);
+                       conics, num_tiles_hit, cov3d, (int*)nullptr, (int*)nullptr);
     return launch_status();
+}
+
+int ts_project_fwd(int32_t n, const float* means3d, const float* scales, const float* quats,
+                   const float* viewmat, const float* projmat, const ts_camera* cam,
+                   int32_t flags, float* xys, float* depths, int32_t* radii, float* conics,
+                   int32_t* num_tiles_hit, float* cov3d, void* stream) {
+    return launch_project_fwd(n, means3d, scales, quats, viewmat, projmat, cam, flags, xys, depths, radii, conics,
+                              num_tiles_hit, cov3d, nullptr, nullptr, stream);
+}
+
+int ts_project_fwd_scan(int32_t n, const float* means3d, const float* scales, const float* quats,
+                        const float* viewmat, const float* projmat, const ts_camera* cam,
+                        int32_t flags, float* xys, float* depths, int32_t* radii, float* conics,
+                        int32_t* num_tiles_hit, int32_t* cum_tiles_hit, int32_t* scan_ws, void* stream) {
+    if (n > 0 && (!cum_tiles_hit || !scan_ws)) return TS_E_BADARG;
+    return launch_project_fwd(n, means3d, scales, quats, viewmat, projmat, cam, flags, xys, depths, radii, conics,
+                              num_tiles_hit, nullptr, cum_tiles_hit, scan_ws, stream);
 }
 
 int ts_project_bwd(int32_t n, const float* means3d, const float* scales, const float* quats,
@@ -591,7 +736,7 @@
 static int launch_colors_fwd(int32_t n, int32_t degrees_to_use, int32_t num_bases, const float* means3d,
                              const float* origin, const float* colors_dc, const float* colors_rest,
                              float* colors, uint8_t* clamp_mask, const int32_t* live, const ts::PackArgs& pk,
-                             void* stream) {
+                             const ScanArgs* scan, void* stream) {
     const int chk = sh_check(n, degrees_to_use, num_bases);
     if (chk) return chk;
     if (n == 0) return 0;
@@ -600,6 +745,7 @@
     const int grid = (n + kThreads - 1) / kThreads;
     hipStream_t s = (hipStream_t)stream;
     if (live) {
+        if (scan) return TS_E_BADARG;
 #define TS_SHC_SPARSE(D)                                                                           \
         hipLaunchKernelGGL(sh_colors_fwd_sparse_kernel<D>, dim3(grid), dim3(kThreads), 0, s, n,    \
                            num_bases, live, means3d, origin, colors_dc, colors_rest, colors, clamp_mask, pk)
@@ -616,13 +762,19 @@
     const int ka = (degrees_to_use + 1) * (degrees_to_use + 1);
     const size_t lds = (size_t)kShThreadsFwd * ((3 * (ka - 1)) | 1) * sizeof(float);
     const int grid_d = (n + kShThreadsFwd - 1) / kShThreadsFwd;
-#define TS_SHC_FWD(D)                                                                             \
+#define TS_SHC_FWD2(D, S)                                                                         \
     do {                                                                                          \
         if (lds > 48 * 1024)                                                                      \
-            (void)hipFuncSetAttribute(reinterpret_cast<const void*>(&sh_colors_fwd_kernel<D>),    \
+            (void)hipFuncSetAttribute(reinterpret_cast<const void*>(&sh_colors_fwd_kernel<D, S>), \
                                       hipFuncAttributeMaxDynamicSharedMemorySize, (int)lds);      \
-        hipLaunchKernelGGL(sh_colors_fwd_kernel<D>, dim3(grid_d), dim3(kShThreadsFwd), lds, s, n,  \
-                           num_bases, means3d, origin, colors_dc, colors_rest, colors, clamp_mask, pk); \
+        hipLaunchKernelGGL((sh_colors_fwd_kernel<D, S>), dim3(grid_d), dim3(kShThreadsFwd), lds, s, n, \
+                           num_bases, means3d, origin, colors_dc, colors_rest, colors, clamp_mask, pk, \
+                           scan ? *scan : ScanArgs{});                                            \
+    } while (0)
+#define TS_SHC_FWD(D)                                       \
+    do {                                                    \
+        if (scan) TS_SHC_FWD2(D, true);                     \
+        else TS_SHC_FWD2(D, false);                         \
     } while (0)
     switch (degrees_to_use) {
         case 0: TS_SHC_FWD(0); break;
@@ -631,6 +783,7 @@
         case 3: TS_SHC_FWD(3); break;
         default: TS_SHC_FWD(4); break;
     }
+#undef TS_SHC_FWD2
 #undef TS_SHC_FWD
     return launch_status();
 }
@@ -642,15 +795,15 @@
     none.splats = nullptr;
     if (!colors) return TS_E_BADARG;
     return launch_colors_fwd(n, degrees_to_use, num_bases, means3d, origin, colors_dc, colors_rest, colors,
-                             clamp_mask, live, none, stream);
-}
-
-int ts_colors_pack_fwd(int32_t n, int32_t degrees_to_use, int32_t num_bases, const float* means3d,
-                       const float* origin, const float* colors_dc, const float* colors_rest,
-                       uint8_t* clamp_mask, const int32_t* live, int32_t channels, int32_t flags,
-                       const float* xys, const int32_t* radii, const float* conics, const float* opacity,
-                       const int32_t* cum_tiles_hit, const ts_camera* cam, const float* depths,
-                       float* splats, void* stream) {
+                             clamp_mask, live, none, nullptr, stream);
+}
+
+static int colors_pack_fwd(int32_t n, int32_t degrees_to_use, int32_t num_bases, const float* means3d,
+                           const float* origin, const float* colors_dc, const float* colors_rest,
+                           uint8_t* clamp_mask, const int32_t* live, int32_t channels, int32_t flags,
+                           const float* xys, const int32_t* radii, const float* conics, const float* opacity,
+                           const int32_t* cum_tiles_hit, const ts_camera* cam, const float* depths,
+                           float* splats, const ScanArgs* scan, void* stream) {
     if (n < 0 || !cam || (channels != 3 && channels != 4)) return TS_E_BADARG;
     if (n > 0 && (!xys || !radii || !conics || !opacity || !cum_tiles_hit || !splats ||
                   (channels == 4 && !depths)))
@@ -660,7 +813,31 @@
     pk.opacity = opacity; pk.cum_tiles_hit = cum_tiles_hit; pk.depths = depths;
     pk.splats = reinterpret_cast<float4*>(splats); pk.cam = *cam;
     return launch_colors_fwd(n, degrees_to_use, num_bases, means3d, origin, colors_dc, colors_rest, nullptr,
-                             clamp_mask, live, pk, stream);
+                             clamp_mask, live, pk, scan, stream);
+}
+
+int ts_colors_pack_fwd(int32_t n, int32_t degrees_to_use, int32_t num_bases, const float* means3d,
+                       const float* origin, const float* colors_dc, const float* colors_rest,
+                       uint8_t* clamp_mask, const int32_t* live, int32_t channels, int32_t flags,
+                       const float* xys, const int32_t* radii, const float* conics, const float* opacity,
+                       const int32_t* cum_tiles_hit, const ts_camera* cam, const float* depths,
+                       float* splats, void* stream) {
+    return colors_pack_fwd(n, degrees_to_use, num_bases, means3d, origin, colors_dc, colors_rest, clamp_mask, live,
+                           channels, flags, xys, radii, conics, opacity, cum_tiles_hit, cam, depths, splats, nullptr,
+                           stream);
+}
+
+int ts_colors_pack_fwd_scan(int32_t n, int32_t degrees_to_use, int32_t num_bases, const float* means3d,
+                            const float* origin, const float* colors_dc, const float* colors_rest,
+                            uint8_t* clamp_mask, int32_t channels, int32_t flags, const float* xys,
+                            const int32_t* radii, const float* conics, const float* opacity,
+                            int32_t* cum_tiles_hit, const int32_t* scan_ws, int32_t* total_out,
+                            const ts_camera* cam, const float* depths, float* splats, void* stream) {
+    if (n > 0 && (!scan_ws || (reinterpret_cast<uintptr_t>(scan_ws) & 15) != 0)) return TS_E_BADARG;
+    const ScanArgs scan{cum_tiles_hit, scan_ws, total_out, n > 0 ? (n + ts::kScanSpan - 1) / ts::kScanSpan : 0};
+    return colors_pack_fwd(n, degrees_to_use, num_bases, means3d, origin, colors_dc, colors_rest, clamp_mask, nullptr,
+                           channels, flags, xys, radii, conics, opacity, cum_tiles_hit, cam, depths, splats, &scan,
+                           stream);
 }
 
 static int sh_colors_bwd_launch(int32_t n, int32_t degrees_to_use, int32_t num_bases, const float* means3d,
diff --git a/tinysplat_amd/csrc/scan_util.h b/tinysplat_amd/csrc/scan_util.h
--- /dev/null
+++ b/tinysplat_amd/csrc/scan_util.h
@@ -0,0 +1,38 @@
+#pragma once
+
+#include <hip/hip_runtime.h>
+
+namespace ts {
+
+constexpr int kScanSpan = 1024;
+
+__device__ __forceinline__ int wave_inclusive_scan(int v) {
+    const int lane = threadIdx.x & 63;
+#pragma unroll
+    for (int d = 1; d < 64; d <<= 1) {
+        const int u = __shfl_up(v, d, 64);
+        if (lane >= d) v += u;
+    }
+    return v;
+}
+
+template <int WAVES = 4>
+__device__ __forceinline__ int block_inclusive_scan(int v, int* total) {
+    __shared__ int wave_sums[WAVES];
+    const int lane = threadIdx.x & 63, wave = threadIdx.x >> 6;
+    int inc = wave_inclusive_scan(v);
+    if (lane == 63) wave_sums[wave] = inc;
+    __syncthreads();
+    int add = 0, tot = 0;
+#pragma unroll
+    for (int w = 0; w < WAVES; ++w) {
+        const int s = wave_sums[w];
+        if (w < wave) add += s;
+        tot += s;
+    }
+    *total = tot;
+    __syncthreads();
+    return inc + add;
+}
+
+}
diff --git a/tinysplat_amd/frame.py b/tinysplat_amd/frame.py
--- a/tinysplat_amd/frame.py
+++ b/tinysplat_amd/frame.py
@@ -170,6 +170,8 @@
 GROUP_COUNTS = os.environ.get("TS_GROUP_COUNTS", "1") != "0"
 
 ONE_WALK = os.environ.get("TS_ONE_WALK", "1") != "0"
+
+FUSED_SCAN = os.environ.get("TS_FUSED_SCAN", "1") != "0"
 
 CAPACITY_ALLOC = os.environ.get("TS_CAPACITY_ALLOC", "0") != "0"
 CAPACITY_GROWTH = 1.25
@@ -304,6 +306,9 @@
             fr.flags |= 1024
         if ONE_WALK:
             fr.flags |= 2048
+        fused = FUSED_SCAN and full and not stripe and n > 0
+        if fused:
+            fr.flags |= 4096
         if full:
             _stats_mode[dev.index] = mode
         fr.cam = cam
@@ -334,8 +339,12 @@
                 fr.survivors = F.bucket_ids.data_ptr() + 8 * cap
             return cap
 
-        def prepare():
+        def prepare(again=False):
+            if again:
+                fr.flags &= ~4096
             _lib.check(lib.ts_frame_fwd_prepare(ctypes.byref(fr), s), "ts_frame_fwd_prepare")
+            if fused and not again:
+                event.record()
 
         def composite():
             _lib.check(lib.ts_frame_fwd_composite(ctypes.byref(fr), s), "ts_frame_fwd_composite")
@@ -349,7 +358,8 @@
             _lib.check(lib.ts_frame_fwd_project(ctypes.byref(fr), s), "ts_frame_fwd_project")
             issued = n > 0
             _mark("fwd:call project")
-            event.record()
+            if not fused:
+                event.record()
             cap = None
             if est is not None:
                 cap = lists(est)
@@ -377,6 +387,8 @@
         finally:
             if issued and not consumed:
                 try:
+                    if fused:
+                        event.record()
                     event.synchronize()
                 except Exception:
                     pass
@@ -398,7 +410,7 @@
             fr.capacity, fr.num_intersects = -1, total
             F.segs = segments_for_count(fr.cam, F.segs, total)
             if redo:
-                prepare()
+                prepare(again=True)
             composite()
             _mark("fwd:composite enqueued")
         else:
```

Result: no change. 2053000 billion Gaussians*pixels/s (median of 2 runs) (-0.5%).
